# facebook/facebook360_dep

Measured on AMD Instinct MI355X. Metric: depth Mpix/s per GPU (full pyramid, 16-cam 2048^2 rig); % HBM-read roofline, higher is better.
Workload: dtype f32+f64; 1 GPU; BASELINE config 3: 16-camera 2048x2048 synthetic rig, 8-frame sequence, full 10-level pyramid per frame, per-level temporal filter (+-2 frames); the same sequence for every --gpus N (block partition, 8 frame(s) on this rank); rig=cfg2, cameras=16, frames=8, temporal_filter=True, halo_transport=local, parallelism=frames x1

## Files before the change

### facebook360_dep_amd/csrc/derp_capi.hip

```cpp
#include <hip/hip_runtime.h>

#include <algorithm>
#include <cfloat>
#include <cmath>
#include <cstdarg>
#include <cstdio>
#include <cstdlib>
#include <cstring>
#include <map>
#include <memory>
#include <string>
#include <vector>

#include <rocprim/device/device_radix_sort.hpp>

#include "../../include/derp_hip.h"
#include "derp_host.h"
#include "derp_kernels.h"
#include "derp_mesh.h"
#include "derp_points.h"
#include "derp_render.h"

using namespace derp;

#include "derp_ctx.h"

namespace {

struct Span {
  derp_ctx* c;
  int stage, level;
  hipEvent_t a = nullptr, b = nullptr;
  Span(derp_ctx* ctx, int st, int lv) : c(ctx), stage(st), level(lv) {
    if (c->profiling) {
      (void)hipEventCreate(&a);
      (void)hipEventCreate(&b);
      (void)hipEventRecord(a, c->stream);
    }
  }
  ~Span() {
    if (c->profiling && a) {
      (void)hipEventRecord(b, c->stream);
      c->spans.push_back({stage, level, a, b});
    }
  }
};

void drain_spans(derp_ctx* c) {
  for (auto& s : c->spans) {
    (void)hipEventSynchronize(s.b);
    float ms = 0;
    (void)hipEventElapsedTime(&ms, s.a, s.b);
    if (s.level >= 0 && s.level < kMaxLevels) {
      c->accMs[s.stage][s.level] += ms;
      c->accLaunch[s.stage][s.level] += 1;
    }
    (void)hipEventDestroy(s.a);
    (void)hipEventDestroy(s.b);
  }
  c->spans.clear();
}

size_t npx(const derp_ctx* c, int level) {
  return (size_t)c->LW[level] * c->LH[level];
}

unsigned long long* counter_slot(derp_ctx* c, int stage, int level) {
  return c->counters.as<unsigned long long>() + ((size_t)stage * kMaxLevels + level) * 4;
}

LevelView make_view(derp_ctx* c, int stage, int dst0, int nd) {
  LevelView V;
  const int L = c->cur;
  V.W = c->LW[L];
  V.H = c->LH[L];
  V.Wd = (double)V.W;
  V.Hd = (double)V.H;
  V.S = c->S;
  V.D = nd;
  V.level = L;
  V.numLevels = c->numLevels;
  V.dst0 = dst0;
  V.hasFg = c->opt.use_foreground_masks;
  const float scale = float(V.W) / c->heightFull;
  const float scaleVar = scale * scale;
  V.varNoiseFloor = std::max(c->opt.var_noise_floor * scaleVar, kMinVar);
  V.varHighThresh = c->opt.var_high_thresh;
  V.minDepthM = c->opt.min_depth_m;
  V.maxDepthM = c->opt.max_depth_m;
  V.randomProposals = c->opt.random_proposals;
  V.partialCoverage = c->opt.partial_coverage;
  V.xcdRotate = c->xcdRotate;
  V.camsSrc = c->camsSrc.as<Cam>();
  V.camsDst = c->camsDst.as<Cam>();
  V.dst2src = c->dst2src.as<int>();
  V.srcColor = c->frame().color[L].as<ushort4>();
  V.ownBias = c->w.ownBias.as<ushort4>();
  V.srcVar = c->w.srcVar.as<float>();
  V.srcFg = c->frame().fg[L].as<uint8_t>();
  V.rayDir = c->rayDir.as<double>();
  V.behind = c->behind.as<unsigned>();
  V.rayStride = (size_t)c->D * V.W * V.H;
  V.projWarp = c->projWarp.as<float2>();
  V.projColor = c->w.projColor.as<ushort4>();
  V.projBias = c->w.projBias.as<ushort4>();
  V.projColorT = c->w.projColorT.as<ushort4>();
  V.disparity = c->w.disparity.as<float>();
  V.cost = c->w.cost.as<float>();
  V.confidence = c->w.confidence.as<float>();
  V.bgDisp = c->frame().bg[L].as<float>();
  V.fovMask = c->w.fovMask.as<uint8_t>();
  V.pairCount = c->w.pairCount.as<uint8_t>();
  V.counters = counter_slot(c, stage, L);
  return V;
}

const dim3 kBlurBlk(64, 4, 1);
dim3 blur_grid(int ow, int oh, int planes) {
  return dim3((ow + 63) / 64, (oh + 4 * kBlurRows - 1) / (4 * kBlurRows), planes);
}

void lanczos_coeffs(float x, float* coeffs) {
  static const double s45 = 0.70710678118654752440084436210485;
  static const double cs[][2] = {{1, 0}, {-s45, -s45}, {0, 1}, {s45, -s45}, {-1, 0}, {s45, s45}, {0, -1}, {-s45, s45}};
  if (x < 1.1920928955078125e-07f) {
    for (int i = 0; i < 8; i++) {
      coeffs[i] = 0;
    }
    coeffs[3] = 1;
    return;
  }
  float sum = 0;
  const double y0 = -(x + 3) * M_PI * 0.25, s0 = std::sin(y0), c0 = std::cos(y0);
  for (int i = 0; i < 8; i++) {
    const double y = -(x + 3 - i) * M_PI * 0.25;
    coeffs[i] = (float)((cs[i][0] * s0 + cs[i][1] * c0) / (y * y));
    sum += coeffs[i];
  }
  sum = 1.f / sum;
  for (int i = 0; i < 8; i++) {
    coeffs[i] *= sum;
  }
}

int get_lanczos(derp_ctx* c, int ssize, int dsize, LanczosTab** out) {
  auto key = std::make_pair(ssize, dsize);
  auto it = c->lanczos.find(key);
  if (it != c->lanczos.end()) {
    *out = &it->second;
    return 0;
  }
  std::vector<int> ofs(dsize);
  std::vector<float> coef((size_t)dsize * 8);
  const double scale = (double)ssize / dsize;
  for (int d = 0; d < dsize; ++d) {
    float f = (float)((d + 0.5) * scale - 0.5);
    int s = (int)f;
    s -= (s > f);
    f -= s;
    ofs[d] = s;
    lanczos_coeffs(f, &coef[(size_t)d * 8]);
  }
  LanczosTab t;
  ALLOC(c, t.ofs, ofs.size() * sizeof(int));
  ALLOC(c, t.coef, coef.size() * sizeof(float));
  HIPCHK(c, hipMemcpyAsync(t.ofs.p, ofs.data(), ofs.size() * sizeof(int), hipMemcpyHostToDevice, c->stream));
  HIPCHK(c, hipMemcpyAsync(t.coef.p, coef.data(), coef.size() * sizeof(float), hipMemcpyHostToDevice, c->stream));
  HIPCHK(c, hipStreamSynchronize(c->stream));
  *out = &(c->lanczos[key] = std::move(t));
  return 0;
}

int get_area_tab(derp_ctx* c, int ssize, int dsize, AreaTabDev** out, bool forceTable = false) {
  auto key = std::make_pair(forceTable ? -ssize : ssize, dsize);
  auto it = c->areaTabs.find(key);
  if (it != c->areaTabs.end()) {
    *out = &it->second;
    return 0;
  }
  AreaTabDev t;
  const double scale = (double)ssize / dsize;
  const int iscale = (int)std::nearbyint(scale);
  std::vector<int> start(dsize + 1, 0), si;
  std::vector<float> alpha;
  if (!forceTable && iscale >= 1 && std::abs(scale - iscale) < 2.220446049250313e-16) {
    t.iscale = iscale;
  } else {
    for (int dx = 0; dx < dsize; ++dx) {
      start[dx] = (int)si.size();
      const double fsx1 = dx * scale, fsx2 = fsx1 + scale;
      const double cellWidth = std::min(scale, ssize - fsx1);
      int sx1 = (int)std::ceil(fsx1), sx2 = (int)std::floor(fsx2);
      sx2 = std::min(sx2, ssize - 1);
      sx1 = std::min(sx1, sx2);
      if (sx1 - fsx1 > 1e-3) {
        si.push_back(sx1 - 1);
        alpha.push_back((float)((sx1 - fsx1) / cellWidth));
      }
      for (int sx = sx1; sx < sx2; ++sx) {
        si.push_back(sx);
        alpha.push_back(float(1.0 / cellWidth));
      }
      if (fsx2 - sx2 > 1e-3) {
        si.push_back(sx2);
        alpha.push_back((float)(std::min(std::min(fsx2 - sx2, 1.), cellWidth) / cellWidth));
      }
    }
    start[dsize] = (int)si.size();
  }
  if (si.empty()) {
    si.push_back(0);
    alpha.push_back(0.f);
  }
  ALLOC(c, t.start, start.size() * sizeof(int));
  ALLOC(c, t.si, si.size() * sizeof(int));
  ALLOC(c, t.alpha, alpha.size() * sizeof(float));
  HIPCHK(c, hipMemcpy(t.start.p, start.data(), start.size() * sizeof(int), hipMemcpyHostToDevice));
  HIPCHK(c, hipMemcpy(t.si.p, si.data(), si.size() * sizeof(int), hipMemcpyHostToDevice));
  HIPCHK(c, hipMemcpy(t.alpha.p, alpha.data(), alpha.size() * sizeof(float), hipMemcpyHostToDevice));
  *out = &(c->areaTabs[key] = std::move(t));
  return 0;
}

int resize_area_dev(derp_ctx* c, int kind, const void* src, int sw, int sh, void* dst, int dw, int dh, int threshold) {
  if (dw > sw || dh > sh) {
    if (kind < 2) {
      return fail(c, "pyramid levels must not be larger than the full-size frame (%dx%d -> %dx%d)", sw, sh, dw, dh);
    }
    const dim3 g = grid2d(dw, dh, 1, kBlk2d);
    if (kind == 3) {
      hipLaunchKernelGGL(k_resize_linear_area_f32<3>, g, kBlk2d, 0, c->stream, (const float*)src, sw, sh, (float*)dst, dw, dh);
    } else {
      hipLaunchKernelGGL(k_resize_linear_area_f32<1>, g, kBlk2d, 0, c->stream, (const float*)src, sw, sh, (float*)dst, dw, dh);
    }
    KCHECK(c);
    return 0;
  }
  AreaTabDev *tx, *ty;
  TRY(get_area_tab(c, sw, dw, &tx));
  TRY(get_area_tab(c, sh, dh, &ty));
  if ((tx->iscale > 0) != (ty->iscale > 0)) {
    if (tx->iscale > 0) {
      TRY(get_area_tab(c, sw, dw, &tx, true));
    } else {
      TRY(get_area_tab(c, sh, dh, &ty, true));
    }
  }
  AreaAxis ax{tx->start.as<int>(), tx->si.as<int>(), tx->alpha.as<float>(), tx->iscale};
  AreaAxis ay{ty->start.as<int>(), ty->si.as<int>(), ty->alpha.as<float>(), ty->iscale};
  const dim3 g = grid2d(dw, dh, 1, kBlk2d);
  if (kind == 0) {
    hipLaunchKernelGGL(k_resize_area<0>, g, kBlk2d, 0, c->stream, src, sw, sh, dst, dw, dh, ax, ay, threshold);
  } else if (kind == 1) {
    hipLaunchKernelGGL(k_resize_area<1>, g, kBlk2d, 0, c->stream, src, sw, sh, dst, dw, dh, ax, ay, threshold);
  } else if (kind == 3) {
    hipLaunchKernelGGL(k_resize_area<3>, g, kBlk2d, 0, c->stream, src, sw, sh, dst, dw, dh, ax, ay, threshold);
  } else {
    hipLaunchKernelGGL(k_resize_area<2>, g, kBlk2d, 0, c->stream, src, sw, sh, dst, dw, dh, ax, ay, threshold);
  }
  KCHECK(c);
  return 0;
}

std::vector<int2> make_spiral(int w) {
  int x = 0, y = 0, dx = 0, dy = -1, t = w;
  const int samples = t * t;
  std::vector<int2> locs;
  for (int i = 0; i < samples; ++i) {
    const bool vx = (-w / 2 <= x) && (x <= w / 2), vy = (-w / 2 <= y) && (y <= w / 2);
    if (vx && vy) {
      locs.push_back(make_int2(x, y));
    }
    if (x == y || ((x < 0) && (x == -y)) || ((x > 0) && (x == 1 - y))) {
      t = dx;
      dx = -dy;
      dy = t;
    }
    x += dx;
    y += dy;
  }
  return locs;
}

int ensure_spiral(derp_ctx* c, int radius) {
  if (c->spiralRadius == radius) {
    return 0;
  }
  const std::vector<int2> s = make_spiral(radius * 2 + 1);
  ALLOC(c, c->spiral, s.size() * sizeof(int2));
  HIPCHK(c, hipMemcpy(c->spiral.p, s.data(), s.size() * sizeof(int2), hipMemcpyHostToDevice));
  c->spiralN = (int)s.size();
  c->spiralRadius = radius;
  return 0;
}

int upsample_lanczos_dev(derp_ctx* c, const float* in, int sw, int sh, float* out, int dw, int dh, int planes,
                         size_t inStride, size_t outStride) {
  if (sw == dw && sh == dh) {
    return fail(c, "upsample to identical size not supported");
  }
  LanczosTab *tx, *ty;
  TRY(get_lanczos(c, sw, dw, &tx));
  TRY(get_lanczos(c, sh, dh, &ty));
  const size_t tmpStride = (size_t)dw * sh;
  ALLOC(c, c->w.lanczosTmp, tmpStride * planes * sizeof(float));
  hipLaunchKernelGGL(k_lanczos_h, grid2d(dw, sh, planes, kBlk2d), kBlk2d, 0, c->stream, in, sw, sh, dw,
                     tx->ofs.as<int>(), tx->coef.as<float>(), c->w.lanczosTmp.as<float>(), inStride, tmpStride);
  KCHECK(c);
  hipLaunchKernelGGL(k_lanczos_v, grid2d(dw, dh, planes, kBlk2d), kBlk2d, 0, c->stream, c->w.lanczosTmp.as<float>(), sh,
                     dw, dh, ty->ofs.as<int>(), ty->coef.as<float>(), out, tmpStride, outStride);
  KCHECK(c);
  return 0;
}

int upsample_masked_dev(derp_ctx* c, const float* in, const uint8_t* mask, int sw, int sh, const uint8_t* maskUp,
                        const float* bgUp, float* out, int dw, int dh, int planes = 1) {
  const float scale = float(dw) / float(sw);
  const int radius = (int)(scale * scale + 1);
  TRY(ensure_spiral(c, radius));
  ALLOC(c, c->w.lanczosTmp, (size_t)dw * dh * planes * sizeof(float));
  hipLaunchKernelGGL(k_upsample_nearest_masked, grid2d(dw, dh, planes, kBlk2d), kBlk2d, 0, c->stream, in, mask, sw, sh,
                     maskUp, dw, dh, c->w.lanczosTmp.as<float>());
  KCHECK(c);
  hipLaunchKernelGGL(k_spiral_fill, grid2d(dw, dh, planes, kBlk2d), kBlk2d, 0, c->stream, c->w.lanczosTmp.as<float>(), bgUp,
                     maskUp, dw, dh, c->spiral.as<int2>(), c->spiralN, out);
  KCHECK(c);
  return 0;
}

bool batch_needs_inverse_warps(const derp_ctx* c, int dst0, int nd) {
  std::vector<char> covered(c->S, 0);
  for (int d = dst0; d < dst0 + nd; ++d) {
    covered[c->dst2srcH[d]] = 1;
  }
  for (int s = 0; s < c->S; ++s) {
    if (!covered[s]) {
      return true;
    }
  }
  return false;
}

size_t table_bytes_per_dst(const derp_ctx* c, int W, int H, bool withInverse) {
  const size_t wp = (size_t)(W + 2 * kPadW) * (H + 2 * kPadW), cp = (size_t)(W + 2 * kPadC) * (H + 2 * kPadC);
  return (size_t)(c->S - 1) * (wp * sizeof(float2) + 2 * cp * sizeof(ushort4) + (withInverse ? (size_t)W * H * sizeof(float2) : 0) +
                               (DERP_RANDOM_TILED ? tiled_plane(W, H) * sizeof(ushort4) : 0));
}

int compute_fov_and_masks(derp_ctx* c, int level) {
  const int W = c->LW[level], H = c->LH[level];
  const size_t n = (size_t)W * H;
  {
    Span sp(c, ST_FOV, level);
    hipLaunchKernelGGL(k_fov_mask, grid2d(W, H, c->D, kBlk2d), kBlk2d, 0, c->stream, c->camsDst.as<Cam>(), W, H,
                       c->w.fovMask.as<uint8_t>());
    KCHECK(c);
    hipLaunchKernelGGL(k_and_masks, dim3(flat_grid(n), c->D), dim3(256), 0, c->stream, c->w.fovMask.as<uint8_t>(),
                       c->frame().fg[level].as<uint8_t>(), c->dst2src.as<int>(), 0, n, c->w.maskAnd.as<uint8_t>());
    KCHECK(c);
  }
  return 0;
}

int build_warp(derp_ctx* c, int dst0, int nd) {
  const int L = c->cur;
  Span sp(c, ST_PROJ_WARP, L);
  {
    const size_t n = (size_t)c->LW[L] * c->LH[L];
    ALLOC(c, c->rayDir, 3 * n * c->D * sizeof(double));
    ALLOC(c, c->behind, n * c->D * sizeof(unsigned));
  }
  LevelView V = make_view(c, ST_PROJ_WARP, dst0, nd);
  hipLaunchKernelGGL(k_proj_warp, grid2d(V.W + 2 * kPadW, V.H + 2 * kPadW, c->S, kBlk2d), kBlk2d, 0, c->stream, V,
                     c->projWarp.as<float2>());
  KCHECK(c);
  hipLaunchKernelGGL(k_pixel_rays, grid2d(V.W, V.H, nd, kBlk2d), kBlk2d, 0, c->stream, V, c->rayDir.as<double>(),
                     c->behind.as<unsigned>());
  KCHECK(c);
  c->w.colorTablesCleanLevel = -1;
  if (batch_needs_inverse_warps(c, dst0, nd)) {
    hipLaunchKernelGGL(k_proj_warp_inv, grid2d(V.W, V.H, nd, kBlk2d), kBlk2d, 0, c->stream, V, c->projWarpInv.as<float2>());
    KCHECK(c);
  }
  return 0;
}

int build_color_tables(derp_ctx* c, int dst0, int nd) {
  const int L = c->cur;
  LevelView V = make_view(c, ST_REPROJECT, dst0, nd);
  Span sp(c, ST_REPROJECT, L);
  const dim3 grid((V.W + kRbTile - 1) / kRbTile, (V.H + kRbTile - 1) / kRbTile, nd * (c->S - 1));
  ALLOC(c, c->w.tileSeen, (size_t)grid.x * grid.y * grid.z);
  const int skipBlank = c->w.colorTablesCleanLevel == L && nd == c->D && !c->noBlankSkip;
  hipLaunchKernelGGL(k_reproject_bias, grid, dim3(256), 0, c->stream, V, c->projWarpInv.as<float2>(),
                     c->w.projColor.as<ushort4>(), c->w.projBias.as<ushort4>(), c->w.projColorT.as<ushort4>(),
                     c->w.tileSeen.as<uint8_t>(), skipBlank);
  KCHECK(c);
  c->w.colorTablesCleanLevel = nd == c->D ? L : -1;
  return 0;
}

int tiles_of(int W, int H, int& tilesX) {
  constexpr int B = kTileBlock;
  tilesX = ((W + 15) / 16 + B - 1) / B * B;
  const int tilesY = ((H + 15) / 16 + B - 1) / B * B;
  return tilesX * tilesY * (256 / kCostBlock);
}
constexpr size_t kCostLdsPerSrc = (size_t)kCostBlock * sizeof(SsdPair);
int round8(int n) {
  return (n + 7) / 8 * 8;
}
size_t lds_for_waves(size_t needed, int waves, size_t ldsPerCu, size_t fixed) {
  if (waves <= 0 || waves >= 4) {
    return needed;
  }
  const size_t perBlock = ldsPerCu / (size_t)(4 * waves + 1) + 256;
  return std::max(needed, perBlock > fixed ? perBlock - fixed : needed);
}
constexpr size_t kCostLdsStatic = sizeof(PatchWin) * (kCostBlock / 64) + kAtanLutDoubles * sizeof(double);
bool cost_four_waves(const derp_ctx* c) {
  if (const char* e = getenv("DERP_COST_WAVES")) {
    return atoi(e) >= 4;
  }
  return 16 * (kCostLdsPerSrc * (size_t)c->S + kCostLdsStatic) <= c->ldsPerCu && c->S <= 16;
}

int run_brute_force(derp_ctx* c, int dst0, int nd) {
  const int L = c->cur;
  if (L != c->numLevels - 1) {
    return 0;
  }
  Span sp(c, ST_BRUTE, L);
  LevelView V = make_view(c, ST_BRUTE, dst0, nd);
  const size_t n = (size_t)V.W * V.H;
  ALLOC(c, c->w.bruteCost, (size_t)nd * kNumDepths * n * sizeof(float));
  ALLOC(c, c->w.bruteConf, (size_t)nd * kNumDepths * n * sizeof(float));
  const int tilesX = std::max(1, (V.W - 2 + 7) / 8), tilesY = std::max(1, (V.H - 2 + 7) / 8);
  const int tiles = tilesX * tilesY;
  const size_t lds = kCostLdsPerSrc * (size_t)(c->S);
  hipLaunchKernelGGL(k_brute_costs, dim3(tiles, kNumDepths, nd), dim3(kCostBlock), lds, c->stream, V,
                     c->w.bruteCost.as<float>(), c->w.bruteConf.as<float>(), tilesX, tiles);
  KCHECK(c);
  hipLaunchKernelGGL(k_brute_select, grid2d(V.W, V.H, nd, kBlk2d), kBlk2d, 0, c->stream, V, c->w.bruteCost.as<float>(),
                     c->w.bruteConf.as<float>());
  KCHECK(c);
  hipLaunchKernelGGL(k_brute_margin, grid2d(V.W, V.H, nd, kBlk2d), kBlk2d, 0, c->stream, V);
  KCHECK(c);
  return 0;
}

int run_random_proposals(derp_ctx* c, int dst0, int nd) {
  const int L = c->cur;
  if (c->opt.random_proposals <= 0 || L == c->numLevels - 1) {
    return 0;
  }
  Span sp(c, ST_RANDOM, L);
  c->randomRanThisLevel = true;
  LevelView V = make_view(c, ST_RANDOM, dst0, nd);
  if (V.H > 2 && V.W > 2) {
    hipLaunchKernelGGL(k_row_rank, dim3(V.H - 2, nd), dim3(256), 0, c->stream, V, c->w.rank.as<int>());
    KCHECK(c);
  }
  int tilesX;
  const int tiles = tiles_of(V.W, V.H, tilesX);
  const size_t lds = lds_for_waves(kCostLdsPerSrc * (size_t)(c->S), c->randomWaves, c->ldsPerCu, kCostLdsStatic);
  hipLaunchKernelGGL(cost_four_waves(c) ? k_random_proposals : k_random_proposals_w3, dim3(round8(tiles), nd),
                     dim3(kCostBlock), lds, c->stream, V, c->w.rank.as<int>(), tilesX, tiles);
  KCHECK(c);
  return 0;
}

int run_ping_pong(derp_ctx* c, int dst0, int nd) {
  const int L = c->cur;
  if (L == c->numLevels - 1) {
    return 0;
  }
  Span sp(c, ST_PINGPONG, L);
  LevelView V = make_view(c, ST_PINGPONG, dst0, nd);
  const size_t n = (size_t)V.W * V.H;
  HIPCHK(c, hipMemsetAsync(c->w.changed.as<uint8_t>() + (size_t)dst0 * n, 1, n * nd, c->stream));
  int tilesX;
  const int tiles = tiles_of(V.W, V.H, tilesX);
  const size_t lds = lds_for_waves(kCostLdsPerSrc * (size_t)(c->S), c->ppWaves, c->ldsPerCu, kCostLdsStatic);
  const bool four = cost_four_waves(c);
  const auto kernel = c->ppCompact ? (four ? k_ping_pong : k_ping_pong_w3) : (four ? k_ping_pong_loop : k_ping_pong_loop_w3);
  for (int it = 1; it <= c->opt.ping_pong_iterations; ++it) {
    hipLaunchKernelGGL(kernel, dim3(round8(tiles), nd), dim3(kCostBlock), lds,
                       c->stream, V, c->w.changed.as<uint8_t>(), c->w.dispRes.as<float>(), c->w.costRes.as<float>(), tilesX,
                       (int)(it == 1 && c->randomRanThisLevel && !c->noMemo));
    KCHECK(c);
    hipLaunchKernelGGL(k_ping_pong_commit, dim3(flat_grid(n * nd)), dim3(256), 0, c->stream,
                       c->w.disparity.as<float>() + (size_t)dst0 * n, c->w.cost.as<float>() + (size_t)dst0 * n,
                       c->w.dispRes.as<float>() + (size_t)dst0 * n, c->w.costRes.as<float>() + (size_t)dst0 * n,
                       c->w.changed.as<uint8_t>() + (size_t)dst0 * n, n * nd);
    KCHECK(c);
  }
  if (dst0 + nd >= c->D) {
    c->randomRanThisLevel = false;
  }
  return 0;
}

int run_mismatches(derp_ctx* c) {
  const int L = c->cur;
  if (L > c->opt.mismatches_start_level || L == c->numLevels - 1) {
    return 0;
  }
  if (c->D != c->S) {
    return fail(c, "Check failed: rigDst.size() == rigSrc.size()  Mismatches only valid when considering all cameras");
  }
  for (int d = 0; d < c->D; ++d) {
    if (c->dst2srcH[d] != d) {
      return fail(c, "mismatch handling needs destinations in rig order (dst %d maps to src %d)", d, c->dst2srcH[d]);
    }
  }
  Span sp(c, ST_MISMATCH, L);
  c->randomRanThisLevel = false;
  LevelView V = make_view(c, ST_MISMATCH, 0, c->D);
  const size_t n = (size_t)V.W * V.H;
  hipLaunchKernelGGL(k_mismatch, dim3((V.W + 15) / 16, (V.H + 15) / 16, c->D), dim3(256), 256 * sizeof(float) * c->S,
                     c->stream, V, c->w.dispRes.as<float>(), c->w.mismatchMask.as<uint8_t>());
  KCHECK(c);
  HIPCHK(c, hipMemcpyAsync(c->w.disparity.p, c->w.dispRes.p, n * c->D * sizeof(float), hipMemcpyDeviceToDevice, c->stream));
  return 0;
}

int bilateral_radius(int level) {
  const float scale = std::pow(0.9f, level);
  return (int)std::max(std::ceil(5 * scale), float(1));
}

size_t bilateral_lds_bytes(int radius) {
  const size_t side = 16 + 2 * (size_t)radius;
  const size_t t = ((side + 15) & ~(size_t)15) * side;
  return t * 4 * sizeof(float) + ((t + 3) & ~(size_t)3);
}

constexpr size_t kBilateralMaxLds = 64 * 1024 - 256;

int run_bilateral(derp_ctx* c) {
  const int L = c->cur;
  Span sp(c, ST_BILATERAL, L);
  c->randomRanThisLevel = false;
  const int W = c->LW[L], H = c->LH[L];
  const size_t n = (size_t)W * H;
  const int radius = bilateral_radius(L);
  hipLaunchKernelGGL(k_joint_bilateral<true>, dim3((W + 15) / 16, (H + 15) / 16, c->D), dim3(256),
                     bilateral_lds_bytes(radius), c->stream, c->w.disparity.as<float>(),
                     (const void*)c->frame().color[L].as<ushort4>(), c->w.maskAnd.as<uint8_t>(), W, H, radius, 0.005f, 0.5f,
                     1.0f, 1.0f, c->w.tmpF.as<float>(), n, n, c->dst2src.as<int>());
  KCHECK(c);
  HIPCHK(c, hipMemcpyAsync(c->w.disparity.p, c->w.tmpF.p, n * c->D * sizeof(float), hipMemcpyDeviceToDevice, c->stream));
  return 0;
}

int run_median(derp_ctx* c, bool fuseMaskFov) {
  const int L = c->cur;
  Span sp(c, ST_MEDIAN, L);
  c->randomRanThisLevel = false;
  const int W = c->LW[L], H = c->LH[L];
  const size_t n = (size_t)W * H;
  hipLaunchKernelGGL(k_masked_median, grid2d(W, H, c->D, kBlk2d), kBlk2d, 0, c->stream, c->w.disparity.as<float>(),
                     c->opt.use_foreground_masks ? c->frame().bg[L].as<float>() : (const float*)nullptr,
                     c->w.maskAnd.as<uint8_t>(), W, H, 1, c->w.tmpF.as<float>(), n,
                     fuseMaskFov ? c->w.fovMask.as<uint8_t>() : (const uint8_t*)nullptr);
  KCHECK(c);
  HIPCHK(c, hipMemcpyAsync(c->w.disparity.p, c->w.tmpF.p, n * c->D * sizeof(float), hipMemcpyDeviceToDevice, c->stream));
  return 0;
}

int run_mask_fov(derp_ctx* c) {
  const int L = c->cur;
  Span sp(c, ST_MASKFOV, L);
  const size_t n = npx(c, L) * c->D;
  hipLaunchKernelGGL(k_mask_fov, dim3(flat_grid(n)), dim3(256), 0, c->stream, c->w.disparity.as<float>(),
                     c->w.fovMask.as<uint8_t>(), n);
  KCHECK(c);
  return 0;
}

int check_level(derp_ctx* c, int level) {
  if (!c || c->numLevels == 0) {
    return fail(c, "derp_set_pyramid has not been called");
  }
  if (level < 0 || level >= c->numLevels) {
    return fail(c, "level %d out of range [0, %d)", level, c->numLevels);
  }
  if (c->LW[level] <= 0 || c->LH[level] <= 0) {
    return fail(c, "level %d was declared absent in derp_set_pyramid", level);
  }
  return 0;
}

int level_begin(derp_ctx* c, int level, bool buildAllTables) {
  TRY(check_level(c, level));
  if (c->S - 1 > kMaxSrc) {
    return fail(c, "too many source cameras (%d > %d)", c->S, kMaxSrc + 1);
  }
  c->cur = level;
  const int W = c->LW[level], H = c->LH[level];
  const size_t n = (size_t)W * H;
  if (W < 3 || H < 3) {
    return fail(c, "level %d is too small (%dx%d)", level, W, H);
  }
  TRY(compute_fov_and_masks(c, level));
  {
    Span sp(c, ST_VARIANCE, level);
    hipLaunchKernelGGL(k_variance, grid2d(W, H, c->S, kBlk2d), kBlk2d, 0, c->stream, c->frame().color[level].as<ushort4>(),
                       W, H, c->w.srcVar.as<float>());
    KCHECK(c);
  }
  {
    Span sp(c, ST_OWN_BIAS, level);
    hipLaunchKernelGGL(k_blur3_u16, blur_grid(W, H, c->S), kBlurBlk, 0, c->stream,
                       c->frame().color[level].as<ushort4>(), 0, c->w.ownBias.as<ushort4>(), 0, W, H, n, n);
    KCHECK(c);
  }
  HIPCHK(c, hipMemsetAsync(c->w.cost.p, 0, n * c->D * sizeof(float), c->stream));
  HIPCHK(c, hipMemsetAsync(c->w.confidence.p, 0, n * c->D * sizeof(float), c->stream));
  HIPCHK(c, hipMemsetAsync(c->w.mismatchMask.p, 0, n * c->D, c->stream));
  if (level < c->numLevels - 1 && !c->frame().haveDisp[level + 1] && !buildAllTables) {
    return fail(c, "Missing disparity of level %d needed to start level %d", level + 1, level);
  }
  if (level < c->numLevels - 1 && c->frame().haveDisp[level + 1]) {
    Span sp(c, ST_UPSAMPLE, level);
    const int sw = c->LW[level + 1], sh = c->LH[level + 1];
    if (!c->opt.use_foreground_masks) {
      TRY(upsample_lanczos_dev(c, c->frame().disp[level + 1].as<float>(), sw, sh, c->w.disparity.as<float>(), W, H, c->D,
                               (size_t)sw * sh, n));
    } else {
      ALLOC(c, c->w.staging, (size_t)sw * sh * c->D);
      hipLaunchKernelGGL(k_fov_mask, grid2d(sw, sh, c->D, kBlk2d), kBlk2d, 0, c->stream, c->camsDst.as<Cam>(), sw, sh,
                         c->w.staging.as<uint8_t>());
      KCHECK(c);
      hipLaunchKernelGGL(k_and_masks, dim3(flat_grid((size_t)sw * sh), c->D), dim3(256), 0, c->stream,
                         c->w.staging.as<uint8_t>(), c->frame().fg[level + 1].as<uint8_t>(), c->dst2src.as<int>(), 0,
                         (size_t)sw * sh, c->w.staging.as<uint8_t>());
      KCHECK(c);
      TRY(upsample_masked_dev(c, c->frame().disp[level + 1].as<float>(), c->w.staging.as<uint8_t>(), sw, sh,
                              c->w.maskAnd.as<uint8_t>(), c->frame().bg[level].as<float>(), c->w.disparity.as<float>(), W, H, c->D));
    }
  } else {
// ... 127 lines not shown
    ALLOC(c, f.bg[l], n * c->D * sizeof(float));
    ALLOC(c, f.disp[l], n * c->D * sizeof(float));
    HIPCHK(c, hipMemsetAsync(f.fg[l].p, 1, n * c->S, c->stream));
    HIPCHK(c, hipMemsetAsync(f.bg[l].p, 0, n * c->D * sizeof(float), c->stream));
  }
  return 0;
}

int alloc_work_set(derp_ctx* c, WorkSet& w, size_t n) {
  ALLOC(c, w.srcVar, n * c->S * sizeof(float));
  ALLOC(c, w.ownBias, n * c->S * sizeof(ushort4));
  ALLOC(c, w.fovMask, n * c->D);
  ALLOC(c, w.maskAnd, n * c->D);
  for (DevBuf* b : {&w.disparity, &w.cost, &w.confidence, &w.dispRes, &w.costRes, &w.tmpF, &w.rank}) {
    ALLOC(c, *b, n * c->D * sizeof(float));
  }
  ALLOC(c, w.changed, n * c->D);
  ALLOC(c, w.mismatchMask, n * c->D);
  ALLOC(c, w.pairCount, n * c->D);
  return 0;
}

int select_frame(derp_ctx* c, int slot) {
  if (slot < 0 || slot >= (int)c->frames.size()) {
    return fail(c, "frame slot %d out of range [0, %d)", slot, (int)c->frames.size());
  }
  if (slot != c->curSlot) {
    c->curSlot = slot;
    c->cur = -1;
  }
  return 0;
}

void lane_swap(derp_ctx* c, int i) {
  std::swap(c->stream, c->lanes[i]->stream);
  std::swap(c->w, c->lanes[i]->w);
}

int lanes_prepare(derp_ctx* c, int count, size_t n) {
  while ((int)c->lanes.size() < count) {
    c->lanes.emplace_back(new WorkLane);
    WorkLane& l = *c->lanes.back();
    if (hipStreamCreateWithFlags(&l.stream, hipStreamNonBlocking) != hipSuccess ||
        hipEventCreateWithFlags(&l.done, hipEventDisableTiming) != hipSuccess) {
      return fail(c, "work lane: hipStreamCreate / hipEventCreate failed");
    }
  }
  if (!c->laneReady) {
    HIPCHK(c, hipEventCreateWithFlags(&c->laneReady, hipEventDisableTiming));
  }
  for (int i = 0; i < count; ++i) {
    TRY(alloc_work_set(c, c->lanes[i]->w, n));
  }
  return 0;
}

int process_level_on_lane(derp_ctx* c, int i, int slot, int level) {
  if (i < 0) {
    TRY(select_frame(c, slot));
    return process_level(c, level);
  }
  HIPCHK(c, hipStreamWaitEvent(c->lanes[i]->stream, c->laneReady, 0));
  lane_swap(c, i);
  c->activeLane = i;
  int rc = select_frame(c, slot);
  if (!rc) {
    rc = process_level(c, level);
  }
  if (!rc && hipEventRecord(c->lanes[i]->done, c->stream) != hipSuccess) {
    rc = fail(c, "work lane: hipEventRecord failed");
  }
  lane_swap(c, i);
  c->activeLane = -1;
  c->cur = -1;
  return rc;
}

int temporal_launch(derp_ctx* c, const void* const* guides, const float* const* images, const uint8_t* const* masks, int n,
                    int centre, int W, int H, int planes, float sigma, int radius, float w0, float w1, float w2,
                    float* out, const int* dst2src) {
  if (n < 1 || centre < 0 || centre >= n) {
    return fail(c, "temporal window must hold at least the centre frame");
  }
  if (n > kMaxTemporalFrames) {
    ALLOC(c, c->temporalCarry, (size_t)planes * W * H * sizeof(float2));
  }
  for (int t0 = 0; t0 < n; t0 += kMaxTemporalFrames) {
    TemporalFrames F;
    F.n = std::min(kMaxTemporalFrames, n - t0);
    for (int t = 0; t < F.n; ++t) {
      F.guides[t] = reinterpret_cast<const ushort4*>(guides[t0 + t]);
      F.images[t] = images[t0 + t];
      F.masks[t] = masks[t0 + t];
    }
    F.refGuide = reinterpret_cast<const ushort4*>(guides[centre]);
    F.refImage = images[centre];
    F.refMask = masks[centre];
    F.carry = n > kMaxTemporalFrames ? c->temporalCarry.as<float2>() : nullptr;
    F.first = t0 == 0;
    F.last = t0 + F.n >= n;
    const size_t lds = 2 * ((((size_t)(32 + 2 * radius) * (8 + 2 * radius) * 9) + 15) & ~(size_t)15);
    if (radius >= 0 && lds <= 48 * 1024 && !c->noTemporalTile) {
      hipLaunchKernelGGL(k_temporal_tiled, grid2d(W, H, planes, kBlk2d), kBlk2d, lds, c->stream, F, W, H, sigma, radius, w0,
                         w1, w2, out, dst2src);
    } else {
      hipLaunchKernelGGL(k_temporal, grid2d(W, H, planes, kBlk2d), kBlk2d, 0, c->stream, F, W, H, sigma, radius, w0, w1, w2,
                         out, dst2src);
    }
    KCHECK(c);
  }
  return 0;
}

}

extern "C" {

void derp_options_default(derp_options* o) {
  o->min_depth_m = 0.5f;
  o->max_depth_m = 1e4f;
  o->var_noise_floor = 4e-5f;
  o->var_high_thresh = 1e-3f;
  o->random_proposals = 2;
  o->ping_pong_iterations = 1;
  o->mismatches_start_level = -1;
  o->do_bilateral_filter = 1;
  o->do_median_filter = 1;
  o->use_foreground_masks = 0;
  o->partial_coverage = 0;
  o->rebuild_warp_tables = 1;
}

int derp_create(derp_ctx** out, int device, const derp_camera_desc* src, int n_src, const derp_camera_desc* dst,
                int n_dst) {
  if (!out) {
    return 1;
  }
  *out = nullptr;
  std::unique_ptr<derp_ctx> owner(new derp_ctx);
  derp_ctx* c = owner.get();
  derp_options_default(&c->opt);
  if (n_src <= 0 || n_dst <= 0) {
    return create_fail("no source / destination cameras!");
  }
  hipDeviceProp_t prop;
  TRY(open_device(device, "the depth path", &prop));
  c->device = device;
  if (prop.maxSharedMemoryPerMultiProcessor > 0) {
    c->ldsPerCu = prop.maxSharedMemoryPerMultiProcessor;
  }
  if (const char* e = getenv("DERP_XCD_ROTATE")) {
    c->xcdRotate = atoi(e);
  }
  c->noMemo = getenv("DERP_NO_MEMO") != nullptr;
  if (const char* e = getenv("DERP_PP_COMPACT")) {
    c->ppCompact = atoi(e) != 0;
  }
  if (const char* e = getenv("DERP_RANDOM_WAVES")) {
    c->randomWaves = atoi(e);
  }
  if (const char* e = getenv("DERP_PP_WAVES")) {
    c->ppWaves = atoi(e);
  }
  c->noTemporalTile = getenv("DERP_NO_TEMPORAL_TILE") != nullptr;
  c->noBlankSkip = getenv("DERP_NO_BLANK_SKIP") != nullptr;
  c->S = n_src;
  c->D = n_dst;
  c->frames.resize(1);
  c->camsSrcH.resize(n_src);
  c->camsDstH.resize(n_dst);
  for (int i = 0; i < n_src; ++i) {
    if (const char* m = host_prepare_camera(src[i], c->camsSrcH[i])) {
      return create_fail(std::string("camera ") + src[i].id + ": " + m);
    }
  }
  c->dst2srcH.assign(n_dst, 0);
  c->descDstH.assign(dst, dst + n_dst);
  for (int i = 0; i < n_dst; ++i) {
    if (const char* m = host_prepare_camera(dst[i], c->camsDstH[i])) {
      return create_fail(std::string("camera ") + dst[i].id + ": " + m);
    }
    bool found = false;
    for (int s = 0; s < n_src; ++s) {
      if (strncmp(dst[i].id, src[s].id, sizeof dst[i].id) == 0) {
        c->dst2srcH[i] = s;
        found = true;
        break;
      }
    }
    if (!found) {
      return create_fail(std::string("destination camera ") + dst[i].id + " is not a source camera");
    }
    if (memcmp(&c->camsDstH[i], &c->camsSrcH[c->dst2srcH[i]], sizeof(Cam)) != 0) {
      return create_fail(std::string("destination camera ") + dst[i].id + " differs from the source camera of the same id "
                  "(destinations must be cameras of the source rig, as filterDestinations makes them)");
    }
  }
  if (c->camsSrc.ensure(sizeof(Cam) * n_src) || c->camsDst.ensure(sizeof(Cam) * n_dst) ||
      c->dst2src.ensure(sizeof(int) * n_dst) || c->counters.ensure(sizeof(unsigned long long) * ST_COUNT * kMaxLevels * 4)) {
    return create_fail("out of device memory");
  }
  if (hipStreamCreateWithFlags(&c->stream, hipStreamNonBlocking) != hipSuccess) {
    return create_fail("hipStreamCreate failed");
  }
  if (hipStreamCreateWithFlags(&c->copyStream, hipStreamNonBlocking) != hipSuccess) {
    (void)hipStreamDestroy(c->stream);
    return create_fail("hipStreamCreate failed");
  }
  (void)hipMemcpy(c->camsSrc.p, c->camsSrcH.data(), sizeof(Cam) * n_src, hipMemcpyHostToDevice);
  (void)hipMemcpy(c->camsDst.p, c->camsDstH.data(), sizeof(Cam) * n_dst, hipMemcpyHostToDevice);
  (void)hipMemcpy(c->dst2src.p, c->dst2srcH.data(), sizeof(int) * n_dst, hipMemcpyHostToDevice);
  (void)hipMemset(c->counters.p, 0, c->counters.bytes);
  *out = owner.release();
  return 0;
}

void derp_destroy(derp_ctx* c) {
  if (!c) {
    return;
  }
  (void)hipSetDevice(c->device);
  (void)hipStreamSynchronize(c->stream);
  for (auto& l : c->lanes) {
    (void)hipStreamSynchronize(l->stream);
  }
  drain_spans(c);
  for (auto& l : c->lanes) {
    (void)hipStreamDestroy(l->stream);
    (void)hipEventDestroy(l->done);
  }
  if (c->laneReady) {
    (void)hipEventDestroy(c->laneReady);
  }
  (void)hipStreamDestroy(c->stream);
  (void)hipStreamDestroy(c->copyStream);
  delete c;
}

const char* derp_last_error(const derp_ctx* c) {
  return c ? c->err.c_str() : g_create_error.c_str();
}

int derp_set_options(derp_ctx* c, const derp_options* o) {
  if (!c || !o) {
    return 1;
  }
  if (o->random_proposals < 0) {
    return fail(c, "Check failed: random_proposals >= 0");
  }
  c->opt = *o;
  return 0;
}

int derp_set_pyramid(derp_ctx* c, int num_levels, const int* widths, const int* heights, int width_full,
                     int height_full) {
  if (!c) {
    return 1;
  }
  if (num_levels <= 0 || num_levels > kMaxLevels) {
    return fail(c, "num_levels %d out of range (1..%d)", num_levels, kMaxLevels);
  }
  HIPCHK(c, hipSetDevice(c->device));
  c->numLevels = num_levels;
  c->widthFull = width_full;
  c->heightFull = height_full;
  c->LW.assign(widths, widths + num_levels);
  c->LH.assign(heights, heights + num_levels);
  c->frames.clear();
  c->frames.resize(1);
  c->curSlot = 0;
  TRY(alloc_pyramid(c, c->frame()));
  size_t nmax = 0;
  for (int l = 0; l < num_levels; ++l) {
    nmax = std::max(nmax, npx(c, l));
  }
  TRY(alloc_work_set(c, c->w, nmax));
  c->cur = -1;
  c->warpCachedLevel = -1;
  HIPCHK(c, hipStreamSynchronize(c->stream));
  return 0;
}

int derp_set_frame_slots(derp_ctx* c, int n_slots) {
  if (!c || c->numLevels == 0) {
    return fail(c, "derp_set_pyramid has not been called");
  }
  if (n_slots < 1 || n_slots > 4096) {
    return fail(c, "n_slots %d out of range (1..4096)", n_slots);
  }
  HIPCHK(c, hipSetDevice(c->device));
  TRY(select_frame(c, 0));
  const int had = (int)c->frames.size();
  c->frames.resize(n_slots);
  for (int k = had; k < n_slots; ++k) {
    TRY(alloc_pyramid(c, c->frames[k]));
  }
  HIPCHK(c, hipStreamSynchronize(c->stream));
  return 0;
}

int derp_select_frame(derp_ctx* c, int slot) {
  if (!c || c->numLevels == 0) {
    return fail(c, "derp_set_pyramid has not been called");
  }
  return select_frame(c, slot);
}
// ... 326 lines not shown
```

### facebook360_dep_amd/csrc/derp_ctx.h

```cpp
#pragma once

namespace {

enum Stage {
  ST_FOV = 0,
  ST_VARIANCE,
  ST_OWN_BIAS,
  ST_UPSAMPLE,
  ST_PROJ_WARP,
  ST_REPROJECT,
  ST_PROJ_BIAS,
  ST_BRUTE,
  ST_RANDOM,
  ST_PINGPONG,
  ST_MISMATCH,
  ST_BILATERAL,
  ST_MEDIAN,
  ST_MASKFOV,
  ST_TEMPORAL,
  ST_LANES,
  ST_COUNT
};
const char* kStageNames[ST_COUNT] = {"fov_mask",  "variance",    "own_bias",         "upsample",  "proj_warp",
                                     "reproject", "proj_bias",   "brute_force",      "random_proposals",
                                     "ping_pong", "mismatches",  "bilateral",        "median",    "mask_fov",
                                     "temporal",  "lanes_wall"};
constexpr int kMaxLevels = 24;

struct TimedSpan {
  int stage, level;
  hipEvent_t a, b;
};

struct LanczosTab {
  DevBuf ofs, coef;
};

struct AreaTabDev {
  DevBuf start, si, alpha;
  int iscale = 0;
};

struct WorkSet {
  DevBuf srcVar, ownBias, fovMask, maskAnd, disparity, cost, confidence, dispRes, costRes, changed, tmpF, rank, mismatchMask, pairCount;
  DevBuf tileSeen;
  DevBuf projColor, projBias;
  DevBuf projColorT;
  DevBuf bruteCost, bruteConf, lanczosTmp, staging, stagingB;
  int colorTablesCleanLevel = -1;
};

struct FramePyramid {
  std::vector<DevBuf> color, fg, bg, disp;
  std::vector<char> haveBg, haveDisp;
};

struct WorkLane {
  hipStream_t stream = nullptr;
  hipEvent_t done = nullptr;
  WorkSet w;
};

struct SmrState; struct RephotoState; struct PointsState; struct MeshState;

}

struct derp_ctx {
  derp_ctx();
  ~derp_ctx();
  int device = 0;
  hipStream_t stream = nullptr;
  hipStream_t copyStream = nullptr;
  DevBuf copyStaging;
  std::string err;
  std::string* errSink() {
    return &err;
  }
  derp_options opt;
  int S = 0, D = 0;
  std::vector<Cam> camsSrcH, camsDstH;
  std::vector<int> dst2srcH;
  std::vector<derp_camera_desc> descDstH;
  DevBuf camsSrc, camsDst, dst2src;

  int numLevels = 0, widthFull = 0, heightFull = 0;
  std::vector<int> LW, LH;
  std::vector<FramePyramid> frames;
  int curSlot = 0;
  FramePyramid& frame() {
    return frames[curSlot];
  }
  DevBuf fullFrame;
  DevBuf devMask;

  int cur = -1;
  int DB = 0;
  WorkSet w;
  DevBuf temporalCarry;
  DevBuf projWarp, projWarpInv;
  DevBuf rayDir, behind;
  int warpCachedLevel = -1;
  bool randomRanThisLevel = false;
  bool tablesValid = false;
  std::map<std::pair<int, int>, LanczosTab> lanczos;
  std::map<std::pair<int, int>, AreaTabDev> areaTabs;
  DevBuf spiral;
  int spiralN = 0, spiralRadius = -1;
  std::vector<std::unique_ptr<WorkLane>> lanes;
  hipEvent_t laneReady = nullptr;
  int activeLane = -1;

  DevBuf counters;
  bool profiling = false;
  std::vector<TimedSpan> spans;
  double accMs[ST_COUNT][kMaxLevels] = {};
  int accLaunch[ST_COUNT][kMaxLevels] = {};
  int xcdRotate = 1;
  bool noMemo = false;
  bool ppCompact = true;
  int randomWaves = 0, ppWaves = 0;
  size_t ldsPerCu = 160 * 1024;
  bool noTemporalTile = false;
  bool noBlankSkip = false;
  std::unique_ptr<SmrState> smr;
  std::unique_ptr<RephotoState> rephoto;
  std::unique_ptr<PointsState> points;
  std::unique_ptr<MeshState> mesh;
};

namespace {

int fail(derp_ctx* c, const char* fmt, ...) {
  va_list ap;
  va_start(ap, fmt);
  vfail(c ? &c->err : nullptr, fmt, ap);
  va_end(ap);
  return 1;
}

int use_device(derp_ctx* c) {
  if (!c) {
    return 1;
  }
  HIPCHK(c, hipSetDevice(c->device));
  return 0;
}

int check_camera(derp_ctx* c, int cam) {
  if (cam < 0 || cam >= c->D) {
    return fail(c, "bad camera index %d (the context has %d)", cam, c->D);
  }
  return 0;
}

}
```

### facebook360_dep_amd/csrc/derp_debug_api.h

```cpp
#pragma once

namespace {
struct HostPairs {
  SsdPair* p;
  SsdPair get(int i) const {
    return p[i];
  }
  void set(int i, const SsdPair& v) {
    p[i] = v;
  }
};
int stage_index(const char* stage) {
  for (int i = 0; i < ST_COUNT; ++i) {
    if (strcmp(stage, kStageNames[i]) == 0) {
      return i;
    }
  }
  return -1;
}
}

int derp_debug_atan2_ypos(derp_ctx* c, const double* y, const double* x, double* out, size_t n) {
  if (!c || !y || !x || !out) {
    return fail(c, "bad arguments");
// ... 90 lines not shown
    return 0;
  }
  return fail(c, "unknown table id %d", which);
}

int derp_dev_disparity(derp_ctx* c, int level, int d, float** ptr, size_t* bytes) {
  TRY(check_level(c, level));
  if (d < 0 || d >= c->D || !ptr || !bytes) {
    return fail(c, "bad destination index / null output");
  }
  const size_t n = npx(c, level);
  *ptr = c->frame().disp[level].as<float>() + (size_t)d * n;
  *bytes = n * sizeof(float);
  return 0;
}
int derp_dev_color(derp_ctx* c, int level, int s, void** ptr, size_t* bytes) {
  TRY(check_level(c, level));
  if (s < 0 || s >= c->S || !ptr || !bytes) {
    return fail(c, "bad source index / null output");
  }
  const size_t n = npx(c, level);
  *ptr = c->frame().color[level].as<ushort4>() + (size_t)s * n;
  *bytes = n * sizeof(ushort4);
  return 0;
}
int derp_dev_mask(derp_ctx* c, int level, int d, uint8_t** ptr, size_t* bytes) {
  TRY(check_level(c, level));
  if (d < 0 || d >= c->D || !ptr || !bytes) {
    return fail(c, "bad destination index / null output");
  }
  HIPCHK(c, hipSetDevice(c->device));
  const int W = c->LW[level], H = c->LH[level];
  const size_t n = (size_t)W * H;
  ALLOC(c, c->devMask, n * c->D);
  hipLaunchKernelGGL(k_fov_mask, grid2d(W, H, c->D, kBlk2d), kBlk2d, 0, c->stream, c->camsDst.as<Cam>(), W, H,
                     c->devMask.as<uint8_t>());
  KCHECK(c);
  hipLaunchKernelGGL(k_and_masks, dim3(flat_grid(n), c->D), dim3(256), 0, c->stream, c->devMask.as<uint8_t>(),
                     c->frame().fg[level].as<uint8_t>(), c->dst2src.as<int>(), 0, n, c->devMask.as<uint8_t>());
  KCHECK(c);
  HIPCHK(c, hipStreamSynchronize(c->stream));
  *ptr = c->devMask.as<uint8_t>() + (size_t)d * n;
  *bytes = n;
  return 0;
}

int derp_get_counters(derp_ctx* c, uint64_t* n_cost, uint64_t* n_pair, uint64_t* insufficient) {
  if (!c) {
    return 1;
  }
  HIPCHK(c, hipStreamSynchronize(c->stream));
  std::vector<unsigned long long> h((size_t)ST_COUNT * kMaxLevels * 4);
  HIPCHK(c, hipMemcpy(h.data(), c->counters.p, h.size() * sizeof(unsigned long long), hipMemcpyDeviceToHost));
  uint64_t a = 0, b = 0, i = 0;
  for (size_t k = 0; k < h.size(); k += 4) {
    a += h[k];
    b += h[k + 1];
    i += h[k + 2];
  }
  if (n_cost) {
    *n_cost = a;
  }
  if (n_pair) {
    *n_pair = b;
  }
  if (insufficient) {
    *insufficient = i;
  }
  return 0;
}
int derp_reset_counters(derp_ctx* c) {
  if (!c) {
    return 1;
  }
  HIPCHK(c, hipMemsetAsync(c->counters.p, 0, c->counters.bytes, c->stream));
  return 0;
}
int derp_profile_enable(derp_ctx* c, int on) {
  if (!c) {
    return 1;
  }
  c->profiling = on != 0;
  return 0;
}
int derp_profile_reset(derp_ctx* c) {
  if (!c) {
    return 1;
  }
  HIPCHK(c, hipStreamSynchronize(c->stream));
  drain_spans(c);
  memset(c->accMs, 0, sizeof c->accMs);
  memset(c->accLaunch, 0, sizeof c->accLaunch);
  return derp_reset_counters(c);
}
int derp_profile_query(derp_ctx* c, const char* stage, int level, double* ms, int* launches, uint64_t* n_cost,
                       uint64_t* n_pair) {
  if (!c || !stage) {
    return 1;
  }
  const int st = stage_index(stage);
  if (st < 0) {
    return fail(c, "unknown stage '%s'", stage);
  }
  HIPCHK(c, hipStreamSynchronize(c->stream));
  drain_spans(c);
  std::vector<unsigned long long> h((size_t)kMaxLevels * 4);
  HIPCHK(c, hipMemcpy(h.data(), counter_slot(c, st, 0), h.size() * sizeof(unsigned long long), hipMemcpyDeviceToHost));
  double m = 0;
  int l = 0;
  uint64_t a = 0, b = 0;
  for (int lv = 0; lv < kMaxLevels; ++lv) {
    if (level >= 0 && lv != level) {
      continue;
    }
    m += c->accMs[st][lv];
    l += c->accLaunch[st][lv];
    a += h[(size_t)lv * 4];
    b += h[(size_t)lv * 4 + 1];
  }
  if (ms) {
    *ms = m;
  }
  if (launches) {
    *launches = l;
  }
  if (n_cost) {
    *n_cost = a;
  }
  if (n_pair) {
    *n_pair = b;
  }
  return 0;
}
int derp_profile_memoised(derp_ctx* c, const char* stage, int level, uint64_t* n_memoised) {
  if (!c || !stage || !n_memoised) {
    return 1;
  }
  const int st = stage_index(stage);
  if (st < 0) {
    return fail(c, "unknown stage '%s'", stage);
  }
  HIPCHK(c, hipStreamSynchronize(c->stream));
  std::vector<unsigned long long> h((size_t)kMaxLevels * 4);
  HIPCHK(c, hipMemcpy(h.data(), counter_slot(c, st, 0), h.size() * sizeof(unsigned long long), hipMemcpyDeviceToHost));
  uint64_t m = 0;
  for (int lv = 0; lv < kMaxLevels; ++lv) {
    if (level < 0 || lv == level) {
      m += h[(size_t)lv * 4 + 3];
    }
  }
  *n_memoised = m;
  return 0;
}
int derp_device_memory(derp_ctx* c, uint64_t* free_bytes, uint64_t* total_bytes) {
  TRY(use_device(c));
  size_t f = 0, t = 0;
  HIPCHK(c, hipMemGetInfo(&f, &t));
  if (free_bytes) {
    *free_bytes = f;
  }
  if (total_bytes) {
    *total_bytes = t;
  }
  return 0;
}

int derp_device_name(derp_ctx* c, char* buf, int n) {
  if (!c || !buf || n <= 0) {
    return 1;
  }
  hipDeviceProp_t prop;
  HIPCHK(c, hipGetDeviceProperties(&prop, c->device));
  snprintf(buf, n, "%s (%s, %d CUs)", prop.name, prop.gcnArchName, prop.multiProcessorCount);
  return 0;
}

int derp_host_nth_element_pairs(float* pairs, int n, int nth) {
  HostPairs acc{reinterpret_cast<SsdPair*>(pairs)};
  GccSelect<HostPairs> sel(acc);
  sel.nth_element(nth, n);
  return 0;
}
float derp_host_minstd_uniform(int seed, uint64_t draw_index, float a, float b) {
  uint32_t state = minstd_jump(minstd_seed(seed), draw_index);
  return minstd_uniform(state, a, b);
}
```

### facebook360_dep_amd/csrc/derp_kernels.h

```cpp
#pragma once
#include <hip/hip_runtime.h>
#include <math.h>
#include <stdint.h>

#include <type_traits>

#include "derp_camera.h"
#include "gcc_algos.h"

namespace derp {

#ifndef DERP_COST_MIN_WAVES
#define DERP_COST_MIN_WAVES 4
#endif
#ifndef DERP_RANDOM_MIN_WAVES
#define DERP_RANDOM_MIN_WAVES 4
#endif
#ifndef DERP_RANDOM_TILED
#define DERP_RANDOM_TILED 0
#endif
#ifndef DERP_MIX_HOT_ONLY
#define DERP_MIX_HOT_ONLY 0
#endif
#ifndef DERP_PHASE_TIMERS
#define DERP_PHASE_TIMERS 0
#endif
static constexpr int kCostBlock = 64;
static constexpr int kTileBlock = 4;
static constexpr int kPadW = 1;
static constexpr int kPadC = 2;
static constexpr int kMaxSrc = 32;
static constexpr int kNumDepths = 150;
static constexpr float kMinVar = 1.0f / 12.0f / 65025.0f;

typedef float f4a8 __attribute__((ext_vector_type(4), aligned(8)));
typedef unsigned int u4a8 __attribute__((ext_vector_type(4), aligned(8)));

struct LevelView {
  int W, H, S, D;
  double Wd, Hd;
  int level, numLevels;
  int dst0;
  int hasFg;
  float varNoiseFloor, varHighThresh;
  float minDepthM, maxDepthM;
  int randomProposals;
  int partialCoverage;
  int xcdRotate;
  const Cam* camsSrc;
  const Cam* camsDst;
  const int* dst2src;
  const ushort4* srcColor;
  const ushort4* ownBias;
  const float* srcVar;
  const uint8_t* srcFg;
  const double* rayDir;
  const unsigned* behind;
  size_t rayStride;
  const float2* projWarp;
  const ushort4* projColor;
  const ushort4* projBias;
  const ushort4* projColorT;
  float* disparity;
  float* cost;
  float* confidence;
  const float* bgDisp;
  const uint8_t* fovMask;
  uint8_t* pairCount;
  unsigned long long* counters;
};

__device__ __forceinline__ size_t warp_plane(const LevelView& V) {
  return (size_t)(V.W + 2 * kPadW) * (V.H + 2 * kPadW);
}
__device__ __forceinline__ size_t color_plane(const LevelView& V) {
  return (size_t)(V.W + 2 * kPadC) * (V.H + 2 * kPadC);
}
__host__ __device__ __forceinline__ int tiled_tiles_x(int W) {
  return (W + 2 * kPadC + 3) >> 2;
}
__host__ __device__ __forceinline__ size_t tiled_plane(int W, int H) {
  return (size_t)tiled_tiles_x(W) * (size_t)((H + 2 * kPadC + 3) >> 2) * 16;
}
__device__ __forceinline__ size_t tiled_index(int tilesX, int ox, int oy) {
  return ((size_t)(oy >> 2) * tilesX + (ox >> 2)) * 16 + (size_t)((oy & 3) * 4 + (ox & 3));
}
__device__ __forceinline__ int slot(int s, int own) {
  return s < own ? s : s - 1;
}
template <typename T>
__device__ __forceinline__ T& at32(T* base, unsigned i) {
  return *reinterpret_cast<T*>(reinterpret_cast<char*>(const_cast<typename std::remove_const<T>::type*>(base)) + i * (unsigned)sizeof(T));
}

__device__ __forceinline__ int xcd_swizzle(int b, int n, int rot) {
  const int per = (n + 7) >> 3;
  const int t = (((b & 7) + rot) & 7) * per + (b >> 3);
  return t;
}

__device__ __forceinline__ void tile_pixel(int item, int tilesX, int& x, int& y) {
  const int lane = threadIdx.x & 63;
  const int gw = item * (int)(blockDim.x >> 6) + (int)(threadIdx.x >> 6);
  const int super = gw >> 2, quad = gw & 3;
  constexpr int B = kTileBlock;
  const int blk = super / (B * B), in = super % (B * B);
  const int blocksX = tilesX / B;
  const int tx = (blk % blocksX) * B + (in % B), ty = (blk / blocksX) * B + (in / B);
  x = tx * 16 + (quad & 1) * 8 + (lane & 7);
  y = ty * 16 + (quad >> 1) * 8 + (lane >> 3);
}

__device__ __forceinline__ float bilerp_f(float p00, float p01, float p10, float p11, float w00, float w01,
                                          float w10, float w11) {
  return w00 * p00 + w01 * p01 + w10 * p10 + w11 * p11;
}
__device__ __forceinline__ float bilerp_u16(float p00, float p01, float p10, float p11, float w00, float w01,
                                            float w10, float w11) {
  const float v = w00 * p00 + w01 * p01 + w10 * p10 + w11 * p11;
  return __builtin_truncf(v);
}

typedef float v2f __attribute__((ext_vector_type(2)));
__device__ __forceinline__ v2f splat2(float a) {
  return (v2f){a, a};
}
__device__ __forceinline__ v2f trunc2(v2f v) {
  return (v2f){__builtin_truncf(v.x), __builtin_truncf(v.y)};
}
__device__ __forceinline__ v2f bg_of(unsigned u) {
  return (v2f){(float)(u & 0xffff), (float)(u >> 16)};
}

static constexpr int kWinW = 10, kWinTexels = kWinW * kWinW;
struct PatchWin {
  v2f bg[kWinTexels];
  float r[kWinTexels];
};

struct PixCtx {
  D3 rayO, rayD;
  const v2f* winBG;
  const float* winR;
  v2f dstBiasBG;
  float dstBiasR;
  __device__ __forceinline__ v2f patchBG(int ix, int iy) const {
    return winBG[iy * kWinW + ix];
  }
  __device__ __forceinline__ float patchR(int ix, int iy) const {
    return winR[iy * kWinW + ix];
  }
  __device__ __forceinline__ float patch(int ix, int iy, int c) const {
    return c == 2 ? patchR(ix, iy) : c == 0 ? patchBG(ix, iy).x : patchBG(ix, iy).y;
  }
  __device__ __forceinline__ float dstBias(int c) const {
    return c == 0 ? dstBiasBG.x : c == 1 ? dstBiasBG.y : dstBiasR;
  }
  float confidence;
};

__device__ __forceinline__ void patch_window_fill(const LevelView& V, int own, int x0, int y0, PatchWin* win) {
  const ushort4* col = V.srcColor + (size_t)own * ((size_t)V.W * V.H);
  for (int t = (int)(threadIdx.x & 63); t < kWinTexels; t += 64) {
    const int j = t / kWinW, i = t - j * kWinW;
    const int xx = min(max(x0 - 1 + i, 0), V.W - 1), yy = min(max(y0 - 1 + j, 0), V.H - 1);
    const ushort4 q = col[(size_t)yy * V.W + xx];
    win->bg[t] = (v2f){(float)q.x, (float)q.y};
    win->r[t] = (float)q.z;
  }
}

struct LdsPairs {
  SsdPair* base;
  int stride;
  const double* atanLut;
  __device__ __forceinline__ SsdPair get(int i) const {
    return base[i * stride];
  }
  __device__ __forceinline__ void set(int i, const SsdPair& v) {
    base[i * stride] = v;
  }
};

__device__ __forceinline__ LdsPairs cost_wave_prologue(const LevelView& V, int d, int x0, int y0, PatchWin*& win) {
  extern __shared__ SsdPair ldsPairs[];
  __shared__ PatchWin patchWin[kCostBlock / 64];
  win = &patchWin[threadIdx.x >> 6];
  patch_window_fill(V, V.dst2src[d], x0, y0, win);
#if defined(__HIP_DEVICE_COMPILE__)
  __shared__ double atanLut[kAtanLutDoubles];
  atan_lut_fill(atanLut);
  LdsPairs pairs{ldsPairs + threadIdx.x, (int)blockDim.x, atanLut};
#else
  LdsPairs pairs{ldsPairs + threadIdx.x, (int)blockDim.x, nullptr};
#endif
  __syncthreads();
  return pairs;
}

struct SsdTexels {
  u4a8 raw[4][2];
  u4a8 ba, bb;
};
template <bool TILED>
__device__ __forceinline__ void ssd_issue_random(const LevelView& V, const ushort4* __restrict__ col, const ushort4* __restrict__ colT,
                                                 const ushort4* __restrict__ bia, float xDstSrc, float yDstSrc, SsdTexels& T,
                                                 bool& border) {
  const int pitch = V.W + 2 * kPadC;
  const int xi = (int)roundf(xDstSrc), yi = (int)roundf(yDstSrc);
  const unsigned off = ((unsigned)(yi - 2 + kPadC) * (unsigned)pitch + (unsigned)(xi - 2 + kPadC)) * 8u;
  if constexpr (TILED) {
    const unsigned xa = (unsigned)(xi - 2 + kPadC), ya = (unsigned)(yi - 2 + kPadC);
    const unsigned rowTiles = (unsigned)tiled_tiles_x(V.W) * 128u;
    const unsigned xr = xa & 3u, yr = ya & 3u;
    const unsigned base0 = (ya >> 2) * rowTiles + (xa >> 2) * 128u + yr * 32u + xr * 8u;
    const char* base = reinterpret_cast<const char*>(colT);
    typedef unsigned int u2 __attribute__((ext_vector_type(2)));
#pragma unroll
    for (int row = 0; row < 4; ++row) {
      const unsigned ro = base0 + (unsigned)row * 32u + ((yr + (unsigned)row > 3u) ? rowTiles - 128u : 0u);
#pragma unroll
      for (int k = 0; k < 4; ++k) {
        const unsigned o = ro + (unsigned)k * 8u + ((xr + (unsigned)k > 3u) ? 96u : 0u);
        const u2 t = *reinterpret_cast<const u2*>(base + o);
        if (k & 1) {
          T.raw[row][k >> 1].z = t.x;
          T.raw[row][k >> 1].w = t.y;
        } else {
          T.raw[row][k >> 1].x = t.x;
          T.raw[row][k >> 1].y = t.y;
        }
      }
    }
  } else {
    const char* base = reinterpret_cast<const char*>(col);
#pragma unroll
    for (int row = 0; row < 4; ++row) {
      T.raw[row][0] = *reinterpret_cast<const u4a8*>(base + (off + (unsigned)row * (unsigned)pitch * 8u));
      T.raw[row][1] = *reinterpret_cast<const u4a8*>(base + (off + (unsigned)row * (unsigned)pitch * 8u + 16u));
    }
  }
  border = xi < 2 || yi < 2 || xi > V.W - 2 || yi > V.H - 2;
  T.ba = T.bb = (u4a8){0u, 0u, 0u, 0u};
  if (border) {
    const unsigned boff = off + ((unsigned)pitch + 1u) * 8u;
    const char* bbase = reinterpret_cast<const char*>(bia);
    T.ba = *reinterpret_cast<const u4a8*>(bbase + boff);
    T.bb = *reinterpret_cast<const u4a8*>(bbase + (boff + (unsigned)pitch * 8u));
  }
}
__device__ __forceinline__ void ssd_issue(const LevelView& V, const ushort4* __restrict__ col,
                                          const ushort4* __restrict__ bia, float xDstSrc, float yDstSrc, SsdTexels& T) {
  const int pitch = V.W + 2 * kPadC;
  const int xi = (int)roundf(xDstSrc), yi = (int)roundf(yDstSrc);
  const unsigned off = ((unsigned)(yi - 2 + kPadC) * (unsigned)pitch + (unsigned)(xi - 2 + kPadC)) * 8u;
  const char* base = reinterpret_cast<const char*>(col);
#pragma unroll
  for (int row = 0; row < 4; ++row) {
    T.raw[row][0] = *reinterpret_cast<const u4a8*>(base + (off + (unsigned)row * (unsigned)pitch * 8u));
    T.raw[row][1] = *reinterpret_cast<const u4a8*>(base + (off + (unsigned)row * (unsigned)pitch * 8u + 16u));
  }
  const unsigned boff = off + ((unsigned)pitch + 1u) * 8u;
  const char* bbase = reinterpret_cast<const char*>(bia);
  T.ba = *reinterpret_cast<const u4a8*>(bbase + boff);
  T.bb = *reinterpret_cast<const u4a8*>(bbase + (boff + (unsigned)pitch * 8u));
}

template <bool RANDOM>
__device__ __forceinline__ SsdPair ssd_arith(const LevelView& V, const PixCtx& px, const ushort4* __restrict__ col,
                                             const SsdTexels& T, float xDstSrc, float yDstSrc, bool border = true) {
  const int pitch = V.W + 2 * kPadC;
  const u4a8 (&raw)[4][2] = T.raw;
  auto word_bg = [&](const u4a8 (&q)[4][2], int r, int k) { return (k & 1) ? q[r][k >> 1].z : q[r][k >> 1].x; };
  auto word_r = [&](const u4a8 (&q)[4][2], int r, int k) { return (k & 1) ? q[r][k >> 1].w : q[r][k >> 1].y; };
  float bias[3];
  const float bxf = roundf(xDstSrc), byf = roundf(yDstSrc);
  const float bxw = xDstSrc - bxf + 0.5f, byw = yDstSrc - byf + 0.5f;
  const float w00 = (1 - bxw) * (1 - byw), w01 = bxw * (1 - byw), w10 = (1 - bxw) * byw, w11 = bxw * byw;
  if constexpr (RANDOM) {
    float top[3][2], bot[3][2];
#pragma unroll
    for (int k = 3; k >= 0; --k) {
      float c[3][4];
#pragma unroll
      for (int r = 0; r < 4; ++r) {
        const unsigned bg = word_bg(raw, r, k), rr = word_r(raw, r, k);
        c[0][r] = (float)(bg & 0xffff);
        c[1][r] = (float)(bg >> 16);
        c[2][r] = (float)(rr & 0xffff);
      }
#pragma unroll
      for (int ch = 0; ch < 3; ++ch) {
        const float m = c[ch][1] + c[ch][2];
        const float vT = m + c[ch][0], vB = m + c[ch][3];
        if (k == 3) {
          top[ch][1] = vT + 4.0f;
          bot[ch][1] = vB + 4.0f;
        } else if (k == 2) {
          top[ch][1] += vT;
          bot[ch][1] += vB;
          top[ch][0] = vT + 4.0f;
          bot[ch][0] = vB + 4.0f;
        } else if (k == 1) {
          top[ch][1] += vT;
          bot[ch][1] += vB;
          top[ch][0] += vT;
          bot[ch][0] += vB;
        } else {
          top[ch][0] += vT;
          bot[ch][0] += vB;
        }
      }
    }
    const float ninth = 1.0f / 9.0f;
#pragma unroll
    for (int ch = 0; ch < 3; ++ch) {
      const float t00 = __builtin_truncf(top[ch][0] * ninth), t01 = __builtin_truncf(top[ch][1] * ninth);
      const float t10 = __builtin_truncf(bot[ch][0] * ninth), t11 = __builtin_truncf(bot[ch][1] * ninth);
      bias[ch] = px.dstBias(ch) - bilerp_u16(t00, t01, t10, t11, w00, w01, w10, w11);
    }
    if (__ballot(border) != 0ull) {
      if (border) {
        const u4a8 a = T.ba, b = T.bb;
        bias[0] = px.dstBias(0) - bilerp_u16((float)(a.x & 0xffff), (float)(a.z & 0xffff), (float)(b.x & 0xffff), (float)(b.z & 0xffff), w00, w01, w10, w11);
        bias[1] = px.dstBias(1) - bilerp_u16((float)(a.x >> 16), (float)(a.z >> 16), (float)(b.x >> 16), (float)(b.z >> 16), w00, w01, w10, w11);
        bias[2] = px.dstBias(2) - bilerp_u16((float)(a.y & 0xffff), (float)(a.w & 0xffff), (float)(b.y & 0xffff), (float)(b.w & 0xffff), w00, w01, w10, w11);
      }
    }
  } else {
    const u4a8 a = T.ba, b = T.bb;
    const v2f sbBG = trunc2(splat2(w00) * bg_of(a.x) + splat2(w01) * bg_of(a.z) + splat2(w10) * bg_of(b.x) +
                            splat2(w11) * bg_of(b.z));
    const v2f bBG = px.dstBiasBG - sbBG;
    bias[0] = bBG.x;
    bias[1] = bBG.y;
    bias[2] = px.dstBiasR - bilerp_u16((float)(a.y & 0xffff), (float)(a.w & 0xffff), (float)(b.y & 0xffff),
                                       (float)(b.w & 0xffff), w00, w01, w10, w11);
  }
  float first = 0.f, second = 0.f;
  u4a8 rawB[4][2];
#pragma unroll
  for (int r = 0; r < 4; ++r) {
    rawB[r][0] = raw[r][0];
    rawB[r][1] = raw[r][1];
    if constexpr (RANDOM) {
      unsigned a = raw[r][1].x, b = raw[r][1].y, c = raw[r][1].z, d = raw[r][1].w;
      asm("" : "+v"(a), "+v"(b), "+v"(c), "+v"(d));
      rawB[r][1] = (u4a8){a, b, c, d};
    }
  }
// ... 69 lines not shown
        const v2f v = splat2(w00) * lo.bg[iy] + splat2(w01) * hi.bg[iy] + splat2(w10) * lo.bg[iy + 1] +
                      splat2(w11) * hi.bg[iy + 1];
        const v2f db = px.patchBG(ix, iy) - trunc2(v);
        const v2f dn = db - biasBG;
        const v2f s0 = db * db, s1 = dn * dn;
        float t0 = s0.x + s0.y, t1 = s1.x + s1.y;
        asm("" : "+v"(t0), "+v"(t1));
        bgd0[iy] = t0;
        bgd1[iy] = t1;
      }
      v2f e0, e1;
      {
        const v2f v = w00p * lo.rE + w01p * hi.rE + w10p * lo.rO + w11p * hi.rO;
        const v2f db = (v2f){px.patchR(ix, 0), px.patchR(ix, 2)} - trunc2(v);
        const v2f dn = db - splat2(bias[2]);
        e0 = (v2f){bgd0[0], bgd0[2]} + db * db;
        e1 = (v2f){bgd1[0], bgd1[2]} + dn * dn;
      }
      float m0, m1;
      {
        const float v = w00m * lo.rO.x + w01m * hi.rO.x + w10m * lo.rE.y + w11m * hi.rE.y;
        const float db = px.patchR(ix, 1) - __builtin_truncf(v);
        const float dn = db - bias[2];
        m0 = bgd0[1] + db * db;
        m1 = bgd1[1] + dn * dn;
      }
      first += e0.x;
      first += m0;
      first += e0.y;
      second += e1.x;
      second += m1;
      second += e1.y;
      lo = hi;
    }
  };
  const float xfc = roundf(xDstSrc), yfc = roundf(yDstSrc);
  const bool exact = (xDstSrc >= 1.0f) && (yDstSrc >= 1.0f) && ((xDstSrc + 1.0f) - 1.0f == xDstSrc) &&
                     ((yDstSrc + 1.0f) - 1.0f == yDstSrc);
  int xi[3], yi[3];
  float xw[3], yw[3];
  bool regular = true;
  xi[1] = (int)xfc;
  yi[1] = (int)yfc;
  xw[0] = xw[1] = xw[2] = xDstSrc - xfc + 0.5f;
  yw[0] = yw[1] = yw[2] = yDstSrc - yfc + 0.5f;
  if (!exact) {
#pragma unroll
    for (int k = 0; k < 3; k += 2) {
      const float xs = xDstSrc + (float)(k - 1), ys = yDstSrc + (float)(k - 1);
      const float xf = roundf(xs), yf = roundf(ys);
      xi[k] = (int)xf;
      yi[k] = (int)yf;
      xw[k] = xs - xf + 0.5f;
      yw[k] = ys - yf + 0.5f;
    }
    regular = (xi[0] == xi[1] - 1) && (xi[2] == xi[1] + 1) && (yi[0] == yi[1] - 1) && (yi[2] == yi[1] + 1);
  }
  if (!RANDOM && __ballot(!exact) == 0ull) {
    const float xwu[3] = {xw[1], xw[1], xw[1]};
    block_packed(xwu, splat2(yw[1]), yw[1]);
  } else if (regular) {
    if constexpr (RANDOM) {
      block_scalar(xw, yw);
    } else {
      block_packed(xw, (v2f){yw[0], yw[2]}, yw[1]);
    }
  } else if (DERP_MIX_HOT_ONLY) {
    first = second = 0.f;
  } else {
    for (int ix = 0; ix < 3; ++ix) {
      for (int iy = 0; iy < 3; ++iy) {
        const float w00 = (1 - xw[ix]) * (1 - yw[iy]), w01 = xw[ix] * (1 - yw[iy]);
        const float w10 = (1 - xw[ix]) * yw[iy], w11 = xw[ix] * yw[iy];
        const int x0 = min(max(xi[ix] - 1, -kPadC), V.W + kPadC - 1), x1 = min(max(xi[ix], -kPadC), V.W + kPadC - 1);
        const int y0 = min(max(yi[iy] - 1, -kPadC), V.H + kPadC - 1), y1 = min(max(yi[iy], -kPadC), V.H + kPadC - 1);
        const ushort4 q00 = col[(size_t)(y0 + kPadC) * pitch + x0 + kPadC];
        const ushort4 q01 = col[(size_t)(y0 + kPadC) * pitch + x1 + kPadC];
        const ushort4 q10 = col[(size_t)(y1 + kPadC) * pitch + x0 + kPadC];
        const ushort4 q11 = col[(size_t)(y1 + kPadC) * pitch + x1 + kPadC];
        const float p00[3] = {(float)q00.x, (float)q00.y, (float)q00.z};
        const float p01[3] = {(float)q01.x, (float)q01.y, (float)q01.z};
        const float p10[3] = {(float)q10.x, (float)q10.y, (float)q10.z};
        const float p11[3] = {(float)q11.x, (float)q11.y, (float)q11.z};
        const v2f pbg = px.winBG[iy * kWinW + ix];
        const float pch[3] = {pbg.x, pbg.y, px.winR[iy * kWinW + ix]};
        float d0 = 0.f, d1 = 0.f;
        for (int c = 0; c < 3; ++c) {
          const float cs = bilerp_u16(p00[c], p01[c], p10[c], p11[c], w00, w01, w10, w11);
          const float db = pch[c] - cs;
          const float dn = db - bias[c];
          d0 += db * db;
          d1 += dn * dn;
        }
        first += d0;
        second += d1;
      }
    }
  }
  const float scale = 1.0f / (65535.0f * 65535.0f);
  return {first * scale, second * scale};
}
template <bool RANDOM>
__device__ __forceinline__ SsdPair compute_ssd(const LevelView& V, const PixCtx& px, const ushort4* __restrict__ col,
                                               const ushort4* __restrict__ bia, float xDstSrc, float yDstSrc,
                                               const ushort4* __restrict__ colT = nullptr) {
  SsdTexels T;
  if constexpr (RANDOM) {
    bool border;
    ssd_issue_random<DERP_RANDOM_TILED != 0>(V, col, colT, bia, xDstSrc, yDstSrc, T, border);
    return ssd_arith<true>(V, px, col, T, xDstSrc, yDstSrc, border);
  } else {
    ssd_issue(V, col, bia, xDstSrc, yDstSrc, T);
    return ssd_arith<false>(V, px, col, T, xDstSrc, yDstSrc);
  }
}

static constexpr double kCullMinDepth = 0.05;
__device__ __forceinline__ unsigned behind_mask(const LevelView& V, int own, const D3& rayO, const D3& rayD) {
  unsigned m = 0;
  for (int s = 0; s < V.S; ++s) {
    if (s == own) {
      continue;
    }
    const Cam& cs = V.camsSrc[s];
    const double a = sum3(cs.R[6] * (rayO.x - cs.pos[0]), cs.R[7] * (rayO.y - cs.pos[1]), cs.R[8] * (rayO.z - cs.pos[2]));
    const double b = sum3(cs.R[6] * rayD.x, cs.R[7] * rayD.y, cs.R[8] * rayD.z);
    if (cs.cos_fov >= 0 && b > 1e-6 && a + kCullMinDepth * b > 1e-6) {
      m |= 1u << slot(s, own);
    }
  }
  return m;
}
__device__ __forceinline__ unsigned behind_sources(const LevelView& V, int d, size_t idx) {
  const unsigned m = V.behind[(size_t)d * ((size_t)V.W * V.H) + idx];
  unsigned cull = 0;
  for (int t = 0; t < V.S - 1; ++t) {
    if (__ballot(!((m >> t) & 1u)) == 0ull) {
      cull |= 1u << t;
    }
  }
  return __builtin_amdgcn_readfirstlane(cull);
}

struct PhaseTimers {
  unsigned proj = 0, ssd = 0, select = 0, inside = 0;
};
__device__ __forceinline__ unsigned phase_clock() {
#if DERP_PHASE_TIMERS
  return (unsigned)__builtin_amdgcn_s_memtime();
#else
  return 0u;
#endif
}
template <bool RANDOM>
constexpr int cost_sees_lean() {
  return 2 + (RANDOM ? 4 : 0);
}

template <bool RANDOM = false, bool RELOAD_RAY = false>
__device__ __forceinline__ float2 compute_cost(const LevelView& V, int dl, int own, const PixCtx& px, float disparity,
                                               LdsPairs& pairs, unsigned& nPair, unsigned cull = 0, unsigned pix = 0,
                                               unsigned* slots = nullptr, PhaseTimers* tm = nullptr) {
  const unsigned tc0 = phase_clock();
  const double depth = (double)(1.0f / disparity);
  D3 rayD = px.rayD;
  if constexpr (RELOAD_RAY) {
    unsigned i = pix;
    asm("" : "+v"(i) : "v"(disparity));
    const double* rd = V.rayDir + (size_t)(V.dst0 + dl) * ((size_t)V.W * V.H);
    if constexpr (RANDOM) {
      rayD = {at32(rd, i), at32(rd + V.rayStride, i), at32(rd + 2 * V.rayStride, i)};
    } else {
      rayD = {rd[i], rd[V.rayStride + i], rd[2 * V.rayStride + i]};
    }
  }
  const D3 pWorld = {px.rayO.x + rayD.x * depth, px.rayO.y + rayD.y * depth, px.rayO.z + rayD.z * depth};
  const size_t wPlane = warp_plane(V), cPlane = color_plane(V);
  const int wPitch = V.W + 2 * kPadW;
  unsigned mask = 0, waveMask = 0;
  cull = __builtin_amdgcn_readfirstlane(__ballot(!(depth >= kCullMinDepth)) != 0ull ? 0u : cull);
  const ushort4* colBase = V.projColor + (size_t)dl * (V.S - 1) * cPlane;
  const ushort4* biaBase = V.projBias + (size_t)dl * (V.S - 1) * cPlane;
  const size_t tPlane = tiled_plane(V.W, V.H);
  const ushort4* colTBase = RANDOM ? V.projColorT + (size_t)dl * (V.S - 1) * tPlane : nullptr;
  {
    bool pend = false;
    int pendSlot = 0;
    f4a8 pa = {0, 0, 0, 0}, pb = {0, 0, 0, 0};
    float pxw = 0, pyw = 0;
    auto consume = [&]() {
      const float w00 = (1 - pxw) * (1 - pyw), w01 = pxw * (1 - pyw), w10 = (1 - pxw) * pyw, w11 = pxw * pyw;
      const float wx = bilerp_f(pa.x, pa.z, pb.x, pb.z, w00, w01, w10, w11);
      const float wy = bilerp_f(pa.y, pa.w, pb.y, pb.w, w00, w01, w10, w11);
      const float xDstSrc = wx + 0.5f, yDstSrc = wy + 0.5f;
      const bool ok = pend && !(isnan(xDstSrc) || isnan(yDstSrc));
      if (ok) {
        pairs.set(pendSlot, SsdPair{xDstSrc, yDstSrc});
        mask |= 1u << pendSlot;
      }
      if (__ballot(ok) != 0ull) {
        waveMask |= 1u << pendSlot;
      }
    };
    for (int s = 0; s < V.S; ++s) {
      if (s == own || ((cull >> slot(s, own)) & 1u)) {
        continue;
      }
      const Cam& cs = V.camsSrc[s];
      D2 pn;
      const bool vis = sees<cost_sees_lean<RANDOM>()>(cs, pWorld, cs.principal[0], cs.principal[1], cs.focal[0], cs.focal[1],
                                                      1.0, 1.0, pn, pairs.atanLut);
      if (__ballot(pend) != 0ull) {
        consume();
      }
      pend = vis;
      pendSlot = slot(s, own);
      if (__ballot(vis) != 0ull) {
        const float sx = (float)(pn.x * V.Wd), sy = (float)(pn.y * V.Hd);
        const float xf = roundf(sx), yf = roundf(sy);
        const int xi = (int)xf, yi = (int)yf;
        pxw = sx - xf + 0.5f;
        pyw = sy - yf + 0.5f;
        const size_t tab = (size_t)dl * (V.S - 1) + pendSlot;
        const char* wbase = reinterpret_cast<const char*>(V.projWarp + tab * wPlane);
        const unsigned woff = vis ? ((unsigned)(yi - 1 + kPadW) * (unsigned)wPitch + (unsigned)(xi - 1 + kPadW)) * 8u : 0u;
        pa = *reinterpret_cast<const f4a8*>(wbase + woff);
        pb = *reinterpret_cast<const f4a8*>(wbase + (woff + (unsigned)wPitch * 8u));
      }
    }
    if (__ballot(pend) != 0ull) {
      consume();
    }
  }
  const unsigned tc1 = phase_clock();
  const int ssdCount = __popc(mask);
  nPair += ssdCount;
#ifdef DERP_COUNT_UNION
  if (slots) {
    *slots += __popc(__builtin_amdgcn_readfirstlane(waveMask));
  }
#endif
  int keep = 1;
  if (ssdCount < keep) {
    return make_float2(3.402823466e+38f, 0.0f);
  }
  {
    int cnt = 0;
    for (unsigned wm = __builtin_amdgcn_readfirstlane(waveMask); wm != 0; wm &= wm - 1) {
      const int t = __builtin_ctz(wm);
      if ((mask >> t) & 1) {
        const SsdPair e = pairs.get(t);
        const SsdPair ssd = compute_ssd<RANDOM>(V, px, colBase + (size_t)t * cPlane, biaBase + (size_t)t * cPlane, e.first,
                                                        e.second, RANDOM ? colTBase + (size_t)t * tPlane : nullptr);
        pairs.set(cnt, ssd);
        ++cnt;
      }
    }
  }
  const unsigned tc2 = phase_clock();
  keep = max(keep, ssdCount - 2);
  GccSelect<LdsPairs> sel(pairs);
  sel.nth_element(keep, ssdCount);
  float cost = 0;
  for (int i = 0; i < keep; ++i) {
    cost += pairs.get(i).second;
  }
  cost /= (float)keep;
  const float trustCoef = 1.0f / (float)keep;
  float confidence = px.confidence;
  if constexpr (RELOAD_RAY) {
    unsigned i = pix;
    asm("" : "+v"(i) : "v"(cost));
    if constexpr (RANDOM) {
      confidence = fmaxf(at32(V.srcVar + (size_t)own * ((size_t)V.W * V.H), i), kMinVar);
    } else {
      confidence = fmaxf((V.srcVar + (size_t)own * ((size_t)V.W * V.H))[i], kMinVar);
    }
  }
  const float costFinal = cost * trustCoef / confidence;
#if DERP_PHASE_TIMERS
  if (tm) {
    const unsigned tc3 = phase_clock();
    tm->proj += tc1 - tc0, tm->ssd += tc2 - tc1, tm->select += tc3 - tc2, tm->inside += tc3 - tc0;
  }
#endif
  return make_float2(costFinal, confidence);
}

template <bool WITH_RAY = true>
__device__ __forceinline__ void load_pixctx(const LevelView& V, int d, int own, int x, int y, const PatchWin* win, PixCtx& px,
                                            int tl = -1) {
  const Cam& cd = V.camsDst[d];
  px.rayO = {cd.pos[0], cd.pos[1], cd.pos[2]};
  const size_t n = (size_t)V.W * V.H;
  if constexpr (!WITH_RAY) {
    px.rayD = {0, 0, 0};
  } else {
    const size_t i = (size_t)d * n + (size_t)y * V.W + x;
    px.rayD = {V.rayDir[i], V.rayDir[V.rayStride + i], V.rayDir[2 * V.rayStride + i]};
  }
  if (tl < 0) {
    tl = (int)(threadIdx.x & 63);
  }
  const int corner = (tl >> 3) * kWinW + (tl & 7);
  px.winBG = win->bg + corner;
  px.winR = win->r + corner;
// ... 446 lines not shown
    for (int oy = oya; oy <= oyb; ++oy) {
      for (int ox = oxa; ox <= oxb; ++ox) {
        pc[(size_t)oy * OW + ox] = col;
        pb[(size_t)oy * OW + ox] = bia;
        if (pt) {
          pt[tiled_index(tilesX, ox, oy)] = col;
        }
      }
    }
  }
}

__device__ __forceinline__ float probe_disparity(int i, float minD, float maxD) {
  const double fraction = (double)i / (double)(kNumDepths - 1);
  return (float)(fraction * (double)minD + (1 - fraction) * (double)maxD);
}

__global__ void __launch_bounds__(kCostBlock, DERP_COST_MIN_WAVES)
    k_brute_costs(LevelView V, float* __restrict__ costs, float* __restrict__ confs, int tilesX, int tilesPerDst) {
  const int i = blockIdx.y;
  const int dl = blockIdx.z;
  const int d = V.dst0 + dl;
  const int iw = V.W - 2, ih = V.H - 2;
  const int lane = threadIdx.x & 63;
  const int sx = (int)(blockIdx.x % (unsigned)tilesX), sy = (int)(blockIdx.x / (unsigned)tilesX);
  const int x = 1 + sx * 8 + (lane & 7), y = 1 + sy * 8 + (lane >> 3);
  PatchWin* win;
  LdsPairs pairs = cost_wave_prologue(V, d, x - (int)(threadIdx.x & 7), y - (int)((threadIdx.x & 63) >> 3), win);
  unsigned nCost = 0, nPair = 0;
  if (x <= iw && y <= ih) {
    const int own = V.dst2src[d];
    const size_t n = (size_t)V.W * V.H, idx = (size_t)y * V.W + x;
    const float minDisparity = 1.0f / V.maxDepthM, maxDisparity = 1.0f / V.minDepthM;
    const float disparity = probe_disparity(i, minDisparity, maxDisparity);
    const bool fov = V.fovMask[(size_t)d * n + idx], fg = V.srcFg[(size_t)own * n + idx];
    const bool closer = V.hasFg ? (V.bgDisp[(size_t)d * n + idx] < disparity) : true;
    float2 r = make_float2(__builtin_nanf(""), __builtin_nanf(""));
    if (fov && fg && closer) {
      PixCtx px;
      load_pixctx(V, d, own, x, y, win, px);
      r = compute_cost(V, dl, own, px, disparity, pairs, nPair);
      ++nCost;
    }
    const size_t o = ((size_t)dl * kNumDepths + i) * n + idx;
    costs[o] = r.x;
    confs[o] = r.y;
  }
  flush_counters(V, nCost, nPair);
}

__global__ void k_brute_select(LevelView V, const float* __restrict__ costs, const float* __restrict__ confs) {
  const int dl = blockIdx.z;
  const int d = V.dst0 + dl;
  const int x = blockIdx.x * blockDim.x + threadIdx.x, y = blockIdx.y * blockDim.y + threadIdx.y;
  if (x < 1 || y < 1 || x >= V.W - 1 || y >= V.H - 1) {
    return;
  }
  const int own = V.dst2src[d];
  const size_t n = (size_t)V.W * V.H, idx = (size_t)y * V.W + x;
  float* disp = V.disparity + (size_t)d * n;
  if (!V.fovMask[(size_t)d * n + idx]) {
    disp[idx] = __builtin_nanf("");
    return;
  }
  if (!V.srcFg[(size_t)own * n + idx]) {
    disp[idx] = V.bgDisp[(size_t)d * n + idx];
    return;
  }
  float minCost = 3.402823466e+38f, minConf = 0;
  int best = -1;
  for (int i = 0; i < kNumDepths; ++i) {
    const size_t o = ((size_t)dl * kNumDepths + i) * n + idx;
    const float c = costs[o];
    if (c < minCost) {
      minCost = c;
      minConf = confs[o];
      best = i;
    }
  }
  const float minDisparity = 1.0f / V.maxDepthM, maxDisparity = 1.0f / V.minDepthM;
  if (best == -1) {
    atomicAdd(&V.counters[2], 1ull);
    disp[idx] = minDisparity;
  } else {
    disp[idx] = probe_disparity(best, minDisparity, maxDisparity);
  }
  V.cost[(size_t)d * n + idx] = minCost;
  V.confidence[(size_t)d * n + idx] = minConf;
}

__global__ void k_brute_margin(LevelView V) {
  const int d = V.dst0 + blockIdx.z;
  const int x = blockIdx.x * blockDim.x + threadIdx.x, y = blockIdx.y * blockDim.y + threadIdx.y;
  if (x >= V.W || y >= V.H) {
    return;
  }
  if (!(x < 1 || x >= V.W - 1 || y < 1 || y >= V.H - 1)) {
    return;
  }
  const int own = V.dst2src[d];
  const size_t n = (size_t)V.W * V.H, idx = (size_t)y * V.W + x;
  if (!V.srcFg[(size_t)own * n + idx]) {
    V.disparity[(size_t)d * n + idx] = V.bgDisp[(size_t)d * n + idx];
    return;
  }
  const int yy = min(max(y, 1), V.H - 2), xx = min(max(x, 1), V.W - 2);
  const size_t src = (size_t)yy * V.W + xx;
  V.disparity[(size_t)d * n + idx] = V.disparity[(size_t)d * n + src];
  V.cost[(size_t)d * n + idx] = V.cost[(size_t)d * n + src];
  V.confidence[(size_t)d * n + idx] = V.confidence[(size_t)d * n + src];
}

__device__ __forceinline__ bool random_gate(const LevelView& V, int d, int own, size_t idx) {
  const size_t n = (size_t)V.W * V.H;
  if (!V.fovMask[(size_t)d * n + idx] || !V.srcFg[(size_t)own * n + idx]) {
    return false;
  }
  const float varHighDev = 0.1f * V.varHighThresh;
  const float thresh = fmaxf(varHighDev, V.varNoiseFloor);
  return !(V.srcVar[(size_t)own * n + idx] < thresh);
}

__global__ void __launch_bounds__(256) k_row_rank(LevelView V, int* __restrict__ rank) {
  __shared__ int partial[256];
  const int d = V.dst0 + blockIdx.y, y = blockIdx.x + 1;
  const int own = V.dst2src[d];
  const size_t n = (size_t)V.W * V.H;
  const int inner = V.W - 2;
  const int per = (inner + 255) / 256;
  const int x0 = 1 + threadIdx.x * per, x1 = min(x0 + per, V.W - 1);
  int cnt = 0;
  for (int x = x0; x < x1; ++x) {
    cnt += random_gate(V, d, own, (size_t)y * V.W + x);
  }
  partial[threadIdx.x] = cnt;
  __syncthreads();
  for (int off = 1; off < 256; off <<= 1) {
    const int v = ((int)threadIdx.x >= off) ? partial[threadIdx.x - off] : 0;
    __syncthreads();
    partial[threadIdx.x] += v;
    __syncthreads();
  }
  const int run = partial[threadIdx.x] - cnt;
  uint32_t state = minstd_jump(minstd_seed(y * V.level), (uint64_t)V.randomProposals * (uint64_t)run);
  const uint32_t aP = minstd_jump(1u, (uint64_t)V.randomProposals);
  for (int x = x0; x < x1; ++x) {
    rank[(size_t)d * n + (size_t)y * V.W + x] = (int)state;
    if (random_gate(V, d, own, (size_t)y * V.W + x)) {
      state = minstd_mulmod(state, aP);
    }
  }
}

__device__ __forceinline__ void random_proposals_body(const LevelView& V, const int* __restrict__ rank, int tilesX, int tilesPerDst) {
  const int dl = blockIdx.y;
  const int d = V.dst0 + dl;
  int x, y;
  tile_pixel(xcd_swizzle(blockIdx.x, gridDim.x, V.xcdRotate ? d : 0), tilesX, x, y);
  PatchWin* win;
  LdsPairs pairs = cost_wave_prologue(V, d, x - (int)(threadIdx.x & 7), y - (int)((threadIdx.x & 63) >> 3), win);
  unsigned nCost = 0, nPair = 0, nSlots = 0, nSlotsFirst = 0;
  PhaseTimers tm;
  const unsigned tk0 = phase_clock();
  if (x >= 1 && y >= 1 && x < V.W - 1 && y < V.H - 1) {
    const int own = V.dst2src[d];
    const size_t n = (size_t)V.W * V.H;
    const unsigned idx = (unsigned)y * (unsigned)V.W + (unsigned)x;
    float* disp = V.disparity + (size_t)d * n;
    if ((V.fovMask + (size_t)d * n)[idx]) {
      if (!(V.srcFg + (size_t)own * n)[idx]) {
        disp[idx] = (V.bgDisp + (size_t)d * n)[idx];
      } else if (random_gate(V, d, own, idx)) {
        PixCtx px;
        load_pixctx<false>(V, d, own, x, y, win, px);
        const unsigned cull = behind_sources(V, d, idx);
        float currDisp = at32(disp, idx);
        float currCost = 0.f, costThresh = 0.f, amplitude = 0.f;
        const int spare = V.S - 1;
        const float maxDisp = 1.0f / V.minDepthM;
        uint32_t state = (uint32_t)at32(rank + (size_t)d * n, idx);
        for (int i = -1; i < V.randomProposals; ++i) {
          unsigned pi = idx;
          asm("" : "+v"(pi) : "s"(i));
          const float minDisp = V.hasFg ? at32(V.bgDisp + (size_t)d * n, pi) : (1.0f / V.maxDepthM);
          float propDisp = currDisp;
          if (i >= 0) {
            const float lo = fmaxf(minDisp, currDisp - amplitude), hi = fminf(maxDisp, currDisp + amplitude);
            propDisp = minstd_uniform(state, lo, hi);
          }
          unsigned np = 0;
          const float2 pr = compute_cost<true, true>(V, dl, own, px, propDisp, pairs, np, cull, pi, i < 0 ? &nSlotsFirst : &nSlots, &tm);
          nPair += np;
          bool take;
          if (i < 0) {
            costThresh = fminf(0.5f * pr.x, 5.0f);
            amplitude = (maxDisp - minDisp) / 2.0f;
            take = true;
          } else {
            take = pr.x < currCost && pr.x < costThresh;
            if (take) {
              amplitude /= 2.0f;
            }
          }
          if (take) {
            currCost = pr.x;
            currDisp = propDisp;
            pairs.set(spare, SsdPair{pr.y, __uint_as_float(np)});
          }
        }
        {
          unsigned pi = idx;
          asm("" : "+v"(pi) : "v"(currCost));
          const SsdPair best = pairs.get(spare);
          at32(V.confidence + (size_t)d * n, pi) = best.first;
          at32(V.pairCount + (size_t)d * n, pi) = (uint8_t)__float_as_uint(best.second);
          at32(disp, pi) = currDisp;
          at32(V.cost + (size_t)d * n, pi) = currCost;
        }
        nCost = 1u + (unsigned)max(V.randomProposals, 0);
      }
    }
  }
#if DERP_PHASE_TIMERS
  if ((threadIdx.x & 63) == 0) {
    const unsigned body = phase_clock() - tk0;
    atomicAdd(&V.counters[0], (unsigned long long)(DERP_PHASE_TIMERS == 1 ? tm.proj : body));
    atomicAdd(&V.counters[1], (unsigned long long)(DERP_PHASE_TIMERS == 1 ? tm.ssd : body - tm.inside));
    atomicAdd(&V.counters[3], (unsigned long long)(DERP_PHASE_TIMERS == 1 ? tm.select : 0u));
  }
  return;
#endif
  flush_counters(V, nCost, nPair);
#ifdef DERP_COUNT_UNION
  atomicAdd(&V.counters[3], (unsigned long long)nSlots);
  atomicAdd(&V.counters[2], (unsigned long long)nSlotsFirst);
#endif
}

__global__ void __launch_bounds__(kCostBlock, DERP_RANDOM_MIN_WAVES)
    k_random_proposals(LevelView V, const int* __restrict__ rank, int tilesX, int tilesPerDst) {
  random_proposals_body(V, rank, tilesX, tilesPerDst);
}
__global__ void __launch_bounds__(kCostBlock, 3)
    k_random_proposals_w3(LevelView V, const int* __restrict__ rank, int tilesX, int tilesPerDst) {
  random_proposals_body(V, rank, tilesX, tilesPerDst);
}

__constant__ int kCandidates[9][2] = {{0, 0}, {-1, 0}, {1, 0}, {0, -1}, {0, 1}, {-2, -2}, {2, -2}, {-2, 2}, {2, 2}};
constexpr int kCandOff[9][2] = {{0, 0}, {-1, 0}, {1, 0}, {0, -1}, {0, 1}, {-2, -2}, {2, -2}, {-2, 2}, {2, 2}};
constexpr unsigned cand_pack(int c) {
  unsigned p = 0;
  for (int k = 0; k < 9; ++k) {
    p |= (unsigned)(kCandOff[k][c] + 2) << (3 * k);
  }
  return p;
}
constexpr unsigned kCandPackX = cand_pack(0), kCandPackY = cand_pack(1);

#ifdef DERP_COUNT_PP_FILL
__device__ __forceinline__ unsigned pp_fill_entry() {
  return __builtin_ctzll(__ballot(1)) == (int)(threadIdx.x & 63) ? 64u : 0u;
}
#endif

__device__ __forceinline__ void ping_pong_candidates_loop(const LevelView& V, const uint8_t* __restrict__ changed, int dl, int x,
                                                          int y, const PatchWin* win, LdsPairs& pairs, int useMemo, float& outDisp,
                                                          float& outCost, unsigned& counts, unsigned& fillSlots, PhaseTimers& tm) {
  const int d = V.dst0 + dl;
  const int own = V.dst2src[d];
  const size_t n = (size_t)V.W * V.H;
  const unsigned idx = (unsigned)y * (unsigned)V.W + (unsigned)x;
  const float* disp = V.disparity + (size_t)d * n;
  const uint8_t* fov = V.fovMask + (size_t)d * n;
  const uint8_t* chg = changed + (size_t)d * n;
  outDisp = disp[idx];
  const bool interior = x >= 1 && y >= 1 && x < V.W - 1 && y < V.H - 1;
  if (interior && fov[idx]) {
    if (!V.srcFg[(size_t)own * n + idx]) {
      outDisp = V.bgDisp[(size_t)d * n + idx];
    } else if (!(V.srcVar[(size_t)own * n + idx] < V.varNoiseFloor)) {
      PixCtx px;
      load_pixctx<false>(V, d, own, x, y, win, px);
      const unsigned cull = behind_sources(V, d, idx);
      float bestCost = __builtin_inff();
      float bestDisp = outDisp;
      const unsigned xy = (unsigned)x | ((unsigned)y << 16);
      for (int k = 0; k < 9; ++k) {
        unsigned q = xy;
        asm("" : "+v"(q) : "s"(k));
        const int px0 = (int)(q & 0xffffu), py0 = (int)(q >> 16);
        const unsigned pidx = (unsigned)py0 * (unsigned)V.W + (unsigned)px0;
        const int xx = min(max(px0 + kCandidates[k][0], 0), V.W - 1);
        const int yy = min(max(py0 + kCandidates[k][1], 0), V.H - 1);
        const unsigned j = (unsigned)yy * (unsigned)V.W + (unsigned)xx;
        if (fov[j]) {
          const float cand = disp[j];
          const float bg = V.hasFg ? (V.bgDisp + (size_t)d * n)[pidx] : 0.f;
          if (cand >= bg && chg[j]) {
            float2 r;
            const float memoConf = (k == 0 && useMemo) ? (V.confidence + (size_t)d * n)[pidx] : 0.0f;
            if (memoConf != 0.0f) {
              r = make_float2((V.cost + (size_t)d * n)[pidx], memoConf);
              counts += (unsigned)(V.pairCount + (size_t)d * n)[pidx] + (1u << 24);
            } else {
              unsigned np = 0;
#ifdef DERP_COUNT_PP_FILL
              fillSlots += pp_fill_entry();
#endif
              r = compute_cost<false, true>(V, dl, own, px, cand, pairs, np, cull, pidx, nullptr, &tm);
              counts += np;
            }
            counts += 1u << 16;
            if (r.x < bestCost) {
              bestCost = r.x;
              bestDisp = cand;
            }
          }
        }
      }
      outDisp = bestDisp;
      outCost = bestCost;
    }
  }
}

__device__ __forceinline__ void ping_pong_candidates_compact(const LevelView& V, const uint8_t* __restrict__ changed, int dl, int& x,
                                                             int& y, const PatchWin* win, LdsPairs& pairs, int useMemo, float& outDisp,
                                                             float& outCost, unsigned& counts, unsigned& fillSlots, PhaseTimers& tm) {
  const int d = V.dst0 + dl;
  const int own = V.dst2src[d];
  const size_t n = (size_t)V.W * V.H;
  const int lane = (int)(threadIdx.x & 63);
  const float* disp = V.disparity + (size_t)d * n;
  const uint8_t* fov = V.fovMask + (size_t)d * n;
  const uint8_t* chg = changed + (size_t)d * n;
  unsigned cmask = 0;
  bool eval = false;
  const unsigned idx = (unsigned)y * (unsigned)V.W + (unsigned)x;
  if (x < V.W && y < V.H) {
    outDisp = disp[idx];
    const bool interior = x >= 1 && y >= 1 && x < V.W - 1 && y < V.H - 1;
    if (interior && fov[idx]) {
      if (!V.srcFg[(size_t)own * n + idx]) {
        outDisp = V.bgDisp[(size_t)d * n + idx];
      } else if (!(V.srcVar[(size_t)own * n + idx] < V.varNoiseFloor)) {
        eval = true;
        const float bg = V.hasFg ? (V.bgDisp + (size_t)d * n)[idx] : 0.f;
        for (int k = 0; k < 9; ++k) {
          const int xx = min(max(x + (int)((kCandPackX >> (3 * k)) & 7u) - 2, 0), V.W - 1);
          const int yy = min(max(y + (int)((kCandPackY >> (3 * k)) & 7u) - 2, 0), V.H - 1);
          const unsigned j = (unsigned)yy * (unsigned)V.W + (unsigned)xx;
          if (fov[j]) {
            const float cand = disp[j];
            if (cand >= bg && chg[j]) {
              const float memoConf = (k == 0 && useMemo) ? (V.confidence + (size_t)d * n)[idx] : 0.0f;
              if (memoConf != 0.0f) {
                const float c = (V.cost + (size_t)d * n)[idx];
                counts += (unsigned)(V.pairCount + (size_t)d * n)[idx] + (1u << 24) + (1u << 16);
                if (c < outCost) {
                  outCost = c;
                  outDisp = cand;
                }
              } else {
                cmask |= 1u << k;
              }
            }
          }
        }
      }
    }
  }
  unsigned cull = 0;
  const unsigned behind = eval ? V.behind[(size_t)d * n + idx] : ~0u;
  for (int t = 0; t < V.S - 1; ++t) {
    if (__ballot(!((behind >> t) & 1u)) == 0ull) {
      cull |= 1u << t;
    }
  }
  cull = __builtin_amdgcn_readfirstlane(cull);
  int incl = __popc(cmask);
  for (int off = 1; off < 64; off <<= 1) {
    const int v = __builtin_amdgcn_ds_bpermute((lane - off) << 2, incl);
    if (lane >= off) {
      incl += v;
    }
  }
  const int total = __builtin_amdgcn_readlane(incl, 63);
  const unsigned list = cmask | ((unsigned)incl << 16);
  const int x0 = __builtin_amdgcn_readfirstlane(x - (lane & 7)), y0 = __builtin_amdgcn_readfirstlane(y - (lane >> 3));
  extern __shared__ SsdPair ldsPairs[];
  SsdPair* const wavePairs = ldsPairs + (__builtin_amdgcn_readfirstlane(threadIdx.x) & ~63u);
  SsdPair* const stage = wavePairs + (size_t)(V.S - 1) * pairs.stride;
  for (int base = 0; base < total; base += 64) {
    int ln = lane;
    asm("" : "+v"(ln) : "s"(base));
    const int t = base + ln;
    int o = 0;
    for (int step = 32; step > 0; step >>= 1) {
      if ((int)((unsigned)__builtin_amdgcn_ds_bpermute((o + step - 1) << 2, (int)list) >> 16) <= t) {
        o += step;
      }
    }
    o = min(o, 63);
    const unsigned ol = (unsigned)__builtin_amdgcn_ds_bpermute(o << 2, (int)list);
    unsigned m = ol & 0xffffu;
    const int oStart = (int)(ol >> 16) - __popc(m);
#ifdef DERP_COUNT_PP_FILL
    fillSlots += ln == 0 ? 64u : 0u;
#endif
    if (t < total) {
      for (int r = t - oStart; r > 0; --r) {
        m &= m - 1;
      }
      const int k = __builtin_ctz(m);
      const int ox = x0 + (o & 7), oy = y0 + (o >> 3);
      const unsigned pidx = (unsigned)oy * (unsigned)V.W + (unsigned)ox;
      const int xx = min(max(ox + (int)((kCandPackX >> (3 * k)) & 7u) - 2, 0), V.W - 1);
      const int yy = min(max(oy + (int)((kCandPackY >> (3 * k)) & 7u) - 2, 0), V.H - 1);
      const float cand = disp[(unsigned)yy * (unsigned)V.W + (unsigned)xx];
      PixCtx px;
      load_pixctx<false>(V, d, own, ox, oy, win, px, o);
      LdsPairs lp{wavePairs + ln, pairs.stride, pairs.atanLut};
      unsigned np = 0;
      const float2 r = compute_cost<false, true>(V, dl, own, px, cand, lp, np, cull, pidx, nullptr, &tm);
      counts += np + (1u << 16);
      int sl = lane;
      asm("" : "+v"(sl) : "v"(r.x));
      stage[sl] = SsdPair{r.x, cand};
    }
    __builtin_amdgcn_fence(__ATOMIC_SEQ_CST, "wavefront");
    __builtin_amdgcn_wave_barrier();
    const int end = (int)(list >> 16);
    const int lo = max(end - __popc(list & 0xffffu), base), hi = min(end, base + 64);
    for (int i = lo; i < hi; ++i) {
      const SsdPair e = stage[i - base];
      if (e.first < outCost) {
        outCost = e.first;
        outDisp = e.second;
      }
    }
    __builtin_amdgcn_fence(__ATOMIC_SEQ_CST, "wavefront");
    __builtin_amdgcn_wave_barrier();
  }
  x = x0 + (lane & 7);
  y = y0 + (lane >> 3);
}

template <bool COMPACT>
__device__ __forceinline__ void ping_pong_body(const LevelView& V, const uint8_t* __restrict__ changed, float* __restrict__ dispRes,
                                               float* __restrict__ costRes, int tilesX, int useMemo) {
  const int dl = blockIdx.y;
  const int d = V.dst0 + dl;
  int x, y;
  tile_pixel(xcd_swizzle(blockIdx.x, gridDim.x, V.xcdRotate ? d : 0), tilesX, x, y);
  PatchWin* win;
  LdsPairs pairs = cost_wave_prologue(V, d, x - (int)(threadIdx.x & 7), y - (int)((threadIdx.x & 63) >> 3), win);
  unsigned counts = 0, fillSlots = 0;
  PhaseTimers tm;
  const unsigned tk0 = phase_clock();
  float outDisp = 0.f;
  float outCost = __builtin_inff();
  if constexpr (COMPACT) {
    ping_pong_candidates_compact(V, changed, dl, x, y, win, pairs, useMemo, outDisp, outCost, counts, fillSlots, tm);
  } else if (x < V.W && y < V.H) {
    ping_pong_candidates_loop(V, changed, dl, x, y, win, pairs, useMemo, outDisp, outCost, counts, fillSlots, tm);
  }
  if (x < V.W && y < V.H) {
    const size_t n = (size_t)V.W * V.H;
    const unsigned idx = (unsigned)y * (unsigned)V.W + (unsigned)x;
    (dispRes + (size_t)d * n)[idx] = outDisp;
    (costRes + (size_t)d * n)[idx] = outCost;
  }
#if DERP_PHASE_TIMERS
  if ((threadIdx.x & 63) == 0) {
    const unsigned body = phase_clock() - tk0;
    atomicAdd(&V.counters[0], (unsigned long long)(DERP_PHASE_TIMERS == 1 ? tm.proj : body));
    atomicAdd(&V.counters[1], (unsigned long long)(DERP_PHASE_TIMERS == 1 ? tm.ssd : body - tm.inside));
    atomicAdd(&V.counters[3], (unsigned long long)(DERP_PHASE_TIMERS == 1 ? tm.select : 0u));
  }
  return;
#endif
  unsigned nMemo = counts >> 24;
#ifdef DERP_COUNT_PP_FILL
  flush_counters(V, (counts >> 16) & 0xffu, fillSlots);
#else
  (void)fillSlots;
  flush_counters(V, (counts >> 16) & 0xffu, counts & 0xffffu);
#endif
  for (int off = 32; off > 0; off >>= 1) {
    nMemo += __shfl_down(nMemo, off);
  }
  if ((threadIdx.x & 63) == 0 && nMemo) {
    atomicAdd(&V.counters[3], (unsigned long long)nMemo);
  }
}

__global__ void __launch_bounds__(kCostBlock, DERP_COST_MIN_WAVES)
    k_ping_pong(LevelView V, const uint8_t* __restrict__ changed, float* __restrict__ dispRes,
                float* __restrict__ costRes, int tilesX, int useMemo) {
  ping_pong_body<true>(V, changed, dispRes, costRes, tilesX, useMemo);
}
__global__ void __launch_bounds__(kCostBlock, 3)
    k_ping_pong_w3(LevelView V, const uint8_t* __restrict__ changed, float* __restrict__ dispRes,
                   float* __restrict__ costRes, int tilesX, int useMemo) {
  ping_pong_body<true>(V, changed, dispRes, costRes, tilesX, useMemo);
}
__global__ void __launch_bounds__(kCostBlock, DERP_COST_MIN_WAVES)
    k_ping_pong_loop(LevelView V, const uint8_t* __restrict__ changed, float* __restrict__ dispRes,
                     float* __restrict__ costRes, int tilesX, int useMemo) {
  ping_pong_body<false>(V, changed, dispRes, costRes, tilesX, useMemo);
}
__global__ void __launch_bounds__(kCostBlock, 3)
    k_ping_pong_loop_w3(LevelView V, const uint8_t* __restrict__ changed, float* __restrict__ dispRes,
                        float* __restrict__ costRes, int tilesX, int useMemo) {
  ping_pong_body<false>(V, changed, dispRes, costRes, tilesX, useMemo);
}

__global__ void k_ping_pong_commit(float* __restrict__ disp, float* __restrict__ cost, const float* __restrict__ dispRes,
                                   const float* __restrict__ costRes, uint8_t* __restrict__ changed, size_t n) {
  size_t i = (size_t)blockIdx.x * blockDim.x + threadIdx.x;
  const size_t step = (size_t)gridDim.x * blockDim.x;
  for (; i < n; i += step) {
    const float a = disp[i], b = dispRes[i];
    changed[i] = (a != b);
    disp[i] = b;
    cost[i] = costRes[i];
  }
}

__device__ __forceinline__ float clamp_fetch(const float* img, int x, int y, int W, int H) {
  return img[(size_t)min(max(y, 0), H - 1) * W + min(max(x, 0), W - 1)];
}

__global__ void __launch_bounds__(256)
    k_mismatch(LevelView V, float* __restrict__ newDisp, uint8_t* __restrict__ mismatchMask) {
  extern __shared__ float ldsMis[];
  const int d = blockIdx.z;
  const int x = blockIdx.x * 16 + (threadIdx.x & 15), y = blockIdx.y * 16 + (threadIdx.x >> 4);
  if (x >= V.W || y >= V.H) {
    return;
  }
  const size_t n = (size_t)V.W * V.H, idx = (size_t)y * V.W + x;
  if (!V.fovMask[(size_t)d * n + idx]) {
    newDisp[(size_t)d * n + idx] = __builtin_nanf("");
    return;
  }
  float* mis = ldsMis + threadIdx.x;
  const int own = V.dst2src[d];
  const float curr = V.disparity[(size_t)d * n + idx];
  int nMatch = 0, nMis = 0;
  if (V.srcFg[(size_t)own * n + idx]) {
    const Cam& cd = V.camsDst[d];
    const D3 dir = rig_direction(cd, (x + 0.5) / (double)V.W, (y + 0.5) / (double)V.H, cd.principal[0], cd.principal[1],
                                 cd.focal[0], cd.focal[1]);
    const double depth = (double)(1.0f / curr);
    const D3 pWorld = {cd.pos[0] + dir.x * depth, cd.pos[1] + dir.y * depth, cd.pos[2] + dir.z * depth};
    const float dMin = (1.0f - 0.1f) * curr, dMax = (1.0f + 0.1f) * curr;
    for (int s = 0; s < V.S; ++s) {
      if (s == own) {
        continue;
      }
      const Cam& cs = V.camsSrc[s];
      D2 pn;
      if (!sees(cs, pWorld, cs.principal[0], cs.principal[1], cs.focal[0], cs.focal[1], 1.0, 1.0, pn)) {
        continue;
      }
      const float sx = (float)(pn.x * (double)V.W), sy = (float)(pn.y * (double)V.H);
      const float xf = roundf(sx), yf = roundf(sy);
      const int xi = (int)xf, yi = (int)yf;
      const float xw = sx - xf + 0.5f, yw = sy - yf + 0.5f;
      const float* img = V.disparity + (size_t)s * n;
      const float dSrc = bilerp_f(clamp_fetch(img, xi - 1, yi - 1, V.W, V.H), clamp_fetch(img, xi, yi - 1, V.W, V.H),
                                  clamp_fetch(img, xi - 1, yi, V.W, V.H), clamp_fetch(img, xi, yi, V.W, V.H),
                                  (1 - xw) * (1 - yw), xw * (1 - yw), (1 - xw) * yw, xw * yw);
      if (dMin <= dSrc && dSrc <= dMax) {
        ++nMatch;
      } else {
        mis[(nMis++) * 256] = dSrc;
      }
    }
  }
  bool mask = false;
  float dispNew = curr;
  if (nMatch + nMis != 0) {
    const float var = V.srcVar[(size_t)own * n + idx];
    if (!(nMatch >= 1 || V.varHighThresh < var || var < V.varNoiseFloor)) {
      mask = true;
      for (int i = 1; i < nMis; ++i) {
        const float v = mis[i * 256];
        int k = i;
        while (k > 0 && mis[(k - 1) * 256] > v) {
          mis[k * 256] = mis[(k - 1) * 256];
          --k;
        }
        mis[k * 256] = v;
      }
      int closer = 0;
      for (; closer < nMis; ++closer) {
        if (mis[closer * 256] >= curr) {
          break;
        }
      }
      const float m = mis[(closer / 2) * 256];
      dispNew = (m < curr) ? m : curr;
    }
  }
  mismatchMask[(size_t)d * n + idx] = mask;
  newDisp[(size_t)d * n + idx] = dispNew;
}

__global__ void k_layer_disparities(const float* __restrict__ fg, const float* __restrict__ bg, size_t n,
                                    uint8_t* __restrict__ out) {
  size_t i = (size_t)blockIdx.x * blockDim.x + threadIdx.x;
  const size_t step = (size_t)gridDim.x * blockDim.x;
  for (; i < n; i += step) {
    const float m = fg[i] > 0.0f ? 1.0f : 0.0f;
    const float layer = fg[i] * m + bg[i] * (1 - m);
    const int r = cv_round(layer * 255.0f);
    out[i] = (uint8_t)min(max(r, 0), 255);
  }
}

__global__ void __launch_bounds__(kCostBlock, DERP_COST_MIN_WAVES)
    k_cost_map(LevelView V, int d, const float* __restrict__ dispIn, float* __restrict__ costOut,
               float* __restrict__ confOut, int tilesX) {
  const int dl = d - V.dst0;
  int x, y;
  tile_pixel(blockIdx.x, tilesX, x, y);
  PatchWin* win;
  LdsPairs pairs = cost_wave_prologue(V, d, x - (int)(threadIdx.x & 7), y - (int)((threadIdx.x & 63) >> 3), win);
  unsigned nCost = 0, nPair = 0;
  if (x >= 1 && y >= 1 && x < V.W - 1 && y < V.H - 1) {
    const int own = V.dst2src[d];
    PixCtx px;
    load_pixctx(V, d, own, x, y, win, px);
    const float2 r = compute_cost(V, dl, own, px, dispIn[(size_t)y * V.W + x], pairs, nPair);
    ++nCost;
    costOut[(size_t)y * V.W + x] = r.x;
    confOut[(size_t)y * V.W + x] = r.y;
  }
  flush_counters(V, nCost, nPair);
}

__constant__ unsigned long long kExp2fTab[32] = {
    0x3ff0000000000000ull, 0x3fefd9b0d3158574ull, 0x3fefb5586cf9890full, 0x3fef9301d0125b51ull,
    0x3fef72b83c7d517bull, 0x3fef54873168b9aaull, 0x3fef387a6e756238ull, 0x3fef1e9df51fdee1ull,
    0x3fef06fe0a31b715ull, 0x3feef1a7373aa9cbull, 0x3feedea64c123422ull, 0x3feece086061892dull,
    0x3feebfdad5362a27ull, 0x3feeb42b569d4f82ull, 0x3feeab07dd485429ull, 0x3feea47eb03a5585ull,
    0x3feea09e667f3bcdull, 0x3fee9f75e8ec5f74ull, 0x3feea11473eb0187ull, 0x3feea589994cce13ull,
    0x3feeace5422aa0dbull, 0x3feeb737b0cdc5e5ull, 0x3feec49182a3f090ull, 0x3feed503b23e255dull,
    0x3feee89f995ad3adull, 0x3feeff76f2fb5e47ull, 0x3fef199bdd85529cull, 0x3fef3720dcef9069ull,
    0x3fef5818dcfba487ull, 0x3fef7c97337b9b5full, 0x3fefa4afa2a490daull, 0x3fefd0765b6e4540ull};

__device__ __forceinline__ float div_by_const(float y, double rcp) {
  return (float)((double)y * rcp);
}

__device__ __forceinline__ float div_int_by_const(int y, double rcp) {
  return (float)((double)y * rcp);
}

__device__ __forceinline__ float expf_glibc(float x, const unsigned long long* tab) {
  const double InvLn2N = 0x1.71547652b82fep+0 * 32;
  const double C0 = 0x1.c6af84b912394p-5 / 32 / 32 / 32, C1 = 0x1.ebfce50fac4f3p-3 / 32 / 32,
               C2 = 0x1.62e42ff0c52d6p-1 / 32;
  const double SHIFT = 0x1.8p+52;
  const unsigned abstop = (__float_as_uint(x) >> 20) & 0x7ff;
  if (abstop >= (0x42b00000u >> 20)) {
    if (__float_as_uint(x) == 0xff800000u) {
// ... 1228 lines not shown
```

### facebook360_dep_amd/derp.py

```python
import ctypes as C
import os

import numpy as np

_HERE = os.path.dirname(os.path.abspath(__file__))
LIB_PATH = os.environ.get("DERP_LIB") or os.path.join(_HERE, "libderp_hip.so")
CAM_TYPES = {"FTHETA": 0, "RECTILINEAR": 1, "EQUISOLID": 2, "ORTHOGRAPHIC": 3}

STAGES = ["fov_mask", "variance", "own_bias", "upsample", "proj_warp", "reproject", "proj_bias", "brute_force",
          "random_proposals", "ping_pong", "mismatches", "bilateral", "median", "mask_fov", "temporal"]


class SeqOptions(C.Structure):
    _fields_ = [
        ("time_radius", C.c_int32), ("sigma", C.c_float), ("weight_b", C.c_float), ("weight_g", C.c_float),
        ("weight_r", C.c_float), ("space_radius", C.c_int32), ("use_foreground_masks", C.c_int32),
        ("partition", C.c_int32), ("do_temporal_filter", C.c_int32), ("resident_frames", C.c_int32),
    ]


class SeqTransfer(C.Structure):
    _fields_ = [("frame", C.c_int32), ("from_rank", C.c_int32), ("to_rank", C.c_int32)]


class CameraDesc(C.Structure):
    _fields_ = [
        ("type", C.c_int32), ("has_principal", C.c_int32), ("has_distortion", C.c_int32), ("has_fov", C.c_int32),
        ("origin", C.c_double * 3), ("forward", C.c_double * 3), ("up", C.c_double * 3), ("right", C.c_double * 3),
        ("resolution", C.c_double * 2), ("focal", C.c_double * 2), ("principal", C.c_double * 2),
        ("distortion", C.c_double * 3), ("fov", C.c_double), ("id", C.c_char * 64),
    ]


class Options(C.Structure):
    _fields_ = [
        ("min_depth_m", C.c_float), ("max_depth_m", C.c_float), ("var_noise_floor", C.c_float),
        ("var_high_thresh", C.c_float), ("random_proposals", C.c_int32), ("ping_pong_iterations", C.c_int32),
        ("mismatches_start_level", C.c_int32), ("do_bilateral_filter", C.c_int32), ("do_median_filter", C.c_int32),
        ("use_foreground_masks", C.c_int32), ("partial_coverage", C.c_int32), ("rebuild_warp_tables", C.c_int32),
    ]


class MeshPass(C.Structure):
    _fields_ = [("faces", C.c_longlong), ("feasible", C.c_longlong), ("winners", C.c_longlong), ("applied", C.c_longlong),
                ("deleted", C.c_longlong), ("threshold", C.c_double)]


class RenderParams(C.Structure):
    _fields_ = [
        ("kind", C.c_int32), ("width", C.c_int32), ("height", C.c_int32), ("position", C.c_double * 3),
        ("forward", C.c_double * 3), ("up", C.c_double * 3), ("horizontal_fov", C.c_double), ("ipd", C.c_float),
        ("alpha_blend", C.c_int32), ("disparity_color", C.c_int32), ("weight", C.c_int32), ("zero_nans", C.c_int32),
    ]


RENDER_KINDS = {"cube": 0, "equirect": 1, "snapshot": 2}
WEIGHTS = {"svd": 0, "minor": 1}
FORMATS = ["cubecolor", "cubedisp", "eqrcolor", "eqrdisp", "lr180", "snapcolor", "snapdisp", "tb3dof", "tbstereo"]


def render_params(kind="equirect", width=3072, height=None, position=(0, 0, 0), forward=(-1, 0, 0), up=(0, 0, 1),
                  horizontal_fov=90.0, ipd=0.0, alpha_blend=True, disparity_color=False, weight="svd", zero_nans=False):
    p = RenderParams()
    lib().derp_render_params_default(C.byref(p))
    p.kind = RENDER_KINDS[kind]
    p.width = width
    p.height = width // 2 if height is None else height
    for k, v in (("position", position), ("forward", forward), ("up", up)):
        for i in range(3):
            getattr(p, k)[i] = float(v[i])
    p.horizontal_fov = horizontal_fov
    p.ipd = ipd
    p.alpha_blend = int(bool(alpha_blend))
    p.disparity_color = int(bool(disparity_color))
    p.weight = WEIGHTS[weight]
    p.zero_nans = int(bool(zero_nans))
    return p


def render_format_size(fmt, width, height):
    w, h = C.c_int(), C.c_int()
    if lib().derp_render_format_size(fmt.encode(), width, height, C.byref(w), C.byref(h)):
        raise ValueError("Invalid format: %s" % fmt)
    return w.value, h.value


EXPORTS = [
    "derp_options_default", "derp_create", "derp_destroy", "derp_last_error", "derp_set_options", "derp_set_pyramid",
    "derp_build_pyramid_color", "derp_build_pyramid_foreground_mask", "derp_build_pyramid_background_disparity",
    "derp_download_level_color", "derp_download_level_mask", "derp_download_level_background", "derp_resize_area",
    "derp_generate_foreground_mask", "derp_image_info", "derp_image_decode", "derp_image_last_error", "derp_jpeg_encode",
    "derp_upload_color", "derp_upload_foreground_mask", "derp_upload_background_disparity", "derp_upload_disparity",
    "derp_process_level", "derp_process_pyramid", "derp_synchronize", "derp_download_disparity", "derp_download_cost",
    "derp_level_begin", "derp_stage_reproject_colors", "derp_stage_brute_force", "derp_stage_random_proposals",
    "derp_stage_ping_pong", "derp_stage_mismatches", "derp_stage_bilateral_filter", "derp_stage_median_filter", "derp_stage_mask_fov",
    "derp_level_end", "derp_set_level_disparity", "derp_get_level_disparity", "derp_cost_map", "derp_debug_download",
    "derp_debug_atan2_ypos", "derp_debug_fp64", "derp_debug_sees",
    "derp_ssim", "derp_average_score", "derp_rephotograph", "derp_rephotograph_upload", "derp_rephotograph_render", "derp_canopy_cubemap",
    "derp_render_params_default", "derp_render_upload", "derp_render", "derp_render_format_size", "derp_render_format",
    "derp_render_vertices",
    "derp_export_points", "derp_points_begin", "derp_points_splat", "derp_points_download", "derp_project_equirect_mask",
    "derp_mesh_build", "derp_mesh_counts", "derp_mesh_setup", "derp_mesh_simplify", "derp_mesh_download_f64", "derp_mesh_download",
    "derp_mesh_simplify_parallel", "derp_mesh_parallel_pass",
    "derp_mesh_setup_host", "derp_mesh_simplify_host",
    "derp_fov_mask", "derp_layer_disparities", "derp_download_mismatch_mask", "derp_upsample_disparity", "derp_joint_bilateral_u16", "derp_joint_bilateral_f32", "derp_masked_median",
    "derp_temporal_filter", "derp_temporal_filter_dev", "derp_dev_disparity", "derp_dev_color", "derp_dev_mask",
    "derp_get_counters", "derp_reset_counters", "derp_profile_enable", "derp_profile_reset", "derp_profile_query", "derp_profile_memoised",
    "derp_device_name", "derp_device_memory", "derp_host_nth_element_pairs", "derp_host_minstd_uniform",
    "derp_set_frame_slots", "derp_select_frame", "derp_frame_slots", "derp_host_alloc", "derp_host_free", "derp_bind_thread", "derp_host_register", "derp_host_unregister",
    "derp_seq_options_default", "derp_seq_window", "derp_seq_owner", "derp_seq_plan", "derp_seq_create", "derp_seq_destroy",
    "derp_seq_counts", "derp_seq_frames", "derp_seq_frame_slot", "derp_seq_buffer", "derp_rccl_unique_id",
    "derp_seq_attach_rccl", "derp_seq_attach_loopback", "derp_seq_attach_external", "derp_seq_selftest",
    "derp_seq_exchange_inputs", "derp_seq_level_compute", "derp_seq_level_exchange", "derp_seq_level_filter",
    "derp_seq_host_inputs", "derp_seq_buffer_copy", "derp_seq_upload_color_plane", "derp_seq_upload_disparity", "derp_seq_download_disparity", "derp_seq_exchange_inputs_level",
    "derp_seq_level_compute_frame", "derp_seq_level_provided_frame", "derp_seq_mark_exchanged", "derp_seq_level_filter_frame", "derp_seq_download_filtered",
    "derp_seq_run", "derp_seq_stats", "derp_seq_stats_reset", "derp_seq_exchange_exposed_ms",
    "derp_isp_config_default", "derp_isp_create", "derp_isp_destroy", "derp_isp_output_size", "derp_isp_process",
    "derp_isp_stage", "derp_isp_tables",
    "derp_sim_scene_create", "derp_sim_scene_destroy", "derp_sim_scene_icosahedrons", "derp_sim_scene_cubes",
    "derp_sim_scene_ground_plane", "derp_sim_scene_add_triangle", "derp_sim_bvh_build", "derp_sim_scene_counts",
    "derp_sim_scene_get", "derp_sim_perlin_table", "derp_sim_icosahedron", "derp_sim_noise", "derp_sim_trace_host", "derp_sim_create",
    "derp_sim_destroy", "derp_sim_upload", "derp_sim_render_camera", "derp_sim_render_equirect", "derp_sim_trace_rays",
    "derp_sim_stage_size", "derp_sim_stage",
]

_lib = None


def lib():
    global _lib
    if _lib is None:
        if not os.path.exists(LIB_PATH):
            raise RuntimeError(
                "libderp_hip.so is missing: build it with `python -c 'import __graft_entry__ as g; g.build()'` "
                "(hipcc --offload-arch=gfx950). There is no CPU fallback for the depth path."
            )
        try:
            import torch
        except ImportError:
            pass
        _lib = C.CDLL(LIB_PATH)
        _lib.derp_last_error.restype = C.c_char_p
        _lib.derp_last_error.argtypes = [C.c_void_p]
        _lib.derp_host_minstd_uniform.restype = C.c_float
        _lib.derp_host_minstd_uniform.argtypes = [C.c_int, C.c_uint64, C.c_float, C.c_float]
        _lib.derp_sim_scene_create.restype = C.c_void_p
        _lib.derp_sim_scene_destroy.argtypes = [C.c_void_p]
        _lib.derp_sim_scene_destroy.restype = None
    return _lib


def camera_desc(cam):
    j = CameraDesc()
    j.type = CAM_TYPES[cam["type"]]
    for k in ("origin", "forward", "up", "right", "resolution", "focal"):
        for i, v in enumerate(cam[k]):
            getattr(j, k)[i] = float(v)
    j.has_principal = int("principal" in cam)
    if "principal" in cam:
        j.principal[0], j.principal[1] = map(float, cam["principal"])
    j.has_distortion = int("distortion" in cam)
    if "distortion" in cam:
        d = list(cam["distortion"]) + [0.0] * (3 - len(cam["distortion"]))
        for i in range(3):
            j.distortion[i] = float(d[i])
    j.has_fov = int("fov" in cam)
    if "fov" in cam:
        j.fov = float(cam["fov"])
    j.id = cam["id"].encode()
    return j


def filter_destinations(cams, destinations):
    if not destinations:
        return list(cams)
    out = []
    for dest in destinations.split(","):
        for cam in cams:
            if cam["id"] == dest:
                out.append(cam)
    return out


def _p(a):
    return a.ctypes.data_as(C.c_void_p) if a is not None else None


class DerpError(RuntimeError):
    pass


class Derp:

    def __init__(self, cams_src, cams_dst=None, device=0, **options):
        cams_dst = cams_src if cams_dst is None else cams_dst
        self.cams_src, self.cams_dst = list(cams_src), list(cams_dst)
        self.S, self.D = len(self.cams_src), len(self.cams_dst)
        a = (CameraDesc * self.S)(*[camera_desc(c) for c in self.cams_src])
        b = (CameraDesc * self.D)(*[camera_desc(c) for c in self.cams_dst])
        h = C.c_void_p()
        if lib().derp_create(C.byref(h), device, a, self.S, b, self.D):
            raise DerpError(lib().derp_last_error(None).decode())
        self.h = h
        self._seqs = []
        self.sizes = None
        self.opt = Options()
        lib().derp_options_default(C.byref(self.opt))
        self.set_options(**options)

    def close(self):
        if getattr(self, "h", None):
            for ref in list(getattr(self, "_seqs", [])):
                seq = ref()
                if seq is not None:
                    seq.close()
            lib().derp_destroy(self.h)
            self.h = None

    def __del__(self):
        try:
            self.close()
        except Exception:
            pass

    def _ck(self, rc):
        if rc:
            raise DerpError(lib().derp_last_error(self.h).decode())

    def set_options(self, **kw):
        for k, v in kw.items():
            if not hasattr(self.opt, k):
                raise KeyError(k)
            setattr(self.opt, k, type(getattr(self.opt, k))(v))
        self._ck(lib().derp_set_options(self.h, C.byref(self.opt)))

    def set_pyramid(self, sizes, width_full, height_full):
        self.sizes = list(sizes)
        w = (C.c_int * len(sizes))(*[s[0] for s in sizes])
        h = (C.c_int * len(sizes))(*[s[1] for s in sizes])
        self._ck(lib().derp_set_pyramid(self.h, len(sizes), w, h, width_full, height_full))

    def _shape(self, level):
        w, h = self.sizes[level]
        return h, w

    def upload_color(self, level, s, bgr):
        bgr = np.ascontiguousarray(bgr, dtype=np.uint16)
        assert bgr.shape == self._shape(level) + (3,)
        self._ck(lib().derp_upload_color(self.h, level, s, _p(bgr)))

    def upload_foreground_mask(self, level, s, mask):
        mask = np.ascontiguousarray(mask, dtype=np.uint8)
        assert mask.shape == self._shape(level)
        self._ck(lib().derp_upload_foreground_mask(self.h, level, s, _p(mask)))

    def upload_background_disparity(self, level, d, disp):
        disp = np.ascontiguousarray(disp, dtype=np.float32)
        assert disp.shape == self._shape(level)
        self._ck(lib().derp_upload_background_disparity(self.h, level, d, _p(disp)))

    def upload_disparity(self, level, d, disp):
# ... 289 lines not shown
        return self.mesh_counts()

    def mesh_counts(self):
        nv, nf, raw = C.c_size_t(), C.c_size_t(), C.c_size_t()
        self._ck(lib().derp_mesh_counts(self.h, C.byref(nv), C.byref(nf), C.byref(raw)))
        return nv.value, nf.value, raw.value

    def mesh_setup(self, equi_error=True):
        nv, nf, _ = self.mesh_counts()
        planes, costs, vq = np.zeros((nf, 4)), np.zeros((nf, 3)), np.zeros((nv, 10))
        self._ck(lib().derp_mesh_setup(self.h, int(equi_error), _p(planes), _p(costs), _p(vq)))
        return planes, costs, vq

    def mesh_simplify(self, num_faces_out, strictness=0.2, remove_boundary_edges=False, equi_error=True, host_setup=False):
        stats = (C.c_int * 2)()
        self._ck(lib().derp_mesh_simplify(self.h, num_faces_out, C.c_float(strictness), int(remove_boundary_edges),
                                          int(equi_error), int(host_setup), stats))
        return stats[0], stats[1]

    def mesh_simplify_parallel(self, num_faces_out, strictness=0.2, remove_boundary_edges=False, equi_error=True):
        stats = (C.c_int * 2)()
        self._ck(lib().derp_mesh_simplify_parallel(self.h, num_faces_out, C.c_float(strictness), int(remove_boundary_edges),
                                                   int(equi_error), stats))
        return stats[0], stats[1]

    def mesh_parallel_pass(self, index):
        p = MeshPass()
        self._ck(lib().derp_mesh_parallel_pass(self.h, index, C.byref(p)))
        return p.faces, p.feasible, p.winners, p.applied, p.deleted, p.threshold

    def mesh_download_f64(self):
        nv, nf, _ = self.mesh_counts()
        v, f = np.zeros((nv, 3)), np.zeros((nf, 3), dtype=np.int32)
        self._ck(lib().derp_mesh_download_f64(self.h, _p(v), _p(f)))
        return v, f

    def mesh_download(self, clamp_negative_z=False):
        nv, nf, _ = self.mesh_counts()
        v, f = np.zeros((nv, 3), dtype=np.float32), np.zeros((nf, 3), dtype=np.uint32)
        self._ck(lib().derp_mesh_download(self.h, int(clamp_negative_z), _p(v), _p(f)))
        return v, f

    def fov_mask(self, d, w, h):
        out = np.zeros((h, w), dtype=np.uint8)
        self._ck(lib().derp_fov_mask(self.h, d, w, h, _p(out)))
        return out

    def upsample_disparity(self, d, disp, w_up, h_up, bg_up=None, fg=None, fg_up=None):
        disp = np.ascontiguousarray(disp, dtype=np.float32)
        h, w = disp.shape
        use = fg is not None
        out = np.zeros((h_up, w_up), dtype=np.float32)
        if use:
            bg_up = np.ascontiguousarray(bg_up, dtype=np.float32)
            fg = np.ascontiguousarray(fg, dtype=np.uint8)
            fg_up = np.ascontiguousarray(fg_up, dtype=np.uint8)
        self._ck(lib().derp_upsample_disparity(self.h, d, _p(disp), w, h, _p(bg_up) if use else None,
                                               _p(fg) if use else None, _p(fg_up) if use else None, w_up, h_up,
                                               int(use), _p(out)))
        return out

    def joint_bilateral_u16(self, image, guide, mask, radius, sigma, w0, w1, w2):
        image = np.ascontiguousarray(image, dtype=np.float32)
        guide = np.ascontiguousarray(guide, dtype=np.uint16)
        mask = np.ascontiguousarray(mask, dtype=np.uint8)
        h, w = image.shape
        out = np.zeros_like(image)
        self._ck(lib().derp_joint_bilateral_u16(self.h, _p(image), _p(guide), _p(mask), w, h, radius, C.c_float(sigma),
                                                C.c_float(w0), C.c_float(w1), C.c_float(w2), _p(out)))
        return out

    def joint_bilateral_f32(self, image, guide, mask, radius, sigma, w0, w1, w2):
        image = np.ascontiguousarray(image, dtype=np.float32)
        guide = np.ascontiguousarray(guide, dtype=np.float32)
        mask = np.ascontiguousarray(mask, dtype=np.uint8)
        h, w = image.shape
        out = np.zeros_like(image)
        self._ck(lib().derp_joint_bilateral_f32(self.h, _p(image), _p(guide), _p(mask), w, h, radius, C.c_float(sigma),
                                                C.c_float(w0), C.c_float(w1), C.c_float(w2), _p(out)))
        return out

    def masked_median(self, image, background, mask, radius=1):
        image = np.ascontiguousarray(image, dtype=np.float32)
        background = None if background is None else np.ascontiguousarray(background, dtype=np.float32)
        mask = np.ascontiguousarray(mask, dtype=np.uint8)
        h, w = image.shape
        out = np.zeros_like(image)
        self._ck(lib().derp_masked_median(self.h, _p(image), _p(background), _p(mask), w, h, radius, _p(out)))
        return out

    def temporal_filter(self, guides, images, masks, frame_offset, sigma, radius, w0, w1, w2):
        n = len(guides)
        guides = [np.ascontiguousarray(g, dtype=np.uint16) for g in guides]
        images = [np.ascontiguousarray(g, dtype=np.float32) for g in images]
        masks = [np.ascontiguousarray(g, dtype=np.uint8) for g in masks]
        h, w = images[0].shape
        gp = (C.c_void_p * n)(*[g.ctypes.data for g in guides])
        ip = (C.c_void_p * n)(*[g.ctypes.data for g in images])
        mp = (C.c_void_p * n)(*[g.ctypes.data for g in masks])
        out = np.zeros((h, w), dtype=np.float32)
        self._ck(lib().derp_temporal_filter(self.h, gp, ip, mp, n, w, h, frame_offset, C.c_float(sigma), radius,
                                            C.c_float(w0), C.c_float(w1), C.c_float(w2), _p(out)))
        return out

    def temporal_filter_dev(self, guide_ptrs, disp_ptrs, mask_ptrs, w, h, frame_offset, sigma, radius, w0, w1, w2,
                            out_ptr):
        n = len(guide_ptrs)
        gp = (C.c_void_p * n)(*guide_ptrs)
        ip = (C.c_void_p * n)(*disp_ptrs)
        mp = (C.c_void_p * n)(*mask_ptrs)
        self._ck(lib().derp_temporal_filter_dev(self.h, gp, ip, mp, n, w, h, frame_offset, C.c_float(sigma), radius,
                                                C.c_float(w0), C.c_float(w1), C.c_float(w2), C.c_void_p(out_ptr)))

    def dev_disparity(self, level, d):
        p, n = C.c_void_p(), C.c_size_t()
        self._ck(lib().derp_dev_disparity(self.h, level, d, C.byref(p), C.byref(n)))
        return p.value, n.value

    def dev_color(self, level, s):
        p, n = C.c_void_p(), C.c_size_t()
        self._ck(lib().derp_dev_color(self.h, level, s, C.byref(p), C.byref(n)))
        return p.value, n.value

    def dev_mask(self, level, d):
        p, n = C.c_void_p(), C.c_size_t()
        self._ck(lib().derp_dev_mask(self.h, level, d, C.byref(p), C.byref(n)))
        return p.value, n.value

    def counters(self):
        a, b, i = C.c_uint64(), C.c_uint64(), C.c_uint64()
        self._ck(lib().derp_get_counters(self.h, C.byref(a), C.byref(b), C.byref(i)))
        return dict(n_cost=a.value, n_pair=b.value, insufficient=i.value)

    def reset_counters(self):
        self._ck(lib().derp_reset_counters(self.h))

    def profile_enable(self, on=True):
        self._ck(lib().derp_profile_enable(self.h, int(on)))

    def profile_reset(self):
        self._ck(lib().derp_profile_reset(self.h))

    def profile_query(self, stage, level=-1):
        ms, n = C.c_double(), C.c_int()
        a, b = C.c_uint64(), C.c_uint64()
        self._ck(lib().derp_profile_query(self.h, stage.encode(), level, C.byref(ms), C.byref(n), C.byref(a), C.byref(b)))
        return dict(ms=ms.value, launches=n.value, n_cost=a.value, n_pair=b.value)

    def profile_memoised(self, stage, level=-1):
        m = C.c_uint64()
        self._ck(lib().derp_profile_memoised(self.h, stage.encode(), level, C.byref(m)))
        return m.value

    def device_memory(self):
        f, t = C.c_uint64(), C.c_uint64()
        self._ck(lib().derp_device_memory(self.h, C.byref(f), C.byref(t)))
        return f.value, t.value

    def device_name(self):
        buf = C.create_string_buffer(256)
        self._ck(lib().derp_device_name(self.h, buf, 256))
        return buf.value.decode()


MESH_EXIT_BUDGET, MESH_EXIT_INFINITE_THRESHOLD, MESH_EXIT_STUCK = 0, 1, 2


def mesh_setup_host(vertices, faces, equi_error=True):
    v = np.ascontiguousarray(vertices, dtype=np.float64).reshape(-1, 3)
    f = np.ascontiguousarray(faces, dtype=np.int32).reshape(-1, 3)
    planes, costs, vq = np.zeros((len(f), 4)), np.zeros((len(f), 3)), np.zeros((len(v), 10))
    if lib().derp_mesh_setup_host(_p(v), C.c_size_t(len(v)), _p(f), C.c_size_t(len(f)), int(equi_error), _p(planes),
                                  _p(costs), _p(vq)):
        raise DerpError("derp_mesh_setup_host: bad arguments")
    return planes, costs, vq


def mesh_simplify_host(vertices, faces, num_faces_out, strictness=0.2, remove_boundary_edges=False, equi_error=True,
                       setup=None):
    v = np.ascontiguousarray(vertices, dtype=np.float64).reshape(-1, 3)
    f = np.ascontiguousarray(faces, dtype=np.int32).reshape(-1, 3)
    planes, costs, vq = (None, None, None) if setup is None else [np.ascontiguousarray(a, dtype=np.float64) for a in setup]
    ov, of = np.zeros_like(v), np.zeros_like(f)
    nv, nf = C.c_size_t(), C.c_size_t()
    stats = (C.c_int * 2)()
    if lib().derp_mesh_simplify_host(_p(v), C.c_size_t(len(v)), _p(f), C.c_size_t(len(f)), _p(planes), _p(costs), _p(vq),
                                     num_faces_out, C.c_float(strictness), int(remove_boundary_edges), int(equi_error),
                                     _p(ov), _p(of), C.byref(nv), C.byref(nf), stats):
        raise DerpError("derp_mesh_simplify_host: bad arguments")
    return ov[:nv.value].copy(), of[:nf.value].copy(), (stats[0], stats[1])


def host_nth_element_pairs(pairs, nth):
    p = np.ascontiguousarray(pairs, dtype=np.float32).copy()
    lib().derp_host_nth_element_pairs(_p(p), len(p), nth)
    return p


def host_minstd_uniform(seed, draw_index, a, b):
    return lib().derp_host_minstd_uniform(seed, draw_index, C.c_float(a), C.c_float(b))


def average_score(score, mask):
    score = np.ascontiguousarray(score, dtype=np.float32)
    mask = np.ascontiguousarray(mask, dtype=np.uint8)
    h, w = mask.shape
    out = (C.c_double * 3)()
    if lib().derp_average_score(_p(score), _p(mask), w, h, out):
        raise DerpError("derp_average_score: bad arguments")
    return [out[0], out[1], out[2]]


def format_results(avg):
    return "R %.2f%%, G %.2f%%, B %.2f%%" % (100 * avg[2], 100 * avg[1], 100 * avg[0])


ISP_MAX_ROLLOFF = 16
ISP_FILTERS = {"bilinear": 0, "frequency": 1, "edge_aware": 2, "chroma_suppressed_bilinear": 3}
ISP_STAGES = ["load", "pixel", "stuck", "demosaic", "color", "lowpass", "sharpened"]


class IspConfig(C.Structure):
    _fields_ = [
        ("bits_per_pixel", C.c_int32), ("width", C.c_int32), ("height", C.c_int32), ("is_little_endian", C.c_int32),
        ("is_row_major", C.c_int32), ("bayer_pattern", C.c_char * 8), ("plane_order", C.c_char * 8),
        ("black_level", C.c_float * 3), ("clamp_min", C.c_float * 3), ("clamp_max", C.c_float * 3),
        ("stuck_pixel_threshold", C.c_int32), ("stuck_pixel_darkness_threshold", C.c_float),
        ("stuck_pixel_radius", C.c_int32), ("n_rolloff_h", C.c_int32), ("n_rolloff_v", C.c_int32),
        ("rolloff_h", (C.c_float * 3) * ISP_MAX_ROLLOFF), ("rolloff_v", (C.c_float * 3) * ISP_MAX_ROLLOFF),
        ("white_balance_gain", C.c_float * 3), ("ccm", C.c_float * 9), ("saturation", C.c_float), ("gamma", C.c_float * 3),
        ("low_key_boost", C.c_float * 3), ("high_key_boost", C.c_float * 3), ("contrast", C.c_float),
        ("sharpening", C.c_float * 3), ("sharpening_support", C.c_float), ("noise_core", C.c_float),
        ("n_companding_lut", C.c_int32),
    ]


def isp_config(config):
    k = IspConfig()
    lib().derp_isp_config_default(C.byref(k))
    j = config.get("CameraIsp", config) if config else {}
    for key, field in (("bitsPerPixel", "bits_per_pixel"), ("width", "width"), ("height", "height"),
                       ("stuckPixelThreshold", "stuck_pixel_threshold"), ("stuckPixelRadius", "stuck_pixel_radius")):
        if key in j:
            setattr(k, field, int(j[key]))
    for key, field in (("isLittleEndian", "is_little_endian"), ("isRowMajor", "is_row_major")):
        if key in j:
            setattr(k, field, int(bool(j[key])))
    for key, field in (("bayerPattern", "bayer_pattern"), ("planeOrder", "plane_order")):
        if key in j:
            setattr(k, field, j[key].upper().encode())
    for key, field in (("stuckPixelDarknessThreshold", "stuck_pixel_darkness_threshold"), ("saturation", "saturation"),
                       ("contrast", "contrast"), ("sharpeningSupport", "sharpening_support"), ("noiseCore", "noise_core")):
        if key in j:
            setattr(k, field, float(j[key]))
    for key, field in (("blackLevel", "black_level"), ("clampMin", "clamp_min"), ("clampMax", "clamp_max"),
                       ("whiteBalanceGain", "white_balance_gain"), ("gamma", "gamma"), ("lowKeyBoost", "low_key_boost"),
                       ("highKeyBoost", "high_key_boost"), ("sharpening", "sharpening")):
        if j.get(key) is not None:
            for i in range(3):
                getattr(k, field)[i] = float(j[key][i])
    for key, field, count in (("vignetteRollOffH", "rolloff_h", "n_rolloff_h"), ("vignetteRollOffV", "rolloff_v", "n_rolloff_v")):
        if j.get(key) is not None:
            if len(j[key]) > ISP_MAX_ROLLOFF:
                raise DerpError("%s holds more than %d points" % (key, ISP_MAX_ROLLOFF))
            setattr(k, count, len(j[key]))
            for n, p in enumerate(j[key]):
                for i in range(3):
                    getattr(k, field)[n][i] = float(p[i])
    if j.get("ccm") is not None:
        for r in range(3):
            for c in range(3):
                k.ccm[3 * r + c] = float(j["ccm"][r][c])
    if j.get("compandingLut") is not None:
        k.n_companding_lut = len(j["compandingLut"])
    return k


class Isp:

    def __init__(self, config, demosaic_filter=0, pow2_downscale=1, apply_tone_curve=True, device=0):
        self.cfg = config if isinstance(config, IspConfig) else isp_config(config)
        h = C.c_void_p()
        if lib().derp_isp_create(C.byref(h), device, C.byref(self.cfg), int(demosaic_filter), int(pow2_downscale),
                                 int(bool(apply_tone_curve))):
            raise DerpError(lib().derp_last_error(None).decode())
        self.h = h
        w, hh = C.c_int(), C.c_int()
        self._ck(lib().derp_isp_output_size(self.h, C.byref(w), C.byref(hh)))
        self.width, self.height = w.value, hh.value
        self.dtype = np.uint8 if self.cfg.bits_per_pixel == 8 else np.uint16

    def _ck(self, rc):
        if rc:
            raise DerpError(lib().derp_last_error(None).decode())

    def close(self):
        if getattr(self, "h", None):
            lib().derp_isp_destroy(self.h)
            self.h = None

    def __del__(self):
        try:
            self.close()
        except Exception:
            pass

    def process(self, raw):
        buf = np.frombuffer(raw, dtype=np.uint8) if isinstance(raw, (bytes, bytearray)) else np.ascontiguousarray(raw).view(np.uint8).reshape(-1)
        out = np.zeros((self.height, self.width, 3), self.dtype)
        self._ck(lib().derp_isp_process(self.h, _p(buf), C.c_size_t(buf.size), _p(out)))
        return out

    def stage(self, stage):
        s = ISP_STAGES.index(stage) if isinstance(stage, str) else int(stage)
        out = np.zeros((self.height, self.width) if s < 3 else (3, self.height, self.width), np.float32)
        self._ck(lib().derp_isp_stage(self.h, s, _p(out)))
        return out

    def tables(self):
        vh, vv = np.zeros((self.width, 3), np.float32), np.zeros((self.height, 3), np.float32)
        ccm, lut = np.zeros((3, 3), np.float32), np.zeros((4096, 3), np.float32)
        self._ck(lib().derp_isp_tables(self.h, _p(vh), _p(vv), _p(ccm), _p(lut)))
        return vh, vv, ccm, lut


SIM_TRIANGLE = np.dtype([("v0", "<f4", 3), ("v1", "<f4", 3), ("v2", "<f4", 3), ("e1", "<f4", 3), ("e2", "<f4", 3),
                         ("normal", "<f4", 3), ("color", "<f4", 3)])
SIM_NODE = np.dtype([("center", "<f4", 3), ("radius", "<f4"), ("skip", "<i4"), ("first", "<i4"), ("count", "<i4"),
                     ("n_children", "<i4")])
SIM_STAGES = {"origin": (0, np.float32, 3), "direction": (1, np.float32, 3), "hit": (2, np.int32, 1),
              "distance": (3, np.float32, 1), "color": (4, np.float32, 3)}


class SimParams(C.Structure):
    _fields_ = [("ceiling_position", C.c_double), ("ceiling_width", C.c_double), ("ceiling_depth", C.c_double),
                ("marble_scale", C.c_double), ("marble", C.c_int32), ("pad", C.c_int32)]


class SimScene:

    def __init__(self):
        self.h = C.c_void_p(lib().derp_sim_scene_create())

    def close(self):
        if self.h:
            lib().derp_sim_scene_destroy(self.h)
            self.h = None

    def __del__(self):
        self.close()

    @staticmethod
    def _ck(rc):
# ... 115 lines not shown
```

### include/derp_hip.h

```cpp
#ifndef DERP_HIP_H
#define DERP_HIP_H

#include <stddef.h>
#include <stdint.h>

#ifdef __cplusplus
extern "C" {
#endif

typedef struct derp_ctx derp_ctx;

enum { DERP_FTHETA = 0, DERP_RECTILINEAR = 1, DERP_EQUISOLID = 2, DERP_ORTHOGRAPHIC = 3 };

typedef struct {
  int32_t type;
  int32_t has_principal;
  int32_t has_distortion;
  int32_t has_fov;
  double origin[3];
  double forward[3];
  double up[3];
  double right[3];
  double resolution[2];
  double focal[2];
  double principal[2];
  double distortion[3];
  double fov;
  char id[64];
} derp_camera_desc;

typedef struct {
  float min_depth_m;
  float max_depth_m;
  float var_noise_floor;
  float var_high_thresh;
  int32_t random_proposals;
  int32_t ping_pong_iterations;
  int32_t mismatches_start_level;
  int32_t do_bilateral_filter;
  int32_t do_median_filter;
  int32_t use_foreground_masks;
  int32_t partial_coverage;
  int32_t rebuild_warp_tables;
} derp_options;

void derp_options_default(derp_options* o);

int derp_create(derp_ctx** out, int device, const derp_camera_desc* src, int n_src,
                const derp_camera_desc* dst, int n_dst);
void derp_destroy(derp_ctx* ctx);
const char* derp_last_error(const derp_ctx* ctx);
int derp_set_options(derp_ctx* ctx, const derp_options* o);

int derp_set_pyramid(derp_ctx* ctx, int num_levels, const int* widths, const int* heights,
                     int width_full, int height_full);

int derp_set_frame_slots(derp_ctx* ctx, int n_slots);
int derp_select_frame(derp_ctx* ctx, int slot);
int derp_frame_slots(const derp_ctx* ctx, int* n_slots, int* selected);

void* derp_host_alloc(size_t bytes);
void derp_host_free(void* p);
int derp_bind_thread(derp_ctx* ctx);
int derp_host_register(void* p, size_t bytes);
void derp_host_unregister(void* p);

int derp_upload_color(derp_ctx* ctx, int level, int src, const uint16_t* bgr);
int derp_upload_foreground_mask(derp_ctx* ctx, int level, int src, const uint8_t* mask);
int derp_upload_background_disparity(derp_ctx* ctx, int level, int dst, const float* disp);
int derp_upload_disparity(derp_ctx* ctx, int level, int dst, const float* disp);

int derp_build_pyramid_color(derp_ctx* ctx, int src, const uint16_t* bgr, int w, int h);
int derp_build_pyramid_foreground_mask(derp_ctx* ctx, int src, const uint8_t* mask, int w, int h,
                                       int threshold);
int derp_build_pyramid_background_disparity(derp_ctx* ctx, int dst, const float* disp, int w, int h);
int derp_download_level_color(derp_ctx* ctx, int level, int src, uint16_t* bgr);
int derp_download_level_mask(derp_ctx* ctx, int level, int src, uint8_t* mask01);
int derp_download_level_background(derp_ctx* ctx, int level, int dst, float* disp);
int derp_image_info(const void* bytes, size_t n, int* w, int* h, int* channels, int* bitdepth);
int derp_image_decode(const void* bytes, size_t n, void* out, size_t out_bytes);
const char* derp_image_last_error(void);
int derp_jpeg_encode(const void* pixels, int w, int h, int channels, int quality, void* out, size_t cap, size_t* size);

int derp_resize_area(derp_ctx* ctx, int kind, const void* src, int w, int h, void* dst, int dw, int dh);

int derp_generate_foreground_mask(derp_ctx* ctx, const uint16_t* template_bgr, const uint16_t* frame_bgr,
                                  int w, int h, int blur_radius, float threshold,
                                  int morph_closing_size, uint8_t* mask01);

int derp_process_level(derp_ctx* ctx, int level);
int derp_process_pyramid(derp_ctx* ctx, int level_start, int level_end);
int derp_synchronize(derp_ctx* ctx);

int derp_download_disparity(derp_ctx* ctx, int level, int dst, float* disparity);
int derp_download_cost(derp_ctx* ctx, int dst, float* cost, float* confidence);

int derp_level_begin(derp_ctx* ctx, int level);
int derp_stage_reproject_colors(derp_ctx* ctx);
int derp_stage_brute_force(derp_ctx* ctx);
int derp_stage_random_proposals(derp_ctx* ctx);
int derp_stage_ping_pong(derp_ctx* ctx);
int derp_stage_mismatches(derp_ctx* ctx);
int derp_stage_bilateral_filter(derp_ctx* ctx);
int derp_stage_median_filter(derp_ctx* ctx);
int derp_stage_mask_fov(derp_ctx* ctx);
int derp_level_end(derp_ctx* ctx);
int derp_set_level_disparity(derp_ctx* ctx, int dst, const float* disp);
int derp_get_level_disparity(derp_ctx* ctx, int dst, float* disp);
int derp_cost_map(derp_ctx* ctx, int dst, const float* disp, float* cost, float* confidence);
int derp_debug_download(derp_ctx* ctx, int dst, int src, int which, void* out);
int derp_debug_atan2_ypos(derp_ctx* ctx, const double* y, const double* x, double* out, size_t n);
int derp_debug_fp64(derp_ctx* ctx, int op, const double* a, const double* b, double* out, size_t n);
int derp_debug_sees(derp_ctx* ctx, int src, const double* xyz, size_t n, double* out);

int derp_download_mismatch_mask(derp_ctx* ctx, int dst, uint8_t* out);

int derp_layer_disparities(derp_ctx* ctx, const float* foreground, const float* background, size_t n,
                           uint8_t* out);
int derp_ssim(derp_ctx* ctx, const float* x_bgr, const float* y_bgr, int w, int h, int blur_radius, float alpha,
              float beta, float gamma, float* score_bgr);
int derp_average_score(const float* score_bgr, const uint8_t* mask, int w, int h, double* avg_bgr3);
int derp_rephotograph(derp_ctx* ctx, int target, const uint16_t* const* colors, const float* const* disparities,
                      int w, int h, float* out_bgra);
int derp_rephotograph_upload(derp_ctx* ctx, const uint16_t* const* colors, const float* const* disparities, int w,
                             int h);
int derp_rephotograph_render(derp_ctx* ctx, int target, float* out_bgra);
int derp_canopy_cubemap(derp_ctx* ctx, const uint8_t* include, const double* centre, int edge, float* out_bgra);
enum { DERP_RENDER_CUBE = 0, DERP_RENDER_EQUIRECT = 1, DERP_RENDER_SNAPSHOT = 2 };
enum { DERP_WEIGHT_SVD = 0, DERP_WEIGHT_MINOR = 1 };
typedef struct {
  int32_t kind;
  int32_t width, height;
  double position[3];
  double forward[3], up[3];
  double horizontal_fov;
  float ipd;
  int32_t alpha_blend;
  int32_t disparity_color;
  int32_t weight;
  int32_t zero_nans;
} derp_render_params;
void derp_render_params_default(derp_render_params* p);
int derp_render_upload(derp_ctx* ctx, const float* const* colors_bgra, const int* color_w, const int* color_h,
                       const float* const* disparities, const int* disp_w, const int* disp_h);
int derp_render(derp_ctx* ctx, const derp_render_params* p, const uint8_t* include, float* out_bgra);
int derp_render_format_size(const char* format, int width, int height, int* out_w, int* out_h);
int derp_render_format(derp_ctx* ctx, const char* format, const derp_render_params* p, const float* background,
                       const float* background_equirect, int eq_w, int eq_h, float* out_bgra);
int derp_render_vertices(derp_ctx* ctx, int cam, float ipd, float* out_xyzw);
int derp_export_points(derp_ctx* ctx, int cam, const float* disparity, int w, int h, const float* color_bgr,
                       double max_depth, int clip, int subsample, float* out_xyzrgb, size_t cap, size_t* count);
int derp_points_begin(derp_ctx* ctx, const int* widths, const int* heights);
int derp_points_splat(derp_ctx* ctx, const double* xyz, size_t n, double min_depth, double max_depth);
int derp_points_download(derp_ctx* ctx, int cam, float* disparity);
int derp_project_equirect_mask(derp_ctx* ctx, int cam, const uint8_t* eqr, int eqr_w, int eqr_h, int w, int h,
                               double depth, uint8_t* out);
enum {
  DERP_MESH_EXIT_BUDGET = 0,
  DERP_MESH_EXIT_INFINITE_THRESHOLD = 1,
  DERP_MESH_EXIT_STUCK = 2,
  DERP_MESH_EXIT_NO_CANDIDATES = 3
};
typedef struct derp_mesh_pass {
  long long faces;
  long long feasible;
  long long winners;
  long long applied;
  long long deleted;
  double threshold;
} derp_mesh_pass;
int derp_mesh_build(derp_ctx* ctx, int cam, const float* disparity, int w, int h, const double* resolution,
                    double depth_scale, const uint8_t* mask, int mask_w, int mask_h, float tear_ratio);
int derp_mesh_counts(derp_ctx* ctx, size_t* vertices, size_t* faces, size_t* faces_unmasked);
int derp_mesh_setup(derp_ctx* ctx, int equi_error, double* face_planes, double* edge_costs, double* vertex_quadrics);
int derp_mesh_simplify(derp_ctx* ctx, int num_faces_out, float strictness, int remove_boundary_edges, int equi_error,
                       int host_setup, int* stats);
int derp_mesh_simplify_parallel(derp_ctx* ctx, int num_faces_out, float strictness, int remove_boundary_edges,
                                int equi_error, int* stats);
int derp_mesh_parallel_pass(derp_ctx* ctx, int pass, derp_mesh_pass* out);
int derp_mesh_download_f64(derp_ctx* ctx, double* vertices, int32_t* faces);
int derp_mesh_download(derp_ctx* ctx, int clamp_negative_z, float* vtx, uint32_t* idx);
int derp_mesh_setup_host(const double* vertices, size_t nv, const int32_t* faces, size_t nf, int equi_error,
                         double* face_planes, double* edge_costs, double* vertex_quadrics);
int derp_mesh_simplify_host(const double* vertices, size_t nv, const int32_t* faces, size_t nf, const double* face_planes,
                            const double* edge_costs, const double* vertex_quadrics, int num_faces_out, float strictness,
                            int remove_boundary_edges, int equi_error, double* out_vertices, int32_t* out_faces,
                            size_t* out_nv, size_t* out_nf, int* stats);
int derp_fov_mask(derp_ctx* ctx, int dst, int w, int h, uint8_t* out);
int derp_upsample_disparity(derp_ctx* ctx, int dst, const float* disp, int w, int h,
                            const float* bg_disp_up, const uint8_t* fg_mask,
                            const uint8_t* fg_mask_up, int w_up, int h_up,
                            int use_foreground_masks, float* out);
int derp_joint_bilateral_u16(derp_ctx* ctx, const float* image, const uint16_t* guide_bgr,
                             const uint8_t* mask, int w, int h, int radius, float sigma,
                             float weight0, float weight1, float weight2, float* out);
int derp_joint_bilateral_f32(derp_ctx* ctx, const float* image, const float* guide_bgr,
                             const uint8_t* mask, int w, int h, int radius, float sigma,
                             float weight0, float weight1, float weight2, float* out);
int derp_masked_median(derp_ctx* ctx, const float* image, const float* background,
                       const uint8_t* mask, int w, int h, int radius, float* out);
int derp_temporal_filter(derp_ctx* ctx, const uint16_t* const* guides_bgr,
                         const float* const* disparities, const uint8_t* const* masks, int n_frames,
                         int w, int h, int frame_offset, float sigma, int space_radius,
                         float weight0, float weight1, float weight2, float* out);
int derp_temporal_filter_dev(derp_ctx* ctx, const void* const* guides_bgrx_dev,
                             const float* const* disparities_dev, const uint8_t* const* masks_dev,
                             int n_frames, int w, int h, int frame_offset, float sigma,
                             int space_radius, float weight0, float weight1, float weight2,
                             float* out_dev);
int derp_dev_disparity(derp_ctx* ctx, int level, int dst, float** ptr, size_t* bytes);
int derp_dev_color(derp_ctx* ctx, int level, int src, void** ptr_bgrx_u16, size_t* bytes);
int derp_dev_mask(derp_ctx* ctx, int level, int dst, uint8_t** ptr_fov_and_fg, size_t* bytes);

typedef struct derp_seq derp_seq;
enum { DERP_SEQ_BLOCK = 0, DERP_SEQ_CYCLIC = 1 };
typedef struct {
  int32_t time_radius;
  float sigma;
  float weight_b;
  float weight_g;
  float weight_r;
  int32_t space_radius;
  int32_t use_foreground_masks;
  int32_t partition;
  int32_t do_temporal_filter;
  int32_t resident_frames;
} derp_seq_options;
typedef struct {
  int32_t frame, from_rank, to_rank;
} derp_seq_transfer;
void derp_seq_options_default(derp_seq_options* o);
void derp_seq_window(int frame, int first, int last, int time_radius, int* lo, int* hi);
int derp_seq_owner(int first, int last, int world, int partition, int frame);
int derp_seq_plan(int first, int last, int world, int time_radius, int partition, derp_seq_transfer* out, int cap);
int derp_seq_create(derp_seq** out, derp_ctx* ctx, int first, int last, int rank, int world,
                    const derp_seq_options* opt);
void derp_seq_destroy(derp_seq* seq);
int derp_seq_counts(const derp_seq* seq, int* n_owned, int* n_halo);
int derp_seq_frames(const derp_seq* seq, int halo, int* frames, int cap);
int derp_seq_frame_slot(const derp_seq* seq, int frame);
int derp_seq_host_inputs(derp_seq* seq, int frame, int level, const uint16_t* color_bgr, const uint8_t* fg_masks,
                         const float* background_disparity);
int derp_seq_upload_color_plane(derp_seq* seq, int frame, int level, int src, const uint16_t* bgr);
int derp_seq_upload_disparity(derp_seq* seq, int frame, int level, int dst, const float* disparity);
int derp_seq_download_disparity(derp_seq* seq, int frame, int level, int dst, float* disparity);
int derp_seq_buffer(derp_seq* seq, int frame, int level, int kind, void** ptr, size_t* bytes);
int derp_seq_buffer_copy(derp_seq* seq, int frame, int level, int kind, void* host, size_t bytes, int to_device);
int derp_rccl_unique_id(void* out128, size_t cap);
int derp_seq_attach_rccl(derp_seq* seq, const void* unique_id, size_t bytes);
int derp_seq_attach_loopback(derp_seq* seq, derp_seq* const* peers, int n_peers);
int derp_seq_attach_external(derp_seq* seq);
int derp_seq_selftest(derp_seq* seq, int words);
int derp_seq_exchange_inputs(derp_seq* seq);
int derp_seq_exchange_inputs_level(derp_seq* seq, int level);
int derp_seq_level_compute(derp_seq* seq, int level);
int derp_seq_level_compute_frame(derp_seq* seq, int level, int frame);
int derp_seq_level_provided_frame(derp_seq* seq, int level, int frame);
int derp_seq_level_exchange(derp_seq* seq, int level);
int derp_seq_mark_exchanged(derp_seq* seq, int level);
int derp_seq_level_filter(derp_seq* seq, int level);
int derp_seq_level_filter_frame(derp_seq* seq, int level, int frame);
int derp_seq_download_filtered(derp_seq* seq, int frame, int level, int dst, float* disparity);
int derp_seq_run(derp_seq* seq, int level_start, int level_end);
int derp_seq_stats(derp_seq* seq, uint64_t* bytes_sent, uint64_t* bytes_received, double* exchange_ms);
int derp_seq_stats_reset(derp_seq* seq);
int derp_seq_exchange_exposed_ms(derp_seq* seq, double* exposed_ms);

typedef struct derp_isp derp_isp;
enum { DERP_ISP_MAX_ROLLOFF = 16 };
enum { DERP_ISP_BILINEAR = 0, DERP_ISP_FREQUENCY = 1, DERP_ISP_EDGE_AWARE = 2, DERP_ISP_CHROMA_SUPPRESSED = 3 };
enum {
  DERP_ISP_STAGE_LOAD = 0,
  DERP_ISP_STAGE_PIXEL = 1,
  DERP_ISP_STAGE_STUCK = 2,
  DERP_ISP_STAGE_DEMOSAIC = 3,
  DERP_ISP_STAGE_COLOR = 4,
  DERP_ISP_STAGE_LOWPASS = 5,
  DERP_ISP_STAGE_SHARPENED = 6
};
typedef struct {
  int32_t bits_per_pixel;
  int32_t width, height;
  int32_t is_little_endian;
  int32_t is_row_major;
  char bayer_pattern[8];
  char plane_order[8];
  float black_level[3];
  float clamp_min[3];
  float clamp_max[3];
  int32_t stuck_pixel_threshold;
  float stuck_pixel_darkness_threshold;
  int32_t stuck_pixel_radius;
  int32_t n_rolloff_h, n_rolloff_v;
  float rolloff_h[DERP_ISP_MAX_ROLLOFF][3];
  float rolloff_v[DERP_ISP_MAX_ROLLOFF][3];
  float white_balance_gain[3];
  float ccm[9];
  float saturation;
  float gamma[3];
  float low_key_boost[3];
  float high_key_boost[3];
  float contrast;
  float sharpening[3];
  float sharpening_support;
  float noise_core;
  int32_t n_companding_lut;
} derp_isp_config;
void derp_isp_config_default(derp_isp_config* cfg);
int derp_isp_create(derp_isp** out, int device, const derp_isp_config* cfg, int demosaic_filter, int pow2_downscale,
                    int apply_tone_curve);
void derp_isp_destroy(derp_isp* isp);
int derp_isp_output_size(const derp_isp* isp, int* width, int* height);
int derp_isp_process(derp_isp* isp, const void* raw, size_t raw_bytes, void* out_bgr);
int derp_isp_stage(derp_isp* isp, int stage, float* out);
int derp_isp_tables(const derp_isp* isp, float* vignette_h, float* vignette_v, float* ccm9, float* tone_lut);

typedef struct {
  float v0[3], v1[3], v2[3];
  float e1[3], e2[3];
  float normal[3];
  float color[3];
} derp_sim_triangle;
typedef struct {
  float center[3];
  float radius;
  int32_t skip;
  int32_t first;
  int32_t count;
  int32_t n_children;
} derp_sim_node;
typedef struct derp_sim_scene derp_sim_scene;
derp_sim_scene* derp_sim_scene_create(void);
void derp_sim_scene_destroy(derp_sim_scene* scene);
int derp_sim_scene_icosahedrons(derp_sim_scene* scene, int count, double min_dist, double max_dist, double min_radius,
                                double max_radius, int red_triangle);
int derp_sim_scene_cubes(derp_sim_scene* scene);
int derp_sim_scene_ground_plane(derp_sim_scene* scene, double ground_plane_dist_m);
int derp_sim_scene_add_triangle(derp_sim_scene* scene, const float* v0, const float* v1, const float* v2,
                                const float* color_bgr);
int derp_sim_bvh_build(derp_sim_scene* scene, int leaf_threshold, int split_k, int max_depth);
int derp_sim_scene_counts(const derp_sim_scene* scene, int* n_triangles, int* n_nodes, int* n_leaf_indices);
int derp_sim_scene_get(const derp_sim_scene* scene, derp_sim_triangle* triangles, derp_sim_node* nodes,
                       int32_t* leaf_indices);
void derp_sim_perlin_table(uint8_t* p512);
void derp_sim_icosahedron(float* vertices36, int32_t* faces60);
int derp_sim_noise(float* bgr, int w, int h, double amplitude);
int derp_sim_trace_host(const derp_sim_scene* scene, const float* rays6, size_t n, float* out_bgrd);

typedef struct {
  double ceiling_position, ceiling_width, ceiling_depth;
  double marble_scale;
  int32_t marble;
  int32_t pad;
} derp_sim_params;
enum {
  DERP_SIM_STAGE_ORIGIN = 0,
  DERP_SIM_STAGE_DIRECTION,
  DERP_SIM_STAGE_HIT,
  DERP_SIM_STAGE_DISTANCE,
  DERP_SIM_STAGE_COLOR
};
typedef struct derp_sim derp_sim;
int derp_sim_create(derp_sim** out, int device);
void derp_sim_destroy(derp_sim* sim);
int derp_sim_upload(derp_sim* sim, const derp_sim_triangle* triangles, int n_triangles, const derp_sim_node* nodes,
                    int n_nodes, const int32_t* leaf_indices, int n_leaf_indices, const uint8_t* skybox_bgr, int sky_w,
                    int sky_h, const uint8_t* ceiling_bgr, int ceiling_w, int ceiling_h, const derp_sim_params* params);
int derp_sim_render_camera(derp_sim* sim, const derp_camera_desc* cam, int aas, float* bgr_out, float* depth_out);
int derp_sim_render_equirect(derp_sim* sim, int w, int h, int aas, int stereo, double interpupillary_radius,
                             float* bgr_a, float* bgr_b, float* aux_out);
int derp_sim_trace_rays(derp_sim* sim, const float* rays6, size_t n);
int derp_sim_stage_size(const derp_sim* sim, int* width, int* height);
int derp_sim_stage(derp_sim* sim, int stage, int eye, void* out);

int derp_get_counters(derp_ctx* ctx, uint64_t* n_cost, uint64_t* n_pair, uint64_t* insufficient);
int derp_reset_counters(derp_ctx* ctx);
int derp_profile_enable(derp_ctx* ctx, int on);
int derp_profile_reset(derp_ctx* ctx);
int derp_profile_query(derp_ctx* ctx, const char* stage, int level, double* ms, int* launches,
                       uint64_t* n_cost, uint64_t* n_pair);
int derp_profile_memoised(derp_ctx* ctx, const char* stage, int level, uint64_t* n_memoised);
int derp_device_name(derp_ctx* ctx, char* buf, int n);
int derp_device_memory(derp_ctx* ctx, uint64_t* free_bytes, uint64_t* total_bytes);

int derp_host_nth_element_pairs(float* pairs, int n, int nth);
float derp_host_minstd_uniform(int seed, uint64_t draw_index, float a, float b);

#ifdef __cplusplus
}
#endif
#endif
```

Before: 475.9 Mpix/s.

## Band XCD swizzle and allow multi-tile walks in cost kernels, add block trace

Changes the random-proposal and ping-pong launch grids so the XCD swizzle can group tiles into row bands. Random proposals turns banding on by default when the image is tall enough, which aims to keep neighbouring tiles on the same XCD for L2 reuse. An optional walk mode lets one block handle several tiles and build the atan LUT only once, but it is selected only through an environment variable. It also adds a compile-time block-timing trace and a host tile-map helper for debugging, at the cost of extra grid padding and some added code complexity.

```diff
diff --git a/facebook360_dep_amd/csrc/derp_capi.hip b/facebook360_dep_amd/csrc/derp_capi.hip
--- a/facebook360_dep_amd/csrc/derp_capi.hip
+++ b/facebook360_dep_amd/csrc/derp_capi.hip
@@ -112,7 +112,24 @@
   V.fovMask = c->w.fovMask.as<uint8_t>();
   V.pairCount = c->w.pairCount.as<uint8_t>();
   V.counters = counter_slot(c, stage, L);
+#if DERP_BLOCK_TRACE
+  V.blockTrace = nullptr;
+#endif
   return V;
+}
+int block_trace_attach(derp_ctx* c, LevelView& V, int which, int gridX, int gridY) {
+#if DERP_BLOCK_TRACE
+  DevBuf& buf = c->blockTrace[which][V.level];
+  const size_t bytes = (size_t)gridX * gridY * 2 * sizeof(unsigned long long);
+  ALLOC(c, buf, bytes);
+  HIPCHK(c, hipMemsetAsync(buf.as<unsigned long long>(), 0, bytes, c->stream));
+  V.blockTrace = buf.as<unsigned long long>();
+  c->blockTraceGrid[which][V.level][0] = gridX;
+  c->blockTraceGrid[which][V.level][1] = gridY;
+#else
+  (void)c, (void)V, (void)which, (void)gridX, (void)gridY;
+#endif
+  return 0;
 }
 
 const dim3 kBlurBlk(64, 4, 1);
@@ -407,8 +424,29 @@
   return tilesX * tilesY * (256 / kCostBlock);
 }
 constexpr size_t kCostLdsPerSrc = (size_t)kCostBlock * sizeof(SsdPair);
-int round8(int n) {
-  return (n + 7) / 8 * 8;
+struct CostGrid {
+  int blocks, bands, perBlock;
+};
+constexpr int kCostMaxBands = 4, kCostMaxTilesPerBlock = 4;
+int cost_grid_blocks(int tiles, int bands, int perBlock) {
+  const int items = (tiles + perBlock - 1) / perBlock, unit = 8 * bands;
+  return (items + unit - 1) / unit * unit;
+}
+CostGrid cost_grid(const derp_ctx* c, int tiles, int tilesX, bool spread) {
+  const auto pow2_floor = [](int v, int cap) {
+    int p = 1;
+    while (p * 2 <= std::min(v, cap)) {
+      p *= 2;
+    }
+    return p;
+  };
+  CostGrid g;
+  g.perBlock = c->costTilesPerBlock > 0 ? pow2_floor(c->costTilesPerBlock, kCostMaxTilesPerBlock) : 1;
+  const int rowOfSquares = tilesX * (256 / kCostBlock) * kTileBlock;
+  g.bands = c->xcdBands > 0 ? pow2_floor(c->xcdBands, kCostMaxBands)
+                            : spread ? pow2_floor(std::max(1, tiles / (8 * rowOfSquares)), kCostMaxBands) : 1;
+  g.blocks = cost_grid_blocks(tiles, g.bands, g.perBlock);
+  return g;
 }
 size_t lds_for_waves(size_t needed, int waves, size_t ldsPerCu, size_t fixed) {
   if (waves <= 0 || waves >= 4) {
@@ -464,8 +502,12 @@
   int tilesX;
   const int tiles = tiles_of(V.W, V.H, tilesX);
   const size_t lds = lds_for_waves(kCostLdsPerSrc * (size_t)(c->S), c->randomWaves, c->ldsPerCu, kCostLdsStatic);
-  hipLaunchKernelGGL(cost_four_waves(c) ? k_random_proposals : k_random_proposals_w3, dim3(round8(tiles), nd),
-                     dim3(kCostBlock), lds, c->stream, V, c->w.rank.as<int>(), tilesX, tiles);
+  const CostGrid cg = cost_grid(c, tiles, tilesX, true);
+  TRY(block_trace_attach(c, V, 0, cg.blocks, nd));
+  const bool four = cost_four_waves(c);
+  const auto kernel = cg.perBlock > 1 ? (four ? k_random_proposals_walk : k_random_proposals_walk_w3)
+                                      : (four ? k_random_proposals : k_random_proposals_w3);
+  hipLaunchKernelGGL(kernel, dim3(cg.blocks, nd), dim3(kCostBlock), lds, c->stream, V, c->w.rank.as<int>(), tilesX, cg.bands, cg.perBlock);
   KCHECK(c);
   return 0;
 }
@@ -483,11 +525,15 @@
   const int tiles = tiles_of(V.W, V.H, tilesX);
   const size_t lds = lds_for_waves(kCostLdsPerSrc * (size_t)(c->S), c->ppWaves, c->ldsPerCu, kCostLdsStatic);
   const bool four = cost_four_waves(c);
-  const auto kernel = c->ppCompact ? (four ? k_ping_pong : k_ping_pong_w3) : (four ? k_ping_pong_loop : k_ping_pong_loop_w3);
+  const CostGrid cg = cost_grid(c, tiles, tilesX, false);
+  const auto kernel = cg.perBlock > 1
+                          ? (c->ppCompact ? (four ? k_ping_pong_walk : k_ping_pong_walk_w3) : (four ? k_ping_pong_loop_walk : k_ping_pong_loop_walk_w3))
+                          : (c->ppCompact ? (four ? k_ping_pong : k_ping_pong_w3) : (four ? k_ping_pong_loop : k_ping_pong_loop_w3));
+  TRY(block_trace_attach(c, V, 1, cg.blocks, nd));
   for (int it = 1; it <= c->opt.ping_pong_iterations; ++it) {
-    hipLaunchKernelGGL(kernel, dim3(round8(tiles), nd), dim3(kCostBlock), lds,
+    hipLaunchKernelGGL(kernel, dim3(cg.blocks, nd), dim3(kCostBlock), lds,
                        c->stream, V, c->w.changed.as<uint8_t>(), c->w.dispRes.as<float>(), c->w.costRes.as<float>(), tilesX,
-                       (int)(it == 1 && c->randomRanThisLevel && !c->noMemo));
+                       (int)(it == 1 && c->randomRanThisLevel && !c->noMemo), cg.bands, cg.perBlock);
     KCHECK(c);
     hipLaunchKernelGGL(k_ping_pong_commit, dim3(flat_grid(n * nd)), dim3(256), 0, c->stream,
                        c->w.disparity.as<float>() + (size_t)dst0 * n, c->w.cost.as<float>() + (size_t)dst0 * n,
@@ -921,6 +967,12 @@
   if (const char* e = getenv("DERP_XCD_ROTATE")) {
     c->xcdRotate = atoi(e);
   }
+  if (const char* e = getenv("DERP_XCD_BANDS")) {
+    c->xcdBands = atoi(e);
+  }
+  if (const char* e = getenv("DERP_COST_TILES_PER_BLOCK")) {
+    c->costTilesPerBlock = atoi(e);
+  }
   c->noMemo = getenv("DERP_NO_MEMO") != nullptr;
   if (const char* e = getenv("DERP_PP_COMPACT")) {
     c->ppCompact = atoi(e) != 0;
diff --git a/facebook360_dep_amd/csrc/derp_ctx.h b/facebook360_dep_amd/csrc/derp_ctx.h
--- a/facebook360_dep_amd/csrc/derp_ctx.h
+++ b/facebook360_dep_amd/csrc/derp_ctx.h
@@ -116,6 +116,9 @@
   double accMs[ST_COUNT][kMaxLevels] = {};
   int accLaunch[ST_COUNT][kMaxLevels] = {};
   int xcdRotate = 1;
+  int xcdBands = 0, costTilesPerBlock = 0;
+  DevBuf blockTrace[2][kMaxLevels];
+  int blockTraceGrid[2][kMaxLevels][2] = {};
   bool noMemo = false;
   bool ppCompact = true;
   int randomWaves = 0, ppWaves = 0;
diff --git a/facebook360_dep_amd/csrc/derp_debug_api.h b/facebook360_dep_amd/csrc/derp_debug_api.h
--- a/facebook360_dep_amd/csrc/derp_debug_api.h
+++ b/facebook360_dep_amd/csrc/derp_debug_api.h
@@ -266,6 +266,29 @@
   *n_memoised = m;
   return 0;
 }
+int derp_debug_block_trace(derp_ctx* c, const char* stage, int level, uint64_t* out, size_t capacity, int* grid_x, int* grid_y) {
+  if (!c || !stage || !grid_x || !grid_y || level < 0 || level >= kMaxLevels) {
+    return fail(c, "bad arguments");
+  }
+#if DERP_BLOCK_TRACE
+  const int which = strcmp(stage, "random_proposals") == 0 ? 0 : strcmp(stage, "ping_pong") == 0 ? 1 : -1;
+  if (which < 0) {
+    return fail(c, "no block trace of stage '%s'", stage);
+  }
+  *grid_x = c->blockTraceGrid[which][level][0];
+  *grid_y = c->blockTraceGrid[which][level][1];
+  const size_t n = (size_t)*grid_x * *grid_y * 2;
+  if (!out || capacity < n) {
+    return 0;
+  }
+  HIPCHK(c, hipStreamSynchronize(c->stream));
+  HIPCHK(c, hipMemcpy(out, c->blockTrace[which][level].as<unsigned long long>(), n * sizeof(uint64_t), hipMemcpyDeviceToHost));
+  return 0;
+#else
+  (void)out, (void)capacity;
+  return fail(c, "this library records no block trace: build it with -DDERP_BLOCK_TRACE=1 (tools/block_trace.py)");
+#endif
+}
 int derp_device_memory(derp_ctx* c, uint64_t* free_bytes, uint64_t* total_bytes) {
   TRY(use_device(c));
   size_t f = 0, t = 0;
@@ -299,3 +322,19 @@
   uint32_t state = minstd_jump(minstd_seed(seed), draw_index);
   return minstd_uniform(state, a, b);
 }
+int derp_host_cost_tile_map(int tiles, int bands, int rot, int per_block, int* out, int capacity) {
+  const auto pow2 = [](int v) { return v > 0 && (v & (v - 1)) == 0; };
+  if (tiles <= 0 || !pow2(bands) || bands > kCostMaxBands || !pow2(per_block) || per_block > kCostMaxTilesPerBlock || !out) {
+    return 0;
+  }
+  const int blocks = cost_grid_blocks(tiles, bands, per_block);
+  if ((long long)blocks * per_block > capacity) {
+    return 0;
+  }
+  for (int b = 0; b < blocks; ++b) {
+    for (int step = 0; step < per_block; ++step) {
+      out[b * per_block + step] = cost_block_tile(b, blocks, rot, bands, per_block, step);
+    }
+  }
+  return blocks;
+}
diff --git a/facebook360_dep_amd/csrc/derp_kernels.h b/facebook360_dep_amd/csrc/derp_kernels.h
--- a/facebook360_dep_amd/csrc/derp_kernels.h
+++ b/facebook360_dep_amd/csrc/derp_kernels.h
@@ -24,6 +24,9 @@
 #endif
 #ifndef DERP_PHASE_TIMERS
 #define DERP_PHASE_TIMERS 0
+#endif
+#ifndef DERP_BLOCK_TRACE
+#define DERP_BLOCK_TRACE 0
 #endif
 static constexpr int kCostBlock = 64;
 static constexpr int kTileBlock = 4;
@@ -68,6 +71,9 @@
   const uint8_t* fovMask;
   uint8_t* pairCount;
   unsigned long long* counters;
+#if DERP_BLOCK_TRACE
+  unsigned long long* blockTrace;
+#endif
 };
 
 __device__ __forceinline__ size_t warp_plane(const LevelView& V) {
@@ -93,10 +99,17 @@
   return *reinterpret_cast<T*>(reinterpret_cast<char*>(const_cast<typename std::remove_const<T>::type*>(base)) + i * (unsigned)sizeof(T));
 }
 
-__device__ __forceinline__ int xcd_swizzle(int b, int n, int rot) {
+__host__ __device__ __forceinline__ int xcd_swizzle(int b, int n, int rot, int bands) {
   const int per = (n + 7) >> 3;
-  const int t = (((b & 7) + rot) & 7) * per + (b >> 3);
-  return t;
+  if (bands <= 1) {
+    return (((b & 7) + rot) & 7) * per + (b >> 3);
+  }
+  const int run = per / bands;
+  const int j = b >> 3, k = j / run;
+  return (k * 8 + (((b & 7) + rot) & 7)) * run + (j - k * run);
+}
+__host__ __device__ __forceinline__ int cost_block_tile(int b, int n, int rot, int bands, int perBlock, int step) {
+  return xcd_swizzle(b, n, rot, bands) * perBlock + step;
 }
 
 __device__ __forceinline__ void tile_pixel(int item, int tilesX, int& x, int& y) {
@@ -196,6 +209,30 @@
 #endif
   __syncthreads();
   return pairs;
+}
+__device__ __forceinline__ LdsPairs cost_block_prologue(PatchWin*& win) {
+  static_assert(kCostBlock == 64, "a wave leaves an empty tile on its own: the block must be that one wave");
+  extern __shared__ SsdPair ldsPairs[];
+  __shared__ PatchWin patchWin[kCostBlock / 64];
+  win = &patchWin[threadIdx.x >> 6];
+#if defined(__HIP_DEVICE_COMPILE__)
+  __shared__ double atanLut[kAtanLutDoubles];
+  return LdsPairs{ldsPairs + threadIdx.x, (int)blockDim.x, atanLut};
+#else
+  return LdsPairs{ldsPairs + threadIdx.x, (int)blockDim.x, nullptr};
+#endif
+}
+__device__ __forceinline__ void cost_tile_prologue(const LevelView& V, int d, int x0, int y0, PatchWin* win, const LdsPairs& pairs,
+                                                   bool& lutReady) {
+  __syncthreads();
+  patch_window_fill(V, V.dst2src[d], x0, y0, win);
+#if defined(__HIP_DEVICE_COMPILE__)
+  if (!lutReady) {
+    atan_lut_fill(const_cast<double*>(pairs.atanLut));
+    lutReady = true;
+  }
+#endif
+  __syncthreads();
 }
 
 struct SsdTexels {
@@ -571,6 +608,25 @@
   return 0u;
 #endif
 }
+__device__ __forceinline__ unsigned long long block_trace_begin() {
+#if DERP_BLOCK_TRACE
+  return (unsigned long long)wall_clock64();
+#else
+  return 0ull;
+#endif
+}
+__device__ __forceinline__ void block_trace_end(const LevelView& V, unsigned long long t0) {
+#if DERP_BLOCK_TRACE
+  if ((threadIdx.x & 63) == 0 && V.blockTrace) {
+    unsigned long long* e = V.blockTrace + ((size_t)blockIdx.y * gridDim.x + blockIdx.x) * 2;
+    e[0] = t0;
+    e[1] = (unsigned long long)wall_clock64();
+  }
+#else
+  (void)V;
+  (void)t0;
+#endif
+}
 template <bool RANDOM>
 constexpr int cost_sees_lean() {
   return 2 + (RANDOM ? 4 : 0);
@@ -1323,74 +1379,64 @@
   }
 }
 
-__device__ __forceinline__ void random_proposals_body(const LevelView& V, const int* __restrict__ rank, int tilesX, int tilesPerDst) {
-  const int dl = blockIdx.y;
+__device__ __forceinline__ void random_proposals_tile(const LevelView& V, const int* __restrict__ rank, int dl, int x, int y, bool go,
+                                                      const PatchWin* win, LdsPairs& pairs) {
   const int d = V.dst0 + dl;
-  int x, y;
-  tile_pixel(xcd_swizzle(blockIdx.x, gridDim.x, V.xcdRotate ? d : 0), tilesX, x, y);
-  PatchWin* win;
-  LdsPairs pairs = cost_wave_prologue(V, d, x - (int)(threadIdx.x & 7), y - (int)((threadIdx.x & 63) >> 3), win);
+  const int own = V.dst2src[d];
+  const size_t n = (size_t)V.W * V.H;
+  const unsigned idx = (unsigned)y * (unsigned)V.W + (unsigned)x;
+  float* disp = V.disparity + (size_t)d * n;
   unsigned nCost = 0, nPair = 0, nSlots = 0, nSlotsFirst = 0;
   PhaseTimers tm;
   const unsigned tk0 = phase_clock();
-  if (x >= 1 && y >= 1 && x < V.W - 1 && y < V.H - 1) {
-    const int own = V.dst2src[d];
-    const size_t n = (size_t)V.W * V.H;
-    const unsigned idx = (unsigned)y * (unsigned)V.W + (unsigned)x;
-    float* disp = V.disparity + (size_t)d * n;
-    if ((V.fovMask + (size_t)d * n)[idx]) {
-      if (!(V.srcFg + (size_t)own * n)[idx]) {
-        disp[idx] = (V.bgDisp + (size_t)d * n)[idx];
-      } else if (random_gate(V, d, own, idx)) {
-        PixCtx px;
-        load_pixctx<false>(V, d, own, x, y, win, px);
-        const unsigned cull = behind_sources(V, d, idx);
-        float currDisp = at32(disp, idx);
-        float currCost = 0.f, costThresh = 0.f, amplitude = 0.f;
-        const int spare = V.S - 1;
-        const float maxDisp = 1.0f / V.minDepthM;
-        uint32_t state = (uint32_t)at32(rank + (size_t)d * n, idx);
-        for (int i = -1; i < V.randomProposals; ++i) {
-          unsigned pi = idx;
-          asm("" : "+v"(pi) : "s"(i));
-          const float minDisp = V.hasFg ? at32(V.bgDisp + (size_t)d * n, pi) : (1.0f / V.maxDepthM);
-          float propDisp = currDisp;
-          if (i >= 0) {
-            const float lo = fmaxf(minDisp, currDisp - amplitude), hi = fminf(maxDisp, currDisp + amplitude);
-            propDisp = minstd_uniform(state, lo, hi);
-          }
-          unsigned np = 0;
-          const float2 pr = compute_cost<true, true>(V, dl, own, px, propDisp, pairs, np, cull, pi, i < 0 ? &nSlotsFirst : &nSlots, &tm);
-          nPair += np;
-          bool take;
-          if (i < 0) {
-            costThresh = fminf(0.5f * pr.x, 5.0f);
-            amplitude = (maxDisp - minDisp) / 2.0f;
-            take = true;
-          } else {
-            take = pr.x < currCost && pr.x < costThresh;
-            if (take) {
-              amplitude /= 2.0f;
-            }
-          }
-          if (take) {
-            currCost = pr.x;
-            currDisp = propDisp;
-            pairs.set(spare, SsdPair{pr.y, __uint_as_float(np)});
-          }
+  if (go) {
+    PixCtx px;
+    load_pixctx<false>(V, d, own, x, y, win, px);
+    const unsigned cull = behind_sources(V, d, idx);
+    float currDisp = at32(disp, idx);
+    float currCost = 0.f, costThresh = 0.f, amplitude = 0.f;
+    const int spare = V.S - 1;
+    const float maxDisp = 1.0f / V.minDepthM;
+    uint32_t state = (uint32_t)at32(rank + (size_t)d * n, idx);
+    for (int i = -1; i < V.randomProposals; ++i) {
+      unsigned pi = idx;
+      asm("" : "+v"(pi) : "s"(i));
+      const float minDisp = V.hasFg ? at32(V.bgDisp + (size_t)d * n, pi) : (1.0f / V.maxDepthM);
+      float propDisp = currDisp;
+      if (i >= 0) {
+        const float lo = fmaxf(minDisp, currDisp - amplitude), hi = fminf(maxDisp, currDisp + amplitude);
+        propDisp = minstd_uniform(state, lo, hi);
+      }
+      unsigned np = 0;
+      const float2 pr = compute_cost<true, true>(V, dl, own, px, propDisp, pairs, np, cull, pi, i < 0 ? &nSlotsFirst : &nSlots, &tm);
+      nPair += np;
+      bool take;
+      if (i < 0) {
+        costThresh = fminf(0.5f * pr.x, 5.0f);
+        amplitude = (maxDisp - minDisp) / 2.0f;
+        take = true;
+      } else {
+        take = pr.x < currCost && pr.x < costThresh;
+        if (take) {
+          amplitude /= 2.0f;
         }
-        {
-          unsigned pi = idx;
-          asm("" : "+v"(pi) : "v"(currCost));
-          const SsdPair best = pairs.get(spare);
-          at32(V.confidence + (size_t)d * n, pi) = best.first;
-          at32(V.pairCount + (size_t)d * n, pi) = (uint8_t)__float_as_uint(best.second);
-          at32(disp, pi) = currDisp;
-          at32(V.cost + (size_t)d * n, pi) = currCost;
-        }
-        nCost = 1u + (unsigned)max(V.randomProposals, 0);
-      }
-    }
+      }
+      if (take) {
+        currCost = pr.x;
+        currDisp = propDisp;
+        pairs.set(spare, SsdPair{pr.y, __uint_as_float(np)});
+      }
+    }
+    {
+      unsigned pi = idx;
+      asm("" : "+v"(pi) : "v"(currCost));
+      const SsdPair best = pairs.get(spare);
+      at32(V.confidence + (size_t)d * n, pi) = best.first;
+      at32(V.pairCount + (size_t)d * n, pi) = (uint8_t)__float_as_uint(best.second);
+      at32(disp, pi) = currDisp;
+      at32(V.cost + (size_t)d * n, pi) = currCost;
+    }
+    nCost = 1u + (unsigned)max(V.randomProposals, 0);
   }
 #if DERP_PHASE_TIMERS
   if ((threadIdx.x & 63) == 0) {
@@ -1408,13 +1454,56 @@
 #endif
 }
 
+template <bool WALK>
+__device__ __forceinline__ void random_proposals_body(const LevelView& V, const int* __restrict__ rank, int tilesX, int bands,
+                                                      int perBlock) {
+  const unsigned long long bt0 = block_trace_begin();
+  const int steps = WALK ? perBlock : 1;
+  const int dl = blockIdx.y;
+  const int d = V.dst0 + dl;
+  PatchWin* win;
+  LdsPairs pairs = cost_block_prologue(win);
+  bool lutReady = false;
+  for (int step = 0; step < steps; ++step) {
+    int x, y;
+    tile_pixel(cost_block_tile(blockIdx.x, gridDim.x, V.xcdRotate ? d : 0, bands, steps, step), tilesX, x, y);
+    bool go = false;
+    if (x >= 1 && y >= 1 && x < V.W - 1 && y < V.H - 1) {
+      const int own = V.dst2src[d];
+      const size_t n = (size_t)V.W * V.H;
+      const unsigned idx = (unsigned)y * (unsigned)V.W + (unsigned)x;
+      if ((V.fovMask + (size_t)d * n)[idx]) {
+        if (!(V.srcFg + (size_t)own * n)[idx]) {
+          (V.disparity + (size_t)d * n)[idx] = (V.bgDisp + (size_t)d * n)[idx];
+        } else {
+          go = random_gate(V, d, own, idx);
+        }
+      }
+    }
+    if (__ballot(go) == 0ull) {
+      continue;
+    }
+    cost_tile_prologue(V, d, x - (int)(threadIdx.x & 7), y - (int)((threadIdx.x & 63) >> 3), win, pairs, lutReady);
+    random_proposals_tile(V, rank, dl, x, y, go, win, pairs);
+  }
+  block_trace_end(V, bt0);
+}
+
 __global__ void __launch_bounds__(kCostBlock, DERP_RANDOM_MIN_WAVES)
-    k_random_proposals(LevelView V, const int* __restrict__ rank, int tilesX, int tilesPerDst) {
-  random_proposals_body(V, rank, tilesX, tilesPerDst);
+    k_random_proposals(LevelView V, const int* __restrict__ rank, int tilesX, int bands, int perBlock) {
+  random_proposals_body<false>(V, rank, tilesX, bands, perBlock);
 }
 __global__ void __launch_bounds__(kCostBlock, 3)
-    k_random_proposals_w3(LevelView V, const int* __restrict__ rank, int tilesX, int tilesPerDst) {
-  random_proposals_body(V, rank, tilesX, tilesPerDst);
+    k_random_proposals_w3(LevelView V, const int* __restrict__ rank, int tilesX, int bands, int perBlock) {
+  random_proposals_body<false>(V, rank, tilesX, bands, perBlock);
+}
+__global__ void __launch_bounds__(kCostBlock, DERP_RANDOM_MIN_WAVES)
+    k_random_proposals_walk(LevelView V, const int* __restrict__ rank, int tilesX, int bands, int perBlock) {
+  random_proposals_body<true>(V, rank, tilesX, bands, perBlock);
+}
+__global__ void __launch_bounds__(kCostBlock, 3)
+    k_random_proposals_walk_w3(LevelView V, const int* __restrict__ rank, int tilesX, int bands, int perBlock) {
+  random_proposals_body<true>(V, rank, tilesX, bands, perBlock);
 }
 
 __constant__ int kCandidates[9][2] = {{0, 0}, {-1, 0}, {1, 0}, {0, -1}, {0, 1}, {-2, -2}, {2, -2}, {-2, 2}, {2, 2}};
@@ -1541,6 +1630,9 @@
       }
     }
   }
+  if (__ballot(cmask != 0u) == 0ull) {
+    return;
+  }
   unsigned cull = 0;
   const unsigned behind = eval ? V.behind[(size_t)d * n + idx] : ~0u;
   for (int t = 0; t < V.S - 1; ++t) {
@@ -1618,14 +1710,10 @@
 }
 
 template <bool COMPACT>
-__device__ __forceinline__ void ping_pong_body(const LevelView& V, const uint8_t* __restrict__ changed, float* __restrict__ dispRes,
-                                               float* __restrict__ costRes, int tilesX, int useMemo) {
-  const int dl = blockIdx.y;
+__device__ __forceinline__ void ping_pong_tile(const LevelView& V, const uint8_t* __restrict__ changed, float* __restrict__ dispRes,
+                                               float* __restrict__ costRes, int dl, int x, int y, const PatchWin* win, LdsPairs& pairs,
+                                               int useMemo) {
   const int d = V.dst0 + dl;
-  int x, y;
-  tile_pixel(xcd_swizzle(blockIdx.x, gridDim.x, V.xcdRotate ? d : 0), tilesX, x, y);
-  PatchWin* win;
-  LdsPairs pairs = cost_wave_prologue(V, d, x - (int)(threadIdx.x & 7), y - (int)((threadIdx.x & 63) >> 3), win);
   unsigned counts = 0, fillSlots = 0;
   PhaseTimers tm;
   const unsigned tk0 = phase_clock();
@@ -1666,26 +1754,40 @@
   }
 }
 
-__global__ void __launch_bounds__(kCostBlock, DERP_COST_MIN_WAVES)
-    k_ping_pong(LevelView V, const uint8_t* __restrict__ changed, float* __restrict__ dispRes,
-                float* __restrict__ costRes, int tilesX, int useMemo) {
-  ping_pong_body<true>(V, changed, dispRes, costRes, tilesX, useMemo);
-}
-__global__ void __launch_bounds__(kCostBlock, 3)
-    k_ping_pong_w3(LevelView V, const uint8_t* __restrict__ changed, float* __restrict__ dispRes,
-                   float* __restrict__ costRes, int tilesX, int useMemo) {
-  ping_pong_body<true>(V, changed, dispRes, costRes, tilesX, useMemo);
-}
-__global__ void __launch_bounds__(kCostBlock, DERP_COST_MIN_WAVES)
-    k_ping_pong_loop(LevelView V, const uint8_t* __restrict__ changed, float* __restrict__ dispRes,
-                     float* __restrict__ costRes, int tilesX, int useMemo) {
-  ping_pong_body<false>(V, changed, dispRes, costRes, tilesX, useMemo);
-}
-__global__ void __launch_bounds__(kCostBlock, 3)
-    k_ping_pong_loop_w3(LevelView V, const uint8_t* __restrict__ changed, float* __restrict__ dispRes,
-                        float* __restrict__ costRes, int tilesX, int useMemo) {
-  ping_pong_body<false>(V, changed, dispRes, costRes, tilesX, useMemo);
-}
+template <bool COMPACT, bool WALK>
+__device__ __forceinline__ void ping_pong_body(const LevelView& V, const uint8_t* __restrict__ changed, float* __restrict__ dispRes,
+                                               float* __restrict__ costRes, int tilesX, int useMemo, int bands, int perBlock) {
+  const unsigned long long bt0 = block_trace_begin();
+  const int steps = WALK ? perBlock : 1;
+  const int dl = blockIdx.y;
+  const int d = V.dst0 + dl;
+  PatchWin* win;
+  LdsPairs pairs = cost_block_prologue(win);
+  bool lutReady = false;
+  for (int step = 0; step < steps; ++step) {
+    int x, y;
+    tile_pixel(cost_block_tile(blockIdx.x, gridDim.x, V.xcdRotate ? d : 0, bands, steps, step), tilesX, x, y);
+    cost_tile_prologue(V, d, x - (int)(threadIdx.x & 7), y - (int)((threadIdx.x & 63) >> 3), win, pairs, lutReady);
+    ping_pong_tile<COMPACT>(V, changed, dispRes, costRes, dl, x, y, win, pairs, useMemo);
+  }
+  block_trace_end(V, bt0);
+}
+
+#define DERP_PING_PONG_KERNEL(NAME, WAVES, COMPACT, WALK)                                                                   \
+  __global__ void __launch_bounds__(kCostBlock, WAVES)                                                                      \
+      NAME(LevelView V, const uint8_t* __restrict__ changed, float* __restrict__ dispRes, float* __restrict__ costRes,     \
+           int tilesX, int useMemo, int bands, int perBlock) {                                                              \
+    ping_pong_body<COMPACT, WALK>(V, changed, dispRes, costRes, tilesX, useMemo, bands, perBlock);                          \
+  }
+DERP_PING_PONG_KERNEL(k_ping_pong, DERP_COST_MIN_WAVES, true, false)
+DERP_PING_PONG_KERNEL(k_ping_pong_w3, 3, true, false)
+DERP_PING_PONG_KERNEL(k_ping_pong_loop, DERP_COST_MIN_WAVES, false, false)
+DERP_PING_PONG_KERNEL(k_ping_pong_loop_w3, 3, false, false)
+DERP_PING_PONG_KERNEL(k_ping_pong_walk, DERP_COST_MIN_WAVES, true, true)
+DERP_PING_PONG_KERNEL(k_ping_pong_walk_w3, 3, true, true)
+DERP_PING_PONG_KERNEL(k_ping_pong_loop_walk, DERP_COST_MIN_WAVES, false, true)
+DERP_PING_PONG_KERNEL(k_ping_pong_loop_walk_w3, 3, false, true)
+#undef DERP_PING_PONG_KERNEL
 
 __global__ void k_ping_pong_commit(float* __restrict__ disp, float* __restrict__ cost, const float* __restrict__ dispRes,
                                    const float* __restrict__ costRes, uint8_t* __restrict__ changed, size_t n) {
diff --git a/facebook360_dep_amd/derp.py b/facebook360_dep_amd/derp.py
--- a/facebook360_dep_amd/derp.py
+++ b/facebook360_dep_amd/derp.py
@@ -95,7 +95,7 @@
     "derp_level_begin", "derp_stage_reproject_colors", "derp_stage_brute_force", "derp_stage_random_proposals",
     "derp_stage_ping_pong", "derp_stage_mismatches", "derp_stage_bilateral_filter", "derp_stage_median_filter", "derp_stage_mask_fov",
     "derp_level_end", "derp_set_level_disparity", "derp_get_level_disparity", "derp_cost_map", "derp_debug_download",
-    "derp_debug_atan2_ypos", "derp_debug_fp64", "derp_debug_sees",
+    "derp_debug_atan2_ypos", "derp_debug_fp64", "derp_debug_sees", "derp_debug_block_trace",
     "derp_ssim", "derp_average_score", "derp_rephotograph", "derp_rephotograph_upload", "derp_rephotograph_render", "derp_canopy_cubemap",
     "derp_render_params_default", "derp_render_upload", "derp_render", "derp_render_format_size", "derp_render_format",
     "derp_render_vertices",
@@ -106,7 +106,7 @@
     "derp_fov_mask", "derp_layer_disparities", "derp_download_mismatch_mask", "derp_upsample_disparity", "derp_joint_bilateral_u16", "derp_joint_bilateral_f32", "derp_masked_median",
     "derp_temporal_filter", "derp_temporal_filter_dev", "derp_dev_disparity", "derp_dev_color", "derp_dev_mask",
     "derp_get_counters", "derp_reset_counters", "derp_profile_enable", "derp_profile_reset", "derp_profile_query", "derp_profile_memoised",
-    "derp_device_name", "derp_device_memory", "derp_host_nth_element_pairs", "derp_host_minstd_uniform",
+    "derp_device_name", "derp_device_memory", "derp_host_nth_element_pairs", "derp_host_minstd_uniform", "derp_host_cost_tile_map",
     "derp_set_frame_slots", "derp_select_frame", "derp_frame_slots", "derp_host_alloc", "derp_host_free", "derp_bind_thread", "derp_host_register", "derp_host_unregister",
     "derp_seq_options_default", "derp_seq_window", "derp_seq_owner", "derp_seq_plan", "derp_seq_create", "derp_seq_destroy",
     "derp_seq_counts", "derp_seq_frames", "derp_seq_frame_slot", "derp_seq_buffer", "derp_rccl_unique_id",
@@ -702,6 +702,13 @@
         self._ck(lib().derp_profile_memoised(self.h, stage.encode(), level, C.byref(m)))
         return m.value
 
+    def block_trace(self, stage, level):
+        gx, gy = C.c_int(), C.c_int()
+        self._ck(lib().derp_debug_block_trace(self.h, stage.encode(), level, None, C.c_size_t(0), C.byref(gx), C.byref(gy)))
+        out = np.zeros((gy.value, gx.value, 2), dtype=np.uint64)
+        self._ck(lib().derp_debug_block_trace(self.h, stage.encode(), level, _p(out), C.c_size_t(out.size), C.byref(gx), C.byref(gy)))
+        return out
+
     def device_memory(self):
         f, t = C.c_uint64(), C.c_uint64()
         self._ck(lib().derp_device_memory(self.h, C.byref(f), C.byref(t)))
@@ -749,6 +756,15 @@
 
 def host_minstd_uniform(seed, draw_index, a, b):
     return lib().derp_host_minstd_uniform(seed, draw_index, C.c_float(a), C.c_float(b))
+
+
+def host_cost_tile_map(tiles, bands, rot, per_block):
+    cap = (tiles + 8 * bands * per_block) // per_block * per_block + 8 * bands * per_block
+    out = np.empty(cap, dtype=np.int32)
+    blocks = lib().derp_host_cost_tile_map(tiles, bands, rot, per_block, _p(out), cap)
+    if blocks <= 0:
+        raise ValueError("bad tile map arguments")
+    return out[:blocks * per_block].reshape(blocks, per_block)
 
 
 def average_score(score, mask):
diff --git a/include/derp_hip.h b/include/derp_hip.h
--- a/include/derp_hip.h
+++ b/include/derp_hip.h
@@ -112,6 +112,8 @@
 int derp_debug_atan2_ypos(derp_ctx* ctx, const double* y, const double* x, double* out, size_t n);
 int derp_debug_fp64(derp_ctx* ctx, int op, const double* a, const double* b, double* out, size_t n);
 int derp_debug_sees(derp_ctx* ctx, int src, const double* xyz, size_t n, double* out);
+
+int derp_debug_block_trace(derp_ctx* ctx, const char* stage, int level, uint64_t* out, size_t capacity, int* grid_x, int* grid_y);
 
 int derp_download_mismatch_mask(derp_ctx* ctx, int dst, uint8_t* out);
 
@@ -385,6 +387,7 @@
 
 int derp_host_nth_element_pairs(float* pairs, int n, int nth);
 float derp_host_minstd_uniform(int seed, uint64_t draw_index, float a, float b);
+int derp_host_cost_tile_map(int tiles, int bands, int rot, int per_block, int* out, int capacity);
 
 #ifdef __cplusplus
 }
```

Measured after the change: 502.3 Mpix/s (median of 6 runs). +5.5%, better.
